# AHupuJR/REFID

Measured on AMD Instinct MI355X. Metric: interpolated frames/sec (train step) GoPro 256x256 11+1, higher is better.
Workload: dtype f32

## Files before the change

### include/refid_hip.h

```cpp
#ifndef REFID_HIP_H
#define REFID_HIP_H

#include <stddef.h>
#include <stdint.h>

#ifdef __cplusplus
extern "C" {
#endif

#define REFID_ABI_VERSION 9

const char* refid_last_error(void);
int refid_abi_version(void);
int refid_experimental_tiles(void);

int refid_device_cu_count(void);

typedef struct refid_pw_extras {
    const float* ln_gamma; const float* ln_beta; float ln_eps; float* ln_out; int ld_ln_out;
    const float* pool; int pool_parts; float inv_hw; int hw; int se_c;
    const float* se_w1; const float* se_b1; const float* se_w2; const float* se_b2;
    float* se_m; float* se_z1; float* se_s;
    float* xs_out; int ld_xs_out;
    const float* res2; int ld_res2;
    float* out2; int ld_out2;
} refid_pw_extras;

typedef struct refid_conv_desc {
    const float* in_a;  const float* in_b;
    int ld_a, ld_b;
    int c_a, c_b;
    const float* w_packed;
    const float* bias;
    float* out;          int ld_out;
    const float* res;    int ld_res;
    const float* mask;   int ld_mask;
    int n, h, w;
    int ho, wo;
    int cout;
    int cout_pad;
    int co_base;
    int kh, kw, stride, pad;
    int mode;
    float slope_pre, slope_post, slope_mask;
    int algo;
    int split_k;
    int wino_tile;
    const refid_pw_extras* pw;
    int mfma_terms;
    float* ws;  size_t ws_bytes;
    const float* add2; int ld_add2;
    float* out2;       int ld_out2;
    int mask_mode;
} refid_conv_desc;

size_t refid_conv_workspace_bytes(const refid_conv_desc* d);
int refid_conv2d(const refid_conv_desc* d, void* stream);

int refid_conv_kc(int kh, int kw, int stride, int mode);
const char* refid_conv_tile_name(int kh, int kw, int stride, int mode, int cout);
int refid_conv_bn(int kh, int kw, int stride, int mode, int cout);

#define REFID_WGRAD_MAX_GROUPS 24
typedef struct refid_wgrad_desc {
    const float* g;      int ld_g;   int c_o;
    const float* in_a;   const float* in_b;
    int ld_a, ld_b;
    int c_a, c_b;
    float* dw;
    float* db;
    float* slabs;
    int n, h, w, ho, wo;
    int kh, kw, stride, pad;
    int i_base, i_total;
    int o_real;
    int algo;
    int phase;
    int groups;
    const float* g_more[REFID_WGRAD_MAX_GROUPS - 1];
    const float* in_a_more[REFID_WGRAD_MAX_GROUPS - 1];
    const float* in_b_more[REFID_WGRAD_MAX_GROUPS - 1];
} refid_wgrad_desc;

size_t refid_wgrad_workspace_bytes(const refid_wgrad_desc* d);
int refid_conv2d_wgrad(const refid_wgrad_desc* d, void* stream);
int refid_wgrad_finish_flush(void* stream);

enum { REFID_ROLE_FWD = 0, REFID_ROLE_DGRAD = 1, REFID_ROLE_CONVT = 2, REFID_ROLE_CONVT_DGRAD = 3,
       REFID_ROLE_DOWN_DGRAD = 4,
       REFID_ROLE_WINO_FWD = 5, REFID_ROLE_WINO_DGRAD = 6,
       REFID_ROLE_CONVT_DGRAD_PW = 7 };
size_t refid_packed_weight_floats(int role, int o, int i, int kh, int kw, int kc, int bn);
int refid_pack_conv_weights(const float* w, float* packed, int role, int o, int i, int kh, int kw,
                            int kc, int bn, void* stream);

int refid_pack_conv_weights_scaled(const float* w, const float* oscale, float* packed, int role, int o,
                                   int i, int kh, int kw, int kc, int bn, void* stream);
int refid_pack_conv_weights_bf16(const float* w, const float* oscale, void* packed_bf16, int role, int o, int i,
                                 int kh, int kw, int kc, int bn, void* stream);
size_t refid_packed_weight_split_bytes(int role, int o, int i, int kh, int kw, int bn, int planes);
size_t refid_packed_weight_split_f16_bytes(int role, int o, int i, int kh, int kw, int bn);
int refid_pack_conv_weights_split_f16(const float* w, const float* oscale, void* packed, int role, int o, int i,
                                      int kh, int kw, int bn, void* stream);
int refid_pack_conv_weights_split(const float* w, const float* oscale, void* packed, int role, int o, int i,
                                  int kh, int kw, int bn, int planes, void* stream);
size_t refid_packed_weight_wino6_bytes(int role, int o, int i, int bn);
int refid_pack_conv_weights_wino6(const float* w, const float* oscale, void* packed, int role, int o, int i, int bn,
                                  void* stream);
size_t refid_packed_weight_wino3h_bytes(int role, int o, int i, int bn);
int refid_pack_conv_weights_wino3h(const float* w, const float* oscale, void* packed, int role, int o, int i, int bn,
                                   void* stream);
size_t refid_packed_weight_wino1h_bytes(int role, int o, int i, int bn);
int refid_pack_conv_weights_wino1h(const float* w, const float* oscale, void* packed, int role, int o, int i, int bn,
                                   void* stream);
size_t refid_pack_entry_bytes(void);
int refid_pack_table_check(const void* table_host, int n);
int refid_pack_entry_fill(void* entry_host, int kind, const float* w, const float* oscale, void* dst, int role, int o, int i,
                          int kh, int kw, int kc, int bn, int planes, int blk0);
int refid_pack_batch_prepass(const void* table_dev, int n, void* stream);
int refid_pack_batch(const void* table_dev, int n, int nblocks, void* stream);
int refid_mul_vec(const float* a, const float* b, float* out, int n, void* stream);
int refid_fold_back(const float* w, const float* b, const float* scale, const float* gw_folded,
                    const float* gb_folded, float* gw, float* gb, float* dscale, int rows, int k, void* stream);

int refid_layernorm2d_fwd(const float* x, int ld_x, const float* w, const float* b, float* out,
                          int ld_out, long long npix, int c, float eps, void* stream);
int refid_layernorm2d_bwd_parts(long long npix, int c);
int refid_layernorm2d_bwd(const float* g, int ld_g, const float* x, int ld_x, const float* w, float* gx,
                          int ld_gx, const float* res, int ld_res, float* dw, float* db, float* parts, long long npix,
                          int c, float eps, void* stream);
int refid_hin_parts(int hw);
int refid_hin_lrelu_fwd(const float* x, int ld_x, const float* gamma, const float* beta, float* out, int ld_out,
                        float* stats, float* parts, int n, int hw, int c, int ch, float eps, float slope,
                        void* stream);
int refid_hin_lrelu_bwd(const float* g, int ld_g, const float* out, int ld_out, const float* x, int ld_x,
                        const float* gamma, const float* stats, float* gx, int ld_gx, float* dgamma,
                        float* dbeta, float* sums, float* parts, int n, int hw, int c, int ch, float slope,
                        void* stream);
int refid_fac_fwd(const float* feat, int ld_feat, const float* filt, int ld_filt, float* out, int ld_out,
                  long long npix, int c, void* stream);
int refid_fac_bwd(const float* g, int ld_g, const float* feat, int ld_feat, const float* filt, int ld_filt,
                  float* gfeat, int ld_gfeat, float* gfilt, int ld_gfilt, long long npix, int c, void* stream);

int refid_dwconv_pool_parts(int h, int wd, int c);
int refid_dwconv3x3_gelu_fwd(const float* in, int ld_in, const float* w, const float* b, float* pre,
                             float* act, float* pool, int n, int h, int wd, int c, void* stream);
int refid_dwconv3x3_bwd_parts(int h, int wd, int c);
int refid_dwconv3x3_bwd(const float* gd, const float* in, int ld_in, const float* w, float* gin,
                        float* dw, float* db, float* parts, int n, int h, int wd, int c, void* stream);
int refid_se_fwd(const float* pool, int n_parts, float inv_hw, const float* w1, const float* b1, const float* w2,
                 const float* b2, float* m, float* z1, float* s, int n, int c, void* stream);
int refid_se_bwd(const float* gs, const float* s, const float* z1, const float* m, const float* w1,
                 const float* w2, float* gm, float* dw1, float* db1, float* dw2, float* db2, float* scratch, int n,
                 int c, void* stream);
int refid_scale_cat(const float* xi, const float* xe, const float* s, float* out, int n, int hw, int c,
                    void* stream);
int refid_egaca_gs_reduce_parts(int hw, int c);
int refid_egaca_gs_reduce(const float* gxs, const float* xi, const float* xe, float* gs, float* parts, int n, int hw,
                          int c, void* stream);
int refid_egaca_bwd_elem(const float* gxs, const float* s, const float* gm, float inv_hw, const float* dwe,
                         float* gdwe, float* gxi, int accumulate_xi, int n, int hw, int c, void* stream);
int refid_gelu_fwd(const float* in, float* out, long long count, void* stream);
int refid_gelu_bwd(const float* g, const float* in, float* out, long long count, void* stream);
int refid_colsum_parts(long long npix, int c);
int refid_colsum(const float* g, int ld_g, float* db, float* parts, long long npix, int c, void* stream);

int refid_charbonnier_parts(long long count);
int refid_charbonnier(const float* pred, const float* gt, float* grad, double* loss_sum, double* parts, long long count,
                      float eps, float grad_scale, void* stream);
int refid_psnr_loss_parts(int n_samples, long long per_sample);
int refid_psnr_loss(const float* pred, const float* gt, float* grad, double* sq, double* loss, double* parts, int n_samples,
                    long long per_sample, float weight, void* stream);
#define REFID_SQNORM_WORDS 2049
int refid_grad_sqnorm(const float* g, double* out, long long count, void* stream);
int refid_clip_adamw(float* p, const float* g, float* m, float* v, const double* sqnorm, float max_norm,
                     float grad_scale, float lr, float beta1, float beta2, float eps, float weight_decay,
                     int step, long long count, void* stream);

int refid_clip_adamw_dev(float* p, const float* g, float* m, float* v, const double* sqnorm, float max_norm,
                         float grad_scale, const float* hyper, float beta1, float beta2, float eps,
                         float weight_decay, long long count, void* stream);

int refid_nchw_to_nhwc(const float* src, long long src_batch_stride, float* dst, int n, int c, int h, int w,
                       int c_pad, void* stream);
int refid_nchw_tsum_to_nhwc(const float* src, long long src_batch_stride, long long t_stride, int t_count, float* dst,
                            int n, int c, int h, int w, int c_pad, void* stream);
int refid_nhwc_to_nchw(const float* src, int ld, float* dst, long long dst_batch_stride,
                       int n, int c, int h, int w, void* stream);
int refid_nchw_to_nhwc_tb(const float* src, long long b_stride, long long t_stride, float* dst, int nb, int nt, int c, int h,
                          int w, int c_pad, void* stream);
int refid_nhwc_to_nchw_tb(const float* src, int ld, float* dst, long long b_stride, long long t_stride, int nb, int nt, int c,
                          int h, int w, void* stream);
int refid_rows_sum_defer(int on);
int refid_rows_sum_flush(void* stream);
int refid_add(const float* a, const float* b, float* out, long long count, void* stream);
#define REFID_SUM_MAX 48
int refid_sum_n(const float* const* in, int n, float* out, long long count, void* stream);
int refid_act_bwd(const float* g, const float* y, float* out, float slope, int accumulate,
                  long long count, void* stream);

int refid_events_to_voxel(const double* ts, const int* xs, const int* ys, const float* ps, long long n_events,
                          int num_bins, int width, int height, double first_stamp, double last_stamp,
                          float* voxel, void* stream);
int refid_sqerr_u8_parts(int n_frames, long long frame_elems);
int refid_sqerr_u8(const float* a, const float* b, int n_frames, long long frame_elems, double* sq, double* parts,
                   void* stream);
int refid_ssim3d_u8_parts(int n_frames, int h, int w);
int refid_ssim3d_u8(const float* a, const float* b, int n_frames, int h, int w, double* sum_out, double* parts,
                    void* stream);
#define REFID_VAL_TAIL_BGR 1
long long refid_val_tail_parts(int n_frames, int h, int w);
int refid_val_tail(const float* pred, const float* gt, int n_frames, int h, int w, int flags, unsigned char* pred_u8,
                   unsigned char* gt_u8, unsigned long long* sq_out, double* ssim_out, void* parts, void* stream);
int refid_tile_add(const float* tile, float* acc, float* cnt, int c, int th, int tw, int h, int w, int i0, int j0,
                   void* stream);
int refid_tile_normalize(float* acc, const float* cnt, int c, int h, int w, void* stream);

typedef struct refid_sample_desc {
    const float* events;
    long long n_events;
    float first_stamp, last_stamp;
    int height, width;
    const unsigned char* frames;
    long long frame_stride;
    int row_pitch;
    int y0, x0;
    int top, left;
    int hflip, vflip, rot90;
} refid_sample_desc;

#define REFID_LAYOUT_BLUR 0
#define REFID_LAYOUT_SHARP 1
#define REFID_ASSEMBLE_ZERO 1
#define REFID_ASSEMBLE_SCATTER 2
#define REFID_ASSEMBLE_FINISH 4
#define REFID_ASSEMBLE_FRAMES 8
#define REFID_ASSEMBLE_ALL 15
typedef struct refid_assemble_desc {
    const refid_sample_desc* samples_host;
    const refid_sample_desc* samples_dev;
    int batch;
    int m, n, layout;
    int crop_h, crop_w;
    long long* scratch;
    float* lq;
    float* voxel;
    float* gt;
} refid_assemble_desc;

int refid_assemble_bins(int m, int n, int layout);
int refid_assemble_batch(const refid_assemble_desc* d, int stages, void* stream);

long long refid_voxel_norm_parts(int batch, long long per_sample);
int refid_voxel_norm(const float* in, float* out, int batch, long long per_sample, void* parts, void* stream);

#define REFID_ASSEMBLE_STATS 16
typedef struct refid_single_desc {
    const refid_sample_desc* samples_host;
    const refid_sample_desc* samples_dev;
    int batch;
    int bins;
    int crop_h, crop_w;
    int norm;
    long long* scratch;
    void* parts;
    float* lq;
    float* voxel;
    float* gt;
} refid_single_desc;
int refid_single_bins(int bins);
int refid_assemble_single(const refid_single_desc* d, int stages, void* stream);

typedef struct refid_seq_pair {
    int left, right;
    long long row0, row1;
    float first_stamp, last_stamp;
} refid_seq_pair;
typedef struct refid_seq_desc {
    const float* events;
    long long n_events;
    const unsigned char* frames;
    int n_frames;
    long long frame_stride;
    int row_pitch;
    int height, width;
    int bgr;
    const refid_seq_pair* pairs_host;
    const refid_seq_pair* pairs_dev;
    int n_pairs;
    int m, n, layout;
    int out_h, out_w;
    long long* scratch;
    float* lq;
    float* voxel;
} refid_seq_desc;
int refid_seq_assemble(const refid_seq_desc* d, int stages, void* stream);

typedef struct refid_seq_single_desc {
    const float* events;
    long long n_events;
    const unsigned char* frames;
    int n_frames;
    long long frame_stride;
    int row_pitch;
    int height, width;
    int bgr;
    const refid_seq_pair* items_host;
    const refid_seq_pair* items_dev;
    int n_items;
    int bins;
    int norm;
    int out_h, out_w;
    long long* scratch;
    void* parts;
// ... 55 lines not shown
```

### refid_amd/_lib.py

```python
import ctypes as C
import os

_HERE = os.path.dirname(os.path.abspath(__file__))
LIB_PATH = os.path.join(_HERE, "librefid_hip.so")


class RefidHipError(RuntimeError):
    pass


class PwExtras(C.Structure):
    _fields_ = [
        ("ln_gamma", C.c_void_p), ("ln_beta", C.c_void_p), ("ln_eps", C.c_float), ("ln_out", C.c_void_p),
        ("ld_ln_out", C.c_int),
        ("pool", C.c_void_p), ("pool_parts", C.c_int), ("inv_hw", C.c_float), ("hw", C.c_int), ("se_c", C.c_int),
        ("se_w1", C.c_void_p), ("se_b1", C.c_void_p), ("se_w2", C.c_void_p), ("se_b2", C.c_void_p),
        ("se_m", C.c_void_p), ("se_z1", C.c_void_p), ("se_s", C.c_void_p),
        ("xs_out", C.c_void_p), ("ld_xs_out", C.c_int),
        ("res2", C.c_void_p), ("ld_res2", C.c_int),
        ("out2", C.c_void_p), ("ld_out2", C.c_int),
    ]


class ConvDesc(C.Structure):
    _fields_ = [
        ("in_a", C.c_void_p), ("in_b", C.c_void_p),
        ("ld_a", C.c_int), ("ld_b", C.c_int),
        ("c_a", C.c_int), ("c_b", C.c_int),
        ("w_packed", C.c_void_p), ("bias", C.c_void_p),
        ("out", C.c_void_p), ("ld_out", C.c_int),
        ("res", C.c_void_p), ("ld_res", C.c_int),
        ("mask", C.c_void_p), ("ld_mask", C.c_int),
        ("n", C.c_int), ("h", C.c_int), ("w", C.c_int),
        ("ho", C.c_int), ("wo", C.c_int),
        ("cout", C.c_int), ("cout_pad", C.c_int), ("co_base", C.c_int),
        ("kh", C.c_int), ("kw", C.c_int), ("stride", C.c_int), ("pad", C.c_int),
        ("mode", C.c_int),
        ("slope_pre", C.c_float), ("slope_post", C.c_float), ("slope_mask", C.c_float),
        ("algo", C.c_int),
        ("split_k", C.c_int), ("wino_tile", C.c_int),
        ("pw", C.POINTER(PwExtras)),
        ("mfma_terms", C.c_int),
        ("ws", C.c_void_p), ("ws_bytes", C.c_size_t),
        ("add2", C.c_void_p), ("ld_add2", C.c_int), ("out2", C.c_void_p), ("ld_out2", C.c_int),
        ("mask_mode", C.c_int),
    ]


WGRAD_MAX_GROUPS = 24


class WgradDesc(C.Structure):
    _fields_ = [
        ("g", C.c_void_p), ("ld_g", C.c_int), ("c_o", C.c_int),
        ("in_a", C.c_void_p), ("in_b", C.c_void_p),
        ("ld_a", C.c_int), ("ld_b", C.c_int),
        ("c_a", C.c_int), ("c_b", C.c_int),
        ("dw", C.c_void_p), ("db", C.c_void_p), ("slabs", C.c_void_p),
        ("n", C.c_int), ("h", C.c_int), ("w", C.c_int), ("ho", C.c_int), ("wo", C.c_int),
        ("kh", C.c_int), ("kw", C.c_int), ("stride", C.c_int), ("pad", C.c_int),
        ("i_base", C.c_int), ("i_total", C.c_int), ("o_real", C.c_int), ("algo", C.c_int),
        ("phase", C.c_int),
        ("groups", C.c_int),
        ("g_more", C.c_void_p * (WGRAD_MAX_GROUPS - 1)), ("in_a_more", C.c_void_p * (WGRAD_MAX_GROUPS - 1)),
        ("in_b_more", C.c_void_p * (WGRAD_MAX_GROUPS - 1)),
    ]


class SampleDesc(C.Structure):
    _fields_ = [
        ("events", C.c_void_p), ("n_events", C.c_longlong),
        ("first_stamp", C.c_float), ("last_stamp", C.c_float),
        ("height", C.c_int), ("width", C.c_int),
        ("frames", C.c_void_p), ("frame_stride", C.c_longlong), ("row_pitch", C.c_int),
        ("y0", C.c_int), ("x0", C.c_int),
        ("top", C.c_int), ("left", C.c_int),
        ("hflip", C.c_int), ("vflip", C.c_int), ("rot90", C.c_int),
    ]


class AssembleDesc(C.Structure):
    _fields_ = [
        ("samples_host", C.c_void_p), ("samples_dev", C.c_void_p),
        ("batch", C.c_int),
        ("m", C.c_int), ("n", C.c_int), ("layout", C.c_int),
        ("crop_h", C.c_int), ("crop_w", C.c_int),
        ("scratch", C.c_void_p),
        ("lq", C.c_void_p), ("voxel", C.c_void_p), ("gt", C.c_void_p),
    ]


class SingleDesc(C.Structure):
    _fields_ = [
        ("samples_host", C.c_void_p), ("samples_dev", C.c_void_p),
        ("batch", C.c_int),
        ("bins", C.c_int),
        ("crop_h", C.c_int), ("crop_w", C.c_int),
        ("norm", C.c_int),
        ("scratch", C.c_void_p),
        ("parts", C.c_void_p),
        ("lq", C.c_void_p), ("voxel", C.c_void_p), ("gt", C.c_void_p),
    ]


class SeqPair(C.Structure):
    _fields_ = [
        ("left", C.c_int), ("right", C.c_int),
        ("row0", C.c_longlong), ("row1", C.c_longlong),
        ("first_stamp", C.c_float), ("last_stamp", C.c_float),
    ]


class SeqDesc(C.Structure):
    _fields_ = [
        ("events", C.c_void_p), ("n_events", C.c_longlong),
        ("frames", C.c_void_p), ("n_frames", C.c_int),
        ("frame_stride", C.c_longlong), ("row_pitch", C.c_int), ("height", C.c_int), ("width", C.c_int), ("bgr", C.c_int),
        ("pairs_host", C.c_void_p), ("pairs_dev", C.c_void_p), ("n_pairs", C.c_int),
        ("m", C.c_int), ("n", C.c_int), ("layout", C.c_int),
        ("out_h", C.c_int), ("out_w", C.c_int),
        ("scratch", C.c_void_p),
        ("lq", C.c_void_p), ("voxel", C.c_void_p),
    ]


class SeqSingleDesc(C.Structure):
    _fields_ = [
        ("events", C.c_void_p), ("n_events", C.c_longlong),
        ("frames", C.c_void_p), ("n_frames", C.c_int),
        ("frame_stride", C.c_longlong), ("row_pitch", C.c_int), ("height", C.c_int), ("width", C.c_int), ("bgr", C.c_int),
        ("items_host", C.c_void_p), ("items_dev", C.c_void_p), ("n_items", C.c_int),
        ("bins", C.c_int), ("norm", C.c_int),
        ("out_h", C.c_int), ("out_w", C.c_int),
        ("scratch", C.c_void_p),
        ("parts", C.c_void_p),
        ("lq", C.c_void_p), ("voxel", C.c_void_p),
    ]


class PngUnfilterDesc(C.Structure):
    _fields_ = [
        ("rows", C.c_void_p), ("frames", C.c_void_p), ("bands", C.c_void_p),
        ("n_bands", C.c_int32), ("n_frames", C.c_int32), ("height", C.c_int32), ("width", C.c_int32), ("channels", C.c_int32),
    ]


class PngFilterDesc(C.Structure):
    _fields_ = [
        ("frames", C.c_void_p), ("rows", C.c_void_p), ("costs", C.c_void_p),
        ("n_frames", C.c_int32), ("height", C.c_int32), ("width", C.c_int32), ("mode", C.c_int32),
    ]


class PngDeflateDesc(C.Structure):
    _fields_ = [
        ("src", C.c_void_p), ("out", C.c_void_p), ("lens", C.c_void_p), ("work", C.c_void_p),
        ("n_streams", C.c_int32), ("stream_bytes", C.c_int32), ("block_bytes", C.c_int32), ("out_pitch", C.c_int32),
    ]


LAYOUT_BLUR, LAYOUT_SHARP = 0, 1
ASSEMBLE_ZERO, ASSEMBLE_SCATTER, ASSEMBLE_FINISH, ASSEMBLE_FRAMES, ASSEMBLE_ALL = 1, 2, 4, 8, 15
ASSEMBLE_STATS = 16

VAL_TAIL_BGR = 1
NIQE_BGR = 1
SCORE_BGR = 1
PNG_MAX_ROW_BYTES = 32760
PNG_FILTER_ADAPTIVE = 5
PNG_FILTER_MAX_WIDTH = 11184810
PNG_DEFLATE_BLOCK = 32768
PNG_DEFLATE_MAX_BLOCK = 65535
PNG_DEFLATE_RECORD = 1088
ABI_VERSION = 9
_lib = None

_PACK_FAMILY = (
    ("refid_packed_weight_floats", ("refid_pack_conv_weights", "refid_pack_conv_weights_scaled", "refid_pack_conv_weights_bf16"),
     "role o i kh kw kc bn"),
    ("refid_packed_weight_split_bytes", ("refid_pack_conv_weights_split",), "role o i kh kw bn planes"),
    ("refid_packed_weight_split_f16_bytes", ("refid_pack_conv_weights_split_f16",), "role o i kh kw bn"),
    ("refid_packed_weight_wino6_bytes", ("refid_pack_conv_weights_wino6",), "role o i bn"),
    ("refid_packed_weight_wino3h_bytes", ("refid_pack_conv_weights_wino3h",), "role o i bn"),
    ("refid_packed_weight_wino1h_bytes", ("refid_pack_conv_weights_wino1h",), "role o i bn"),
)
PACK_GEO = {}


def lib():
    global _lib
    if _lib is not None:
        return _lib
    if not os.path.exists(LIB_PATH):
        raise RefidHipError(
            f"{LIB_PATH} not found: the HIP extension is required (no CPU/eager fallback). "
            "Run `python -m refid_amd.build`.")
    L = C.CDLL(LIB_PATH)
    L.refid_last_error.restype = C.c_char_p
    L.refid_abi_version.restype = C.c_int
    L.refid_device_cu_count.restype = C.c_int
    L.refid_conv2d.argtypes = [C.POINTER(ConvDesc), C.c_void_p]
    L.refid_conv_workspace_bytes.argtypes = [C.POINTER(ConvDesc)]
    L.refid_conv_workspace_bytes.restype = C.c_size_t
    L.refid_conv_kc.argtypes = [C.c_int] * 4
    L.refid_conv_bn.argtypes = [C.c_int] * 5
    L.refid_conv_tile_name.argtypes = [C.c_int] * 5
    L.refid_conv_tile_name.restype = C.c_char_p
    L.refid_wgrad_workspace_bytes.argtypes = [C.POINTER(WgradDesc)]
    L.refid_wgrad_workspace_bytes.restype = C.c_size_t
    L.refid_conv2d_wgrad.argtypes = [C.POINTER(WgradDesc), C.c_void_p]
    L.refid_wgrad_finish_flush.argtypes = [C.c_void_p]
    L.refid_rows_sum_defer.argtypes = [C.c_int]
    L.refid_rows_sum_flush.argtypes = [C.c_void_p]
    L.refid_nchw_to_nhwc.argtypes = [C.c_void_p, C.c_longlong, C.c_void_p] + [C.c_int] * 5 + [C.c_void_p]
    L.refid_nchw_tsum_to_nhwc.argtypes = [C.c_void_p, C.c_longlong, C.c_longlong, C.c_int, C.c_void_p] + [C.c_int] * 5 + \
        [C.c_void_p]
    L.refid_nhwc_to_nchw.argtypes = [C.c_void_p, C.c_int, C.c_void_p, C.c_longlong] + [C.c_int] * 4 + [C.c_void_p]
    L.refid_nchw_to_nhwc_tb.argtypes = [C.c_void_p, C.c_longlong, C.c_longlong, C.c_void_p] + [C.c_int] * 6 + [C.c_void_p]
    L.refid_nhwc_to_nchw_tb.argtypes = [C.c_void_p, C.c_int, C.c_void_p, C.c_longlong, C.c_longlong] + [C.c_int] * 5 + [C.c_void_p]
    L.refid_add.argtypes = [C.c_void_p, C.c_void_p, C.c_void_p, C.c_longlong, C.c_void_p]
    L.refid_sum_n.argtypes = [C.c_void_p, C.c_int, C.c_void_p, C.c_longlong, C.c_void_p]
    L.refid_act_bwd.argtypes = [C.c_void_p, C.c_void_p, C.c_void_p, C.c_float, C.c_int, C.c_longlong, C.c_void_p]
    _bind_extra(L)
    if L.refid_abi_version() != ABI_VERSION:
        raise RefidHipError("librefid_hip.so ABI version mismatch")
    _lib = L
    return L


def _bind_extra(L):
    vp, i, f, ll = C.c_void_p, C.c_int, C.c_float, C.c_longlong
    for size, entries, geo in _PACK_FAMILY:
        PACK_GEO[size] = geo = tuple(geo.split())
        getattr(L, size).argtypes, getattr(L, size).restype = [i] * len(geo), C.c_size_t
        for e in entries:
            PACK_GEO[e] = geo
            getattr(L, e).argtypes = [vp] * (2 if e == "refid_pack_conv_weights" else 3) + [i] * len(geo) + [vp]
    L.refid_pack_batch_prepass.argtypes = [vp, i, vp]
    L.refid_mul_vec.argtypes = [vp, vp, vp, i, vp]
    L.refid_pack_entry_bytes.restype = C.c_size_t
    L.refid_pack_entry_bytes.argtypes = []
    L.refid_pack_entry_fill.argtypes = [vp, i, vp, vp, vp, i, i, i, i, i, i, i, i, i]
    L.refid_pack_batch.argtypes = [vp, i, i, vp]
    L.refid_pack_table_check.argtypes = [vp, i]
    L.refid_fold_back.argtypes = [vp] * 8 + [i, i, vp]
    L.refid_layernorm2d_fwd.argtypes = [vp, i, vp, vp, vp, i, ll, i, f, vp]
    L.refid_layernorm2d_bwd.argtypes = [vp, i, vp, i, vp, vp, i, vp, i, vp, vp, vp, ll, i, f, vp]
    L.refid_layernorm2d_bwd_parts.argtypes = [ll, i]
    L.refid_colsum_parts.argtypes = [ll, i]
    L.refid_egaca_gs_reduce_parts.argtypes = [i, i]
    L.refid_dwconv3x3_gelu_fwd.argtypes = [vp, i, vp, vp, vp, vp, vp, i, i, i, i, vp]
    L.refid_dwconv3x3_bwd.argtypes = [vp, vp, i, vp, vp, vp, vp, vp, i, i, i, i, vp]
    L.refid_dwconv3x3_bwd_parts.argtypes = [i, i, i]
    L.refid_se_fwd.argtypes = [vp, i, f, vp, vp, vp, vp, vp, vp, vp, i, i, vp]
    L.refid_dwconv_pool_parts.argtypes = [i, i, i]
    L.refid_se_bwd.argtypes = [vp] * 12 + [i, i, vp]
    L.refid_scale_cat.argtypes = [vp, vp, vp, vp, i, i, i, vp]
    L.refid_egaca_gs_reduce.argtypes = [vp, vp, vp, vp, vp, i, i, i, vp]
    L.refid_egaca_bwd_elem.argtypes = [vp, vp, vp, f, vp, vp, vp, i, i, i, i, vp]
    L.refid_gelu_fwd.argtypes = [vp, vp, ll, vp]
    L.refid_gelu_bwd.argtypes = [vp, vp, vp, ll, vp]
    L.refid_colsum.argtypes = [vp, i, vp, vp, ll, i, vp]
    L.refid_charbonnier_parts.argtypes = [ll]
    L.refid_charbonnier.argtypes = [vp, vp, vp, vp, vp, ll, f, f, vp]
    L.refid_grad_sqnorm.argtypes = [vp, vp, ll, vp]
    L.refid_psnr_loss_parts.argtypes = [i, ll]
    L.refid_psnr_loss.argtypes = [vp, vp, vp, vp, vp, vp, i, ll, f, vp]
    L.refid_clip_adamw.argtypes = [vp, vp, vp, vp, vp, f, f, f, f, f, f, f, i, ll, vp]
    L.refid_clip_adamw_dev.argtypes = [vp, vp, vp, vp, vp, f, f, vp, f, f, f, f, ll, vp]
    d = C.c_double
    L.refid_events_to_voxel.argtypes = [vp, vp, vp, vp, ll, i, i, i, d, d, vp, vp]
    L.refid_sqerr_u8_parts.argtypes = [i, ll]
    L.refid_sqerr_u8.argtypes = [vp, vp, i, ll, vp, vp, vp]
    L.refid_ssim3d_u8_parts.argtypes = [i, i, i]
    L.refid_ssim3d_u8.argtypes = [vp, vp, i, i, i, vp, vp, vp]
    L.refid_val_tail_parts.argtypes = [i, i, i]
    L.refid_val_tail_parts.restype = ll
    L.refid_val_tail.argtypes = [vp, vp, i, i, i, i, vp, vp, vp, vp, vp, vp]
    L.refid_tile_add.argtypes = [vp, vp, vp, i, i, i, i, i, i, i, vp]
    L.refid_tile_normalize.argtypes = [vp, vp, i, i, i, vp]
    L.refid_hin_parts.argtypes = [i]
    L.refid_hin_lrelu_fwd.argtypes = [vp, i, vp, vp, vp, i, vp, vp, i, i, i, i, f, f, vp]
    L.refid_hin_lrelu_bwd.argtypes = [vp, i, vp, i, vp, i, vp, vp, vp, i, vp, vp, vp, vp, i, i, i, i, f, vp]
    L.refid_fac_fwd.argtypes = [vp, i, vp, i, vp, i, ll, i, vp]
    L.refid_fac_bwd.argtypes = [vp, i, vp, i, vp, i, vp, i, vp, i, ll, i, vp]
    L.refid_assemble_bins.argtypes = [i, i, i]
    L.refid_assemble_batch.argtypes = [C.POINTER(AssembleDesc), i, vp]
    L.refid_seq_assemble.argtypes = [C.POINTER(SeqDesc), i, vp]
    L.refid_voxel_norm_parts.argtypes = [i, ll]
    L.refid_voxel_norm_parts.restype = ll
    L.refid_voxel_norm.argtypes = [vp, vp, i, ll, vp, vp]
    L.refid_single_bins.argtypes = [i]
    L.refid_assemble_single.argtypes = [C.POINTER(SingleDesc), i, vp]
    L.refid_seq_assemble_single.argtypes = [C.POINTER(SeqSingleDesc), i, vp]
    L.refid_niqe_moments_parts.argtypes = [i, i, i]
    L.refid_niqe_moments_parts.restype = ll
    L.refid_niqe_moments.argtypes = [vp, i, i, i, i, i, vp, vp, vp, vp, vp, vp, vp]
    L.refid_png_unfilter.argtypes = [C.POINTER(PngUnfilterDesc), vp]
    L.refid_png_filter.argtypes = [C.POINTER(PngFilterDesc), vp]
    L.refid_png_deflate_bound.argtypes = [C.c_int32, C.c_int32]
    L.refid_png_deflate_bound.restype = C.c_size_t
    L.refid_png_deflate_work_bytes.argtypes = [C.c_int32, C.c_int32, C.c_int32]
    L.refid_png_deflate_work_bytes.restype = C.c_size_t
    L.refid_png_deflate.argtypes = [C.POINTER(PngDeflateDesc), vp]
    L.refid_score_u8_parts.argtypes = [i, i, i, i]
    L.refid_score_u8_parts.restype = ll
    L.refid_score_u8.argtypes = [vp, vp, i, i, i, i, i, vp, vp, vp, vp, vp, vp, vp, vp]


def check(rc, what):
    if rc != 0:
        msg = lib().refid_last_error().decode("utf-8", "replace")
        raise RefidHipError(f"{what} failed (rc={rc}): {msg}")
```

### refid_amd/csrc/conv_args.h

```cpp
#pragma once
#include <functional>

struct ConvKArgs {
    const float* inA; const float* inB;
    int ldA, ldB, Ca, Ctot;
    const float* w; const float* bias;
    float* out; int ldO;
    const float* res; int ldR;
    const float* mask; int ldM;
    int N, H, W, Ho, Wo;
    int Cout, CoutPad, coBase;
    int pad, nchunks, tilesX, tilesY;
    float slopePre, slopePost, slopeMask;
    long long wClsStride;
    int vecOK;
    int ncot;
    int bf16;
    int ksplit = 1;
    long long wsStride = 0;
    const float* add2 = nullptr; float* out2 = nullptr; int ldA2 = 0, ldO2 = 0;
    int maskMode = 0;
    int shuffle = 0;
    int patchW = 0, patchRow = 0;
};


int refid_splitk_count(int nwg, int nchunks, int wgLimit, int minChunks, int div);
size_t refid_splitk_bytes(int ks, long long npix, int cout);
int refid_launch_splitk(const char* tile, const ConvKArgs& a, int ks, long long npix, float* ws, size_t ws_bytes,
                        const std::function<int(const ConvKArgs&)>& partial, hipStream_t st);
size_t refid_wino3x3_workspace_bytes(const ConvKArgs& a, int split_mode);
int refid_launch_wino3x3(const ConvKArgs& a, float* ws, size_t ws_bytes, int split_mode, hipStream_t st);
bool refid_wino6_eligible(const ConvKArgs& a);
size_t refid_wino6_workspace_bytes(const ConvKArgs& a, int split_mode);
int refid_launch_wino6(const ConvKArgs& a, float* ws, size_t ws_bytes, int split_mode, int tile_hint, int terms, hipStream_t st);
bool refid_split3x3_eligible(const ConvKArgs& a);
int refid_launch_split3x3(const ConvKArgs& a, int terms, int mode, int cus, int split_mode, hipStream_t st);
struct PwExtra {
    const float* lnG = nullptr; const float* lnB = nullptr; float lnEps = 0.f; float* lnOut = nullptr; int ldLn = 0;
    const float* pool = nullptr; int poolParts = 0; float invHW = 0.f; int hw = 0; int seC = 0;
    const float* seW1 = nullptr; const float* seB1 = nullptr; const float* seW2 = nullptr; const float* seB2 = nullptr;
    float* seM = nullptr; float* seZ1 = nullptr; float* seS = nullptr;
    float* xsOut = nullptr; int ldXs = 0;
    const float* res2 = nullptr; int ldR2 = 0;
    float* out2 = nullptr; int ldO2 = 0;
};
int refid_launch_pointwise(const ConvKArgs& a, hipStream_t st, const PwExtra* ex = nullptr, int terms = 0);
```

### refid_amd/csrc/conv_igemm.hip

```cpp
#include "common.h"
#include "conv_args.h"
#include "conv_epilogue.h"
#include "conv_planes.h"

namespace {

template <int KH_, int KW_, int S_, int WM_, int WN_, int MT_, int NT_, int NSUB_, int MODE_>
struct Cfg {
    static constexpr int KH = KH_, KW = KW_, S = S_, WM = WM_, WN = WN_, MT = MT_, NT = NT_;
    static constexpr int NSUB = NSUB_, MODE = MODE_;
    static constexpr int TW = 32;
    static constexpr int TH = WM * MT;
    static constexpr int BN = WN * NT * 32;
    static constexpr int NTAPS = (MODE == 2) ? 4 : KH * KW;
    static constexpr int HH = (MODE == 2) ? TH + 2 : (TH - 1) * S + KH;
    static constexpr int HWD = (MODE == 2) ? TW + 2 : (TW - 1) * S + KW;
    static constexpr int HP = HH * HWD;
    static constexpr int NQ = NSUB * 2;
    static constexpr int KC = NSUB * 8;
    static constexpr int A_TOTAL = HP * NQ;
    static constexpr int B_TOTAL = NTAPS * BN * NQ;
    static constexpr int A_ITEMS = (A_TOTAL + 255) / 256;
    static constexpr int B_ITEMS = (B_TOTAL + 255) / 256;
    static constexpr int LDS_BYTES = (A_TOTAL + B_TOTAL) * 16;
// ... 276 lines not shown
    if (kh == 4 && kw == 4 && stride == 2) return F_4x4s2;
    if (kh == 2 && kw == 2 && stride == 2) return F_2x2s2;
    return F_none;
}

}

extern "C" int refid_conv_kc(int kh, int kw, int stride, int mode) {
    switch (family_of(kh, kw, stride, mode)) {
        case F_3x3: case F_5x5: case F_4x4s2: case F_2x2s2: return 8;
        case F_1x1: case F_convT: return 32;
        case F_downDgrad: return 16;
        default: return -1;
    }
}

extern "C" int refid_conv_bn(int kh, int kw, int stride, int mode, int cout) {
    switch (family_of(kh, kw, stride, mode)) {
        case F_3x3: case F_1x1: return cout <= 32 ? 32 : (cout <= 64 ? 64 : 128);
        case F_5x5: return 32;
        case F_4x4s2: return 64;
        case F_2x2s2: case F_downDgrad: case F_convT: return cout <= 64 ? 64 : 128;
        default: return -1;
    }
}

extern "C" const char* refid_conv_tile_name(int kh, int kw, int stride, int mode, int cout) {
    const int bn = refid_conv_bn(kh, kw, stride, mode, cout);
    switch (family_of(kh, kw, stride, mode)) {
        case F_3x3: return bn == 32 ? "Cfg<3, 3, 1, 4, 1, 2, 1, 1, 0>" : bn == 64 ? "Cfg<3, 3, 1, 4, 1, 2, 2, 1, 0>"
                                                                                  : "Cfg<3, 3, 1, 2, 2, 2, 2, 1, 0>";
        case F_5x5: return "Cfg<5, 5, 1, 4, 1, 2, 1, 1, 0>";
        case F_1x1: return bn == 32 ? "Cfg<1, 1, 1, 4, 1, 2, 1, 4, 0>" : bn == 64 ? "Cfg<1, 1, 1, 4, 1, 2, 2, 4, 0>"
                                                                                  : "Cfg<1, 1, 1, 2, 2, 2, 2, 4, 0>";
        case F_4x4s2: return "Cfg<4, 4, 2, 4, 1, 2, 2, 1, 0>";
        case F_2x2s2: return bn == 64 ? "Cfg<2, 2, 2, 4, 1, 2, 2, 1, 0>" : "Cfg<2, 2, 2, 2, 2, 2, 2, 1, 0>";
        case F_convT: return bn == 64 ? "Cfg<1, 1, 1, 4, 1, 2, 2, 4, 1>" : "Cfg<1, 1, 1, 2, 2, 2, 2, 4, 1>";
        case F_downDgrad: return bn == 64 ? "Cfg<3, 3, 1, 4, 1, 2, 2, 2, 2>" : "Cfg<3, 3, 1, 2, 2, 2, 2, 2, 2>";
        default: return "none";
    }
}

extern "C" size_t refid_conv_workspace_bytes(const refid_conv_desc* d) {
    if (!d || d->split_k == 0) return 0;
    ConvKArgs a;
    a.Ca = d->c_a; a.Ctot = d->c_a + d->c_b;
    a.N = d->n; a.H = d->h; a.W = d->w; a.Ho = d->ho; a.Wo = d->wo;
    a.Cout = d->cout; a.CoutPad = d->cout_pad; a.coBase = d->co_base;
    a.vecOK = 1;
    if (d->algo == 1) return refid_wino3x3_workspace_bytes(a, d->split_k);
    if (d->algo == 5) return refid_wino6_workspace_bytes(a, d->split_k);
    if (d->algo != 0 && d->algo != 2) return 0;
    const bool bf = d->algo == 2;
    const int bn = refid_conv_bn(d->kh, d->kw, d->stride, d->mode, d->cout);
    switch (family_of(d->kh, d->kw, d->stride, d->mode)) {
        case F_4x4s2: return igemm_ws_bytes<C4S2_64>(a, 1, d->split_k, bf);
        case F_downDgrad: return bn == 64 ? igemm_ws_bytes<CD_64>(a, 4, d->split_k, bf) : igemm_ws_bytes<CD_128>(a, 4, d->split_k, bf);
        default: return 0;
    }
}

extern "C" int refid_conv2d(const refid_conv_desc* d, void* stream) {
    hipStream_t st = reinterpret_cast<hipStream_t>(stream);
    REFID_CHECK(d != nullptr, "conv2d: null descriptor");
    const Family f = family_of(d->kh, d->kw, d->stride, d->mode);
    REFID_CHECK(f != F_none, "conv2d: unsupported geometry k=%dx%d stride=%d mode=%d", d->kh, d->kw,
                d->stride, d->mode);
    REFID_CHECK(d->in_a && d->w_packed && d->out, "conv2d: null tensor pointer");
    REFID_CHECK(d->c_a > 0 && d->c_a % 4 == 0 && d->c_b % 4 == 0 && d->c_b >= 0,
                "conv2d: channel counts must be multiples of 4 (c_a=%d c_b=%d)", d->c_a, d->c_b);
    REFID_CHECK(d->ld_a % 4 == 0 && (d->c_b == 0 || d->ld_b % 4 == 0),
                "conv2d: pixel pitches must be multiples of 4 floats");
    REFID_CHECK(d->c_b == 0 || d->in_b != nullptr, "conv2d: c_b > 0 but in_b is null");
    REFID_CHECK(d->n > 0 && d->h > 0 && d->w > 0 && d->ho > 0 && d->wo > 0 && d->cout > 0,
                "conv2d: empty problem (n=%d h=%d w=%d ho=%d wo=%d cout=%d)", d->n, d->h, d->w, d->ho,
                d->wo, d->cout);
    REFID_CHECK(d->pw == nullptr || d->algo == 3, "conv2d: pw fusions belong to the pointwise tile (algo 3)");
    REFID_CHECK(d->algo == 0 || d->algo == 2 || ((d->algo == 1 || d->algo == 5) && f == F_3x3) || (d->algo == 3 && (f == F_1x1 || f == F_convT || f == F_2x2s2)) ||
                    (d->algo == 4 && (f == F_3x3 || f == F_4x4s2 || f == F_downDgrad)),
                "conv2d: algo %d does not fit this geometry (1 / 5 = 3x3 stride 1, 3 = 1x1 and ConvTranspose2d(2,2), 4 = 3x3 stride 1 / 4x4 stride 2 and "
                "its input gradient)", d->algo);
    REFID_CHECK(d->algo != 2 || d->c_b == 0 || d->c_a % 8 == 0, "conv2d: bf16 tile needs c_a %% 8 == 0 for two sources");
    const int bn = refid_conv_bn(d->kh, d->kw, d->stride, d->mode, d->cout);
    REFID_CHECK(d->co_base >= 0 && d->co_base + d->cout <= d->cout_pad,
                "conv2d: rows [%d, %d) exceed the packed weight's %d rows", d->co_base, d->co_base + d->cout,
                d->cout_pad);
    if (d->mode == 0) {
        const int eh = (d->h + 2 * d->pad - d->kh) / d->stride + 1;
        const int ew = (d->w + 2 * d->pad - d->kw) / d->stride + 1;
        REFID_CHECK(eh == d->ho && ew == d->wo, "conv2d: output size %dx%d does not match geometry (%dx%d)",
                    d->ho, d->wo, eh, ew);
    } else {
        REFID_CHECK(d->ho == d->h && d->wo == d->w, "conv2d: mode %d needs ho,wo == h,w", d->mode);
        REFID_CHECK(d->mode != 1 || d->cout % 4 == 0, "conv2d: mode 1 needs cout = 4*Co");
    }
    ConvKArgs a;
    a.inA = d->in_a; a.inB = d->in_b; a.ldA = d->ld_a; a.ldB = d->ld_b;
    a.Ca = d->c_a; a.Ctot = d->c_a + d->c_b;
    a.w = d->w_packed; a.bias = d->bias;
    a.out = d->out; a.ldO = d->ld_out;
    a.res = d->res; a.ldR = d->ld_res;
    a.mask = d->mask; a.ldM = d->ld_mask;
    a.add2 = d->add2; a.ldA2 = d->ld_add2; a.out2 = d->out2; a.ldO2 = d->ld_out2;
    a.maskMode = d->mask_mode;
    REFID_CHECK(d->mask_mode == 0 || (d->mask_mode == 1 && d->algo == 3 && d->mask != nullptr),
                "conv2d: mask_mode 1 (GELU derivative) belongs to the pointwise tile (algo 3) and needs a mask tensor");
    REFID_CHECK(d->out2 == nullptr || (d->add2 != nullptr && (d->algo != 3 || d->pw == nullptr)),
                "conv2d: out2 needs add2 (and, on the pointwise tile, no fusions)");
    a.N = d->n; a.H = d->h; a.W = d->w; a.Ho = d->ho; a.Wo = d->wo;
    a.Cout = d->cout; a.CoutPad = d->cout_pad; a.coBase = d->co_base;
    a.pad = d->pad; a.nchunks = 0; a.tilesX = a.tilesY = 0;
    a.slopePre = d->slope_pre; a.slopePost = d->slope_post; a.slopeMask = d->slope_mask;
    auto al16 = [](const void* p) { return (reinterpret_cast<uintptr_t>(p) & 15) == 0; };
    a.vecOK = al16(d->out) && d->ld_out % 4 == 0 && (!d->res || (al16(d->res) && d->ld_res % 4 == 0)) &&
              (!d->mask || (al16(d->mask) && d->ld_mask % 4 == 0)) && (!d->bias || al16(d->bias)) &&
              (!d->out2 || (al16(d->out2) && d->ld_out2 % 4 == 0 && al16(d->add2) && d->ld_add2 % 4 == 0)) &&
              d->co_base % 4 == 0 && (d->mode != 1 || (d->cout / 4) % 4 == 0);
    a.bf16 = (d->algo == 2);
    a.ncot = 0;
    const int kc = refid_conv_kc(d->kh, d->kw, d->stride, d->mode) * (a.bf16 ? 2 : 1);
    a.wClsStride = (long long)cdiv(a.Ctot, kc) * 4 * d->cout_pad * kc;
    if (d->algo == 3) {
        a.shuffle = (d->mode == 1) ? 1 : 0;
        REFID_CHECK(!a.shuffle || (d->pw == nullptr && d->mask == nullptr && d->out2 == nullptr && d->co_base == 0),
                    "conv2d: ConvTranspose2d on the pointwise tile takes no mask / second output / fusions / row range");
        if (f == F_2x2s2) {
            REFID_CHECK(d->c_b == 0 && d->ld_a == d->c_a && d->pad == 0 && d->h == 2 * d->ho && d->w == 2 * d->wo && d->pw == nullptr &&
                            (2 * d->c_a) % 8 == 0,
                        "conv2d: the 2x2 stride-2 patch GEMM (algo 3) needs one source with dense pixels (ld_a == c_a), pad 0, "
                        "even input sizes and c_a %% 4 == 0");
            a.inB = d->in_a + (long long)d->w * d->ld_a;
            a.ldA = a.ldB = 2 * d->ld_a;
            a.Ca = 2 * d->c_a; a.Ctot = 4 * d->c_a;
            a.patchW = d->wo; a.patchRow = 2 * d->w * d->ld_a;
            a.H = d->ho; a.W = d->wo;
            REFID_CHECK((long long)d->n * d->h * d->w * d->ld_a * 4 < 0x7fffffffLL, "conv2d: tensor too large for the pointwise tile's 32-bit offsets");
            return refid_launch_pointwise(a, st, nullptr, 0);
        }
        REFID_CHECK(d->c_b == 0 || d->c_a % 8 == 0, "conv2d: pointwise tile needs c_a %% 8 == 0 for two sources");
        const long long lim = 0x7fffffffLL;
        REFID_CHECK((long long)d->n * d->h * d->w * d->ld_a * 4 < lim &&
                        (d->c_b == 0 || (long long)d->n * d->h * d->w * d->ld_b * 4 < lim),
                    "conv2d: tensor too large for the pointwise tile's 32-bit offsets (use algo 0)");
        if (d->pw != nullptr) {
            const refid_pw_extras* x = d->pw;
            PwExtra e;
            e.lnG = x->ln_gamma; e.lnB = x->ln_beta; e.lnEps = x->ln_eps; e.lnOut = x->ln_out; e.ldLn = x->ld_ln_out;
            e.pool = x->pool; e.poolParts = x->pool_parts; e.invHW = x->inv_hw; e.hw = x->hw; e.seC = x->se_c;
            e.seW1 = x->se_w1; e.seB1 = x->se_b1; e.seW2 = x->se_w2; e.seB2 = x->se_b2;
            e.seM = x->se_m; e.seZ1 = x->se_z1; e.seS = x->se_s;
            e.xsOut = x->xs_out; e.ldXs = x->ld_xs_out;
            e.res2 = x->res2; e.ldR2 = x->ld_res2;
            e.out2 = x->out2; e.ldO2 = x->ld_out2;
            auto al = [](const void* q, int ld) { return (reinterpret_cast<uintptr_t>(q) & 15) == 0 && ld % 4 == 0; };
            REFID_CHECK((!e.lnOut || al(e.lnOut, e.ldLn)) && (!e.xsOut || al(e.xsOut, e.ldXs)) && (!e.res2 || al(e.res2, e.ldR2)) &&
                            (!e.out2 || al(e.out2, e.ldO2)) && (!e.lnG || (al(e.lnG, 4) && al(e.lnB, 4))),
                        "conv2d: pointwise fusion tensors must be 16-byte aligned with pitches that are multiples of 4");
            return refid_launch_pointwise(a, st, &e, d->mfma_terms);
        }
        return refid_launch_pointwise(a, st, nullptr, d->mfma_terms);
    }
    if (d->algo == 4) {
        static int cus = 0;
        if (cus == 0) cus = refid_device_cu_count();
        REFID_CHECK(d->pad == 1, "conv2d: the split tile's geometries all have pad 1");
        return refid_launch_split3x3(a, d->mfma_terms ? d->mfma_terms : 6, f == F_3x3 ? 0 : (f == F_4x4s2 ? 1 : 2),
                                     cus > 0 ? cus : 256, d->split_k, st);
    }
    if (d->algo == 5) return refid_launch_wino6(a, d->ws, d->ws_bytes, d->split_k, d->wino_tile, d->mfma_terms, st);
    if (d->algo == 1) {
        REFID_CHECK(d->c_b == 0 || d->c_a % 8 == 0, "conv2d: Winograd tile needs c_a %% 8 == 0 for two sources");
        const long long lim = 0x7fffffffLL;
        REFID_CHECK((long long)d->n * d->h * d->w * d->ld_a * 4 < lim &&
                        (d->c_b == 0 || (long long)d->n * d->h * d->w * d->ld_b * 4 < lim),
                    "conv2d: tensor too large for the Winograd tile's 32-bit offsets (use algo 0)");
        return refid_launch_wino3x3(a, d->ws, d->ws_bytes, d->split_k, st);
    }
    switch (f) {
        case F_3x3:
            if (bn == 32) return launch<C3_32>(a, 1, st);
            if (bn == 64) return launch<C3_64>(a, 1, st);
            return launch<C3_128>(a, 1, st);
        case F_5x5: return launch<C5_32>(a, 1, st);
        case F_1x1:
            if (bn == 32) return launch<C1_32>(a, 1, st);
            if (bn == 64) return launch<C1_64>(a, 1, st);
            return launch<C1_128>(a, 1, st);
        case F_4x4s2: return launch<C4S2_64>(a, 1, st, SplitArgs{d->ws, d->ws_bytes, d->split_k});
        case F_2x2s2: return bn == 64 ? launch<C2S2_64>(a, 1, st) : launch<C2S2_128>(a, 1, st);
        case F_convT: return bn == 64 ? launch<CT_64>(a, 1, st) : launch<CT_128>(a, 1, st);
        case F_downDgrad: {
            const SplitArgs sp{d->ws, d->ws_bytes, d->split_k};
            return bn == 64 ? launch<CD_64>(a, 4, st, sp) : launch<CD_128>(a, 4, st, sp);
        }
        default: break;
    }
    refid_set_error("conv2d: no tile for this geometry");
    return 1;
}
```

### refid_amd/csrc/conv_pw.hip

```cpp
#include "common.h"
#include "conv_args.h"
#include "conv_epilogue.h"
#include "conv_planes.h"
#include <cstdlib>

namespace {

typedef unsigned int u32x4 __attribute__((ext_vector_type(4)));
constexpr int KC = 8;
__device__ constexpr int PW_TA[6] = {0, 1, 0, 2, 0, 1};
__device__ constexpr int PW_TB[6] = {0, 0, 1, 0, 2, 1};

template <int NT, int XD, bool EX, bool SIX = false>
__global__ __launch_bounds__(256, (SIX || NT > 2) ? 3 : 4) void conv_pw_kernel(const ConvKArgs a, const PwExtra e) {
    const int lane = threadIdx.x & 63, wave = threadIdx.x >> 6;
    const int li = lane & 31, kh = lane >> 5;
    const long long npix = (long long)a.N * a.H * a.W;
    const long long p0 = ((long long)blockIdx.x * 4 + wave) * 32;
    const long long p = p0 + li;
    const int n0 = blockIdx.y * (32 * NT);

    const long long spanA = a.patchW ? (npix / a.patchW) * (long long)a.patchRow : npix * a.ldA;
    const long long spanB = a.patchW ? spanA - a.patchRow / 2 : npix * (a.inB ? a.ldB : a.ldA);
    const __amdgpu_buffer_rsrc_t rsA = __builtin_amdgcn_make_buffer_rsrc(
        const_cast<float*>(a.inA), 0, (int)min(spanA * 4, 0x7fffffffLL), 0x00020000);
    const __amdgpu_buffer_rsrc_t rsB = __builtin_amdgcn_make_buffer_rsrc(
        const_cast<float*>(a.inB ? a.inB : a.inA), 0, (int)min(spanB * 4, 0x7fffffffLL), 0x00020000);
    const __amdgpu_buffer_rsrc_t rsW = __builtin_amdgcn_make_buffer_rsrc(
        const_cast<float*>(a.w), 0, (int)min((long long)a.nchunks * a.CoutPad * KC * (SIX ? 6 : 4), 0x7fffffffLL), 0x00020000);
    const bool pok = p < npix;
    const long long pA = a.patchW ? (p / a.patchW) * a.patchRow + (p % a.patchW) * a.ldA : p * a.ldA;
    const long long pB = a.patchW ? (p / a.patchW) * a.patchRow + (p % a.patchW) * a.ldB : p * a.ldB;
    const int voA = pok ? (int)(pA * 4) + kh * 16 : OOB;
    const int voB = pok ? (int)(pB * 4) + kh * 16 : OOB;
    int voW[NT];
#pragma unroll
    for (int nt = 0; nt < NT; ++nt) {
        const int row = a.coBase + n0 + nt * 32 + li;
        voW[nt] = (row < a.CoutPad) ? (SIX ? row * 32 + kh * 16 : (row * KC + kh * 4) * 4) : OOB;
    }
    const int wChunk = a.CoutPad * KC * 4;
    const int wPlane = a.CoutPad * 32;

    f32x16 acc[NT];
#pragma unroll
    for (int nt = 0; nt < NT; ++nt)
#pragma unroll
        for (int r = 0; r < 16; ++r) acc[nt][r] = 0.f;

    auto load_x = [&](int ch) -> f32x4 {
        const int c0 = ch * KC;
        const bool fromA = c0 < a.Ca;
        const int soff = (fromA ? c0 : c0 - a.Ca) * 4;
        const int vo = (c0 + kh * 4 < a.Ctot) ? (fromA ? voA : voB) : OOB;
        const u32x4 v = fromA ? __builtin_amdgcn_raw_buffer_load_b128(rsA, vo, soff, 0)
                              : __builtin_amdgcn_raw_buffer_load_b128(rsB, vo, soff, 0);
        return __builtin_bit_cast(f32x4, v);
    };
    auto load_w = [&](int ch, f32x4 (&dst)[NT]) {
#pragma unroll
        for (int nt = 0; nt < NT; ++nt)
            dst[nt] = __builtin_bit_cast(f32x4, __builtin_amdgcn_raw_buffer_load_b128(rsW, voW[nt], ch * wChunk, 0));
    };
    auto load_w6 = [&](int c16, f32x4 (&dst)[3][NT]) {
#pragma unroll
        for (int pl = 0; pl < 3; ++pl)
#pragma unroll
            for (int nt = 0; nt < NT; ++nt)
                dst[pl][nt] = __builtin_bit_cast(f32x4, __builtin_amdgcn_raw_buffer_load_b128(rsW, voW[nt], (c16 * 3 + pl) * wPlane, 0));
    };
    auto mfma6 = [&](const f32x4& x0, const f32x4& x1, const f32x4 (&w6)[3][NT]) {
        f32x4 pl[3];
        split8<3>(x0, x1, pl);
#pragma unroll
        for (int t = 0; t < 6; ++t)
#pragma unroll
            for (int nt = 0; nt < NT; ++nt)
                acc[nt] = __builtin_amdgcn_mfma_f32_32x32x16_bf16(__builtin_bit_cast(bf16x8, w6[PW_TA[t]][nt]),
                                                                  __builtin_bit_cast(bf16x8, pl[PW_TB[t]]), acc[nt], 0, 0, 0);
    };

    f32x4 xr[2 * XD];
    f32x4 wr[SIX ? 1 : 2][NT];
    f32x4 w6[SIX ? 2 : 1][3][NT];
    const int nch = a.nchunks;
    __shared__ float sS[EX ? 128 : 1];
    bool ln_done = false;
    if constexpr (EX) {
        if (e.pool != nullptr) {
            __shared__ float sM[128], sZ[64];
            const int C = e.seC, Ch = C / 2, tid = threadIdx.x;
            const int n = (int)(((long long)blockIdx.x * 128) / e.hw);
            for (int c = tid; c < C; c += 256) {
                const float* pp = e.pool + (long long)n * e.poolParts * C + c;
                float s0 = 0.f;
                for (int r = 0; r < e.poolParts; ++r) s0 += pp[(long long)r * C];
                sM[c] = s0 * e.invHW;
            }
            __syncthreads();
            for (int j = tid; j < Ch; j += 256) {
                float z = e.seB1[j];
                for (int c = 0; c < C; ++c) z += e.seW1[j * C + c] * sM[c];
                sZ[j] = z > 0.f ? z : 0.f;
            }
            __syncthreads();
            for (int c = tid; c < C; c += 256) {
                float v = e.seB2[c];
                for (int j = 0; j < Ch; ++j) v += e.seW2[c * Ch + j] * sZ[j];
                sS[c] = 1.f / (1.f + __expf(-v));
            }
            __syncthreads();
            if (e.seS != nullptr && blockIdx.y == 0 && ((long long)blockIdx.x * 128) % e.hw == 0) {
                for (int c = tid; c < C; c += 256) { e.seM[n * C + c] = sM[c]; e.seS[n * C + c] = sS[c]; }
                for (int j = tid; j < Ch; j += 256) e.seZ1[n * Ch + j] = sZ[j];
            }
        }
        if (e.lnG != nullptr) {
#pragma unroll
            for (int j = 0; j < 2 * XD; ++j) xr[j] = (j < nch) ? load_x(j) : f32x4{0.f, 0.f, 0.f, 0.f};
            if constexpr (SIX) load_w6(0, w6[0]);
            else load_w(0, wr[0]);
            float s1 = 0.f;
#pragma unroll
            for (int j = 0; j < 2 * XD; ++j) s1 += (xr[j][0] + xr[j][1]) + (xr[j][2] + xr[j][3]);
            s1 += __shfl_xor(s1, 32, 64);
            const float mu = s1 / (float)a.Ctot;
            float s2 = 0.f;
#pragma unroll
            for (int j = 0; j < 2 * XD; ++j)
                if (j < nch) {
#pragma unroll
                    for (int k = 0; k < 4; ++k) { const float d = xr[j][k] - mu; s2 += d * d; }
                }
            s2 += __shfl_xor(s2, 32, 64);
            const float rstd = 1.f / sqrtf(s2 / (float)a.Ctot + e.lnEps);
#pragma unroll
            for (int j = 0; j < 2 * XD; ++j)
                if (j < nch) {
                    const int c = j * KC + kh * 4;
                    const f32x4 gv = *reinterpret_cast<const f32x4*>(e.lnG + c);
                    const f32x4 bv = *reinterpret_cast<const f32x4*>(e.lnB + c);
#pragma unroll
                    for (int k = 0; k < 4; ++k) xr[j][k] = (xr[j][k] - mu) * rstd * gv[k] + bv[k];
                    if (e.lnOut != nullptr && blockIdx.y == 0 && pok)
                        *reinterpret_cast<f32x4*>(e.lnOut + p * e.ldLn + c) = xr[j];
                }
            if constexpr (SIX) {
#pragma unroll
                for (int j = 0; j < 2 * XD; j += 2)
                    if (j < nch) {
                        if (j + 2 < nch) load_w6(j / 2 + 1, w6[(j / 2 + 1) & 1]);
                        mfma6(xr[j], xr[j + 1], w6[(j / 2) & 1]);
                    }
            } else {
#pragma unroll
                for (int j = 0; j < 2 * XD; ++j)
                    if (j < nch) {
                        if (j + 1 < nch) load_w(j + 1, wr[(j + 1) & 1]);
#pragma unroll
                        for (int kk = 0; kk < 4; ++kk)
#pragma unroll
                            for (int nt = 0; nt < NT; ++nt)
                                acc[nt] = __builtin_amdgcn_mfma_f32_32x32x2f32(wr[j & 1][nt][kk], xr[j][kk], acc[nt], 0, 0, 0);
                    }
            }
            ln_done = true;
        }
    }
    if (!ln_done) {
#pragma unroll
        for (int j = 0; j < XD; ++j)
            if (j < nch) xr[j] = load_x(j);
        if constexpr (SIX) load_w6(0, w6[0]);
        else load_w(0, wr[0]);
        for (int c0 = 0; c0 < nch; c0 += 2 * XD) {
#pragma unroll
            for (int j = 0; j < 2 * XD; ++j) {
                const int c = c0 + j;
                if (c < nch) {
                    if constexpr (SIX) {
                        if ((j & 1) == 0 && c + 2 < nch) load_w6(c / 2 + 1, w6[(j / 2 + 1) & 1]);
                    } else {
                        if (c + 1 < nch) load_w(c + 1, wr[(j + 1) & 1]);
                    }
                    if (c + XD < nch) xr[(j + XD) % (2 * XD)] = load_x(c + XD);
                    if constexpr (EX) {
                        if (e.pool != nullptr) {
                            const int k0 = c * KC + kh * 4;
                            const f32x4 sv = *reinterpret_cast<const f32x4*>(&sS[k0 % e.seC]);
                            xr[j] *= sv;
                            if (e.xsOut != nullptr && blockIdx.y == 0 && pok)
                                *reinterpret_cast<f32x4*>(e.xsOut + p * e.ldXs + k0) = xr[j];
                        }
                    }
                    if constexpr (SIX) {
                        if (j & 1) mfma6(xr[j - 1], xr[j], w6[(j / 2) & 1]);
                    } else {
#pragma unroll
                        for (int kk = 0; kk < 4; ++kk)
#pragma unroll
                            for (int nt = 0; nt < NT; ++nt)
                                acc[nt] = __builtin_amdgcn_mfma_f32_32x32x2f32(wr[j & 1][nt][kk], xr[j][kk], acc[nt], 0, 0, 0);
                    }
                }
            }
        }
    }

    if (a.vecOK) {
        constexpr int HN = (NT > 2) ? 2 : NT;
        constexpr int PITCH = 8 * HN + 1;
        __shared__ f32x4 sT[4][32 * PITCH];
        f32x4* t = sT[wave];
#pragma unroll
        for (int h0 = 0; h0 < NT; h0 += HN) {
            if (h0) __syncthreads();
#pragma unroll
            for (int nt = 0; nt < HN; ++nt)
#pragma unroll
                for (int g = 0; g < 4; ++g) {
                    f32x4 v;
#pragma unroll
                    for (int k = 0; k < 4; ++k) v[k] = acc[h0 + nt][4 * g + k];
                    t[li * PITCH + nt * 8 + 2 * g + kh] = v;
                }
            __syncthreads();
#pragma unroll
            for (int it = 0; it < 4 * HN; ++it) {
                const int f = it * 64 + lane;
                const int px = f / (8 * HN), c4 = f % (8 * HN);
                const long long pp = p0 + px;
                const int j0 = n0 + h0 * 32 + c4 * 4;
                if (pp >= npix || j0 >= a.Cout) continue;
                f32x4 v = t[px * PITCH + c4];
                if (a.shuffle) {
                    const int Co1 = a.Cout >> 2;
                    const unsigned qd = (unsigned)j0 / (unsigned)Co1, ch = (unsigned)j0 - qd * Co1;
                    const unsigned up = (unsigned)pp, row = up / (unsigned)a.W, x = up - row * a.W;
                    const long long op = (long long)(2 * row + (qd >> 1)) * (2 * a.W) + 2 * x + (qd & 1);
                    conv_epilogue(a, v, ch, j0, true, EpiAtOp{op, (int)ch}, false);
                    continue;
                }
                const float* res2 = nullptr;
                if constexpr (EX) {
                    if (e.res2) res2 = e.res2 + pp * e.ldR2 + j0;
                }
                conv_epilogue<true>(a, v, a.coBase + j0, j0, true, EpiAtOp{pp, j0}, false, res2);
                if constexpr (EX) {
                    if (e.out2) {
                        f32x4 gl;
#pragma unroll
                        for (int k = 0; k < 4; ++k) gl[k] = gelu_f(v[k]);
                        *reinterpret_cast<f32x4*>(e.out2 + pp * e.ldO2 + j0) = gl;
                    }
                }
            }
        }
        return;
    }
    if (!pok) return;
#pragma unroll
    for (int nt = 0; nt < NT; ++nt) {
#pragma unroll
        for (int g = 0; g < 4; ++g) {
            const int j0 = n0 + nt * 32 + 8 * g + 4 * kh;
            f32x4 v;
#pragma unroll
            for (int k = 0; k < 4; ++k) v[k] = acc[nt][4 * g + k];
            conv_epilogue<true>(a, v, a.coBase + j0, j0, false, EpiAtOp{p, j0});
        }
    }
}

}

int refid_launch_pointwise(const ConvKArgs& ka, hipStream_t st, const PwExtra* ex, int terms) {
    ConvKArgs a = ka;
    a.nchunks = cdiv(a.Ctot, KC);
    if (a.Cout % 4) a.vecOK = 0;
    const long long npix = (long long)a.N * a.H * a.W;
    const int nb = (int)((npix + 127) / 128);
    const bool six = terms == 6;
    REFID_CHECK(!a.shuffle || (a.vecOK && ex == nullptr && terms == 0 && a.mask == nullptr && a.Cout > 32 && (a.Cout / 4) % 4 == 0 &&
                               npix < 0x7fffffffLL),
                "conv2d: ConvTranspose2d on the pointwise tile needs 16-byte aligned tensors, fp32 products, no mask / fusions and "
                "at least 16 output channels");
    REFID_CHECK(a.out2 == nullptr || (a.vecOK && ex == nullptr), "conv2d: the pointwise tile's second output needs 16-byte aligned tensors and no fusions");
    REFID_CHECK(!a.patchW || (terms == 0 && ex == nullptr && a.inB != nullptr), "conv2d: the patch form of the pointwise tile has fp32 products, no fusions");
    REFID_CHECK(terms == 0 || terms == 6, "conv2d: the pointwise tile has fp32 products (0) or six bf16 products (6), got %d", terms);
    REFID_CHECK(!six || (a.Ctot % 16 == 0 && (a.inB == nullptr || a.Ca % 16 == 0) && a.Cout > 32),
                "conv2d: the six-product pointwise tile needs channel counts that are multiples of 16 and more than 32 outputs");
    if (ex != nullptr) {
        REFID_CHECK(a.vecOK && a.Cout > 32, "conv2d: pointwise fusions need 16-byte aligned tensors and more than 32 outputs");
        REFID_CHECK(!ex->lnG || (a.inB == nullptr && a.Ctot % 8 == 0 && a.Ctot <= 64 && ex->lnB),
                    "conv2d: the LayerNorm prologue needs one source of at most 64 channels (got %d)", a.Ctot);
        REFID_CHECK(!ex->pool || (ex->hw > 0 && ex->hw % 128 == 0 && ex->seC >= 8 && ex->seC <= 128 && ex->seC % 8 == 0 &&
                                  a.Ctot % ex->seC == 0 && ex->poolParts > 0 && ex->seW1 && ex->seB1 && ex->seW2 && ex->seB2 &&
                                  (!ex->seS || (ex->seM && ex->seZ1)) && !ex->lnG),
                    "conv2d: bad squeeze-excite fusion arguments (pixels per sample must be a multiple of 128)");
        if (six) hipLaunchKernelGGL((conv_pw_kernel<2, 4, true, true>), dim3(nb, cdiv(a.Cout, 64)), dim3(256), 0, st, a, *ex);
        else hipLaunchKernelGGL((conv_pw_kernel<2, 4, true>), dim3(nb, cdiv(a.Cout, 64)), dim3(256), 0, st, a, *ex);
        REFID_LAUNCH_CHECK("conv_pw/fused");
        return 0;
    }
    const PwExtra none;
    if (six) hipLaunchKernelGGL((conv_pw_kernel<2, 4, false, true>), dim3(nb, cdiv(a.Cout, 64)), dim3(256), 0, st, a, none);
    else if (a.Cout <= 32) hipLaunchKernelGGL((conv_pw_kernel<1, 8, false>), dim3(nb, 1), dim3(256), 0, st, a, none);
    else {
        static const bool nt4 = []() { const char* e = getenv("REFID_PW_NT4"); return e && e[0] == '1'; }();
        if (nt4 && a.Cout % 128 == 0)
            hipLaunchKernelGGL((conv_pw_kernel<4, 4, false>), dim3(nb, a.Cout / 128), dim3(256), 0, st, a, none);
        else
            hipLaunchKernelGGL((conv_pw_kernel<2, 4, false>), dim3(nb, cdiv(a.Cout, 64)), dim3(256), 0, st, a, none);
    }
    REFID_LAUNCH_CHECK("conv_pw");
    return 0;
}
```

### refid_amd/csrc/egaca.hip

```cpp
#include "common.h"
#include <vector>
#include <cstring>

namespace {

template <int LPP>
__device__ __forceinline__ float group_sum(float v) {
#pragma unroll
    for (int o = LPP / 2; o > 0; o >>= 1) v += __shfl_xor(v, o, 64);
    return v;
}

template <int LPP>
__device__ __forceinline__ float wave_rows_sum(float v) {
#pragma unroll
    for (int o = LPP; o < 64; o <<= 1) v += __shfl_xor(v, o, 64);
    return v;
}

__global__ __launch_bounds__(256) void rows_sum_kernel(const float* __restrict__ parts, int nrows, int ncols,
                                                      float* __restrict__ dst_a, int n_a, float* __restrict__ dst_b,
                                                      int accumulate) {
    const int lane = threadIdx.x & 63;
    const int i = blockIdx.x * 4 + (threadIdx.x >> 6);
    if (i >= ncols) return;
    float a = 0.f;
    for (int b = lane; b < nrows; b += 64) a += parts[(long long)b * ncols + i];
#pragma unroll
    for (int o = 32; o > 0; o >>= 1) a += __shfl_xor(a, o, 64);
    if (lane == 0) {
        float* d = i < n_a ? dst_a + i : dst_b + (i - n_a);
        *d = accumulate ? *d + a : a;
    }
}

constexpr int ROWS_JOBS = 160, ROWS_GROUPS = 24;
struct RowsJob { const float* parts; int nrows; int pad; };
struct RowsGroup { float* dst_a; float* dst_b; int ncols, n_a, first, count, blk0, pad; };
struct RowsBatch { RowsJob job[ROWS_JOBS]; RowsGroup grp[ROWS_GROUPS]; int ngroups; };
static_assert(sizeof(RowsBatch) <= 4096, "kernel-argument block");

__global__ __launch_bounds__(256) void rows_sum_batch_kernel(const RowsBatch b) {
    int gi = 0;
    for (int k = 1; k < b.ngroups; ++k) gi = (int)blockIdx.x >= b.grp[k].blk0 ? k : gi;
    const RowsGroup& g = b.grp[gi];
    const int lane = threadIdx.x & 63;
    const int i = ((int)blockIdx.x - g.blk0) * 4 + (threadIdx.x >> 6);
    if (i >= g.ncols) return;
    float* d = i < g.n_a ? g.dst_a + i : g.dst_b + (i - g.n_a);
    float tot = *d;
    for (int j = g.first; j < g.first + g.count; ++j) {
        const float* parts = b.job[j].parts;
        const int nrows = b.job[j].nrows;
        float a = 0.f;
        for (int r = lane; r < nrows; r += 64) a += parts[(long long)r * g.ncols + i];
#pragma unroll
        for (int o = 32; o > 0; o >>= 1) a += __shfl_xor(a, o, 64);
        tot += a;
    }
    if (lane == 0) *d = tot;
}

struct RowsPending { const float* parts; int nrows, ncols; float* dst_a; int n_a; float* dst_b; };
thread_local std::vector<RowsPending> rows_queue;
thread_local bool rows_defer = false;

int rows_sum_issue(const float* parts, int nrows, int ncols, float* dst_a, int n_a, float* dst_b, hipStream_t st, const char* what) {
    if (rows_defer) {
        rows_queue.push_back({parts, nrows, ncols, dst_a, n_a, dst_b});
        return 0;
    }
    hipLaunchKernelGGL(rows_sum_kernel, dim3(cdiv(ncols, 4)), dim3(256), 0, st, parts, nrows, ncols, dst_a, n_a, dst_b, 1);
    REFID_LAUNCH_CHECK(what);
    return 0;
}

int rows_sum_flush(hipStream_t st) {
    std::vector<char> done(rows_queue.size(), 0);
    size_t left = rows_queue.size();
    while (left) {
        RowsBatch b;
        memset(&b, 0, sizeof(b));
        int nj = 0, ng = 0, blk = 0;
        for (size_t k = 0; k < rows_queue.size() && ng < ROWS_GROUPS && nj < ROWS_JOBS; ++k) {
            if (done[k]) continue;
            const RowsPending& q = rows_queue[k];
            bool open = false;
            for (int g = 0; g < ng; ++g) open = open || (b.grp[g].dst_a == q.dst_a && b.grp[g].dst_b == q.dst_b);
            if (open) continue;
            RowsGroup& g = b.grp[ng];
            g.dst_a = q.dst_a; g.dst_b = q.dst_b; g.ncols = q.ncols; g.n_a = q.n_a; g.first = nj; g.count = 0; g.blk0 = blk;
            for (size_t m = k; m < rows_queue.size() && nj < ROWS_JOBS; ++m) {
                const RowsPending& r = rows_queue[m];
                if (done[m] || r.dst_a != q.dst_a || r.dst_b != q.dst_b) continue;
                if (r.ncols != q.ncols || r.n_a != q.n_a) break;
                b.job[nj].parts = r.parts; b.job[nj].nrows = r.nrows;
                ++nj; ++g.count; done[m] = 1; --left;
            }
            blk += cdiv(g.ncols, 4);
            ++ng;
        }
        b.ngroups = ng;
        hipLaunchKernelGGL(rows_sum_batch_kernel, dim3(blk), dim3(256), 0, st, b);
        if (hipGetLastError() != hipSuccess) { rows_queue.clear(); refid_set_error("rows_sum_batch: launch failed"); return 1; }
    }
    rows_queue.clear();
    return 0;
}

template <int LPP>
__global__ __launch_bounds__(256) void ln_fwd_kernel(const float* __restrict__ x, int ldx,
                                                    const float* __restrict__ w, const float* __restrict__ b,
                                                    float* __restrict__ out, int ldo, long long npix, float eps) {
    constexpr int C = LPP * 4, PPB = 256 / LPP;
    const int q = threadIdx.x % LPP;
    const f32x4 wv = *reinterpret_cast<const f32x4*>(w + q * 4);
    const f32x4 bv = *reinterpret_cast<const f32x4*>(b + q * 4);
    for (long long p = blockIdx.x * (long long)PPB + threadIdx.x / LPP; p < npix; p += (long long)gridDim.x * PPB) {
        const f32x4 v = *reinterpret_cast<const f32x4*>(x + p * ldx + q * 4);
        const float mu = group_sum<LPP>(v[0] + v[1] + v[2] + v[3]) * (1.f / C);
        const f32x4 d = v - mu;
        const float var = group_sum<LPP>(d[0] * d[0] + d[1] * d[1] + d[2] * d[2] + d[3] * d[3]) * (1.f / C);
        const float rstd = 1.f / sqrtf(var + eps);
        *reinterpret_cast<f32x4*>(out + p * ldo + q * 4) = wv * (d * rstd) + bv;
    }
}

template <int LPP>
__global__ __launch_bounds__(256) void ln_bwd_kernel(const float* __restrict__ g, int ldg,
                                                    const float* __restrict__ x, int ldx,
                                                    const float* __restrict__ w, float* gx, int ldgx,
                                                    const float* res, int ldr, float* __restrict__ parts,
                                                    long long npix, float eps) {
    constexpr int C = LPP * 4, PPB = 256 / LPP;
    __shared__ float sred[4][2 * C];
    const int q = threadIdx.x % LPP;
    const f32x4 wv = *reinterpret_cast<const f32x4*>(w + q * 4);
    f32x4 pdw = {0.f, 0.f, 0.f, 0.f}, pdb = {0.f, 0.f, 0.f, 0.f};
    constexpr int U = 4;
    const long long stride = (long long)gridDim.x * PPB;
    for (long long p0 = blockIdx.x * (long long)PPB + threadIdx.x / LPP; p0 < npix; p0 += stride * U) {
        f32x4 v[U], gv[U], rv[U];
        bool ok[U];
#pragma unroll
        for (int u = 0; u < U; ++u) {
            const long long p = p0 + u * stride;
            ok[u] = p < npix;
            const long long pc = ok[u] ? p : p0;
            v[u] = *reinterpret_cast<const f32x4*>(x + pc * ldx + q * 4);
            gv[u] = *reinterpret_cast<const f32x4*>(g + pc * ldg + q * 4);
            rv[u] = res ? *reinterpret_cast<const f32x4*>(res + pc * ldr + q * 4) : f32x4{0.f, 0.f, 0.f, 0.f};
        }
#pragma unroll
// ... 172 lines not shown
    const int lane = threadIdx.x & 63, wave = threadIdx.x >> 6;
    for (int j = wave; j < Ch; j += 4) {
        float a = 0.f;
        for (int c = lane; c < C; c += 64) a += W1[j * C + c] * sm[c];
#pragma unroll
        for (int o = 32; o > 0; o >>= 1) a += __shfl_xor(a, o, 64);
        if (lane == 0) {
            a += b1[j];
            a = a > 0.f ? a : 0.f;
            sz[j] = a; z1[n * Ch + j] = a;
        }
    }
    __syncthreads();
    for (int c = wave; c < C; c += 4) {
        float a = 0.f;
        for (int j = lane; j < Ch; j += 64) a += W2[c * Ch + j] * sz[j];
#pragma unroll
        for (int o = 32; o > 0; o >>= 1) a += __shfl_xor(a, o, 64);
        if (lane == 0) s[n * C + c] = 1.f / (1.f + __expf(-(a + b2[c])));
    }
}

__global__ __launch_bounds__(256) void se_bwd_kernel(const float* __restrict__ gs, const float* __restrict__ s,
                                                    const float* __restrict__ z1, const float* __restrict__ m,
                                                    const float* __restrict__ W1, const float* __restrict__ W2,
                                                    float* __restrict__ gm, float* __restrict__ scratch, int N, int C) {
    __shared__ float d2[256], d1[128], sz[128], sm[256];
    const int Ch = C / 2;
    const int n = blockIdx.x;
    for (int c = threadIdx.x; c < C; c += 256) {
        const float sv = s[n * C + c];
        d2[c] = gs[n * C + c] * sv * (1.f - sv);
        sm[c] = m[n * C + c];
    }
    for (int j = threadIdx.x; j < Ch; j += 256) sz[j] = z1[n * Ch + j];
    __syncthreads();
    for (int j = threadIdx.x; j < Ch; j += 256) {
        float a = 0.f;
        for (int c = 0; c < C; ++c) a += W2[c * Ch + j] * d2[c];
        d1[j] = sz[j] > 0.f ? a : 0.f;
    }
    __syncthreads();
    for (int c = threadIdx.x; c < C; c += 256) {
        float a = 0.f;
        for (int j = 0; j < Ch; ++j) a += W1[j * C + c] * d1[j];
        gm[n * C + c] = a;
        scratch[n * (C + Ch) + c] = d2[c];
    }
    for (int j = threadIdx.x; j < Ch; j += 256) scratch[n * (C + Ch) + C + j] = d1[j];
}

__global__ __launch_bounds__(256) void se_bwd_params_kernel(const float* __restrict__ scratch, const float* __restrict__ z1,
                                                           const float* __restrict__ m, float* __restrict__ dW1,
                                                           float* __restrict__ db1, float* __restrict__ dW2,
                                                           float* __restrict__ db2, int N, int C) {
    const int Ch = C / 2, S = C + Ch;
    const int e = blockIdx.x * 256 + threadIdx.x;
    if (e < C * Ch) {
        float a2 = 0.f, a1 = 0.f;
        for (int n = 0; n < N; ++n) {
            a2 += scratch[n * S + e / Ch] * z1[n * Ch + e % Ch];
            a1 += scratch[n * S + C + e / C] * m[n * C + e % C];
        }
        dW2[e] += a2;
        dW1[e] += a1;
    }
    if (e < C) { float a = 0.f; for (int n = 0; n < N; ++n) a += scratch[n * S + e]; db2[e] += a; }
    if (e < Ch) { float a = 0.f; for (int n = 0; n < N; ++n) a += scratch[n * S + C + e]; db1[e] += a; }
}

template <int LPP>
__global__ __launch_bounds__(256) void scale_cat_kernel(const float* __restrict__ xi, const float* __restrict__ xe,
                                                       const float* __restrict__ s, float* __restrict__ out,
                                                       int HW, long long npix) {
    constexpr int C = LPP * 4, L2 = LPP * 2, PPB = 256 / L2;
    const int q = threadIdx.x % L2;
    for (long long p = blockIdx.x * (long long)PPB + threadIdx.x / L2; p < npix; p += (long long)gridDim.x * PPB) {
        const int n = (int)(p / HW);
        const int c = (q % LPP) * 4;
        const float* src = (q < LPP ? xi : xe) + p * C + c;
        const f32x4 v = *reinterpret_cast<const f32x4*>(src);
        const f32x4 sv = *reinterpret_cast<const f32x4*>(s + n * C + c);
        *reinterpret_cast<f32x4*>(out + p * 2 * C + q * 4) = v * sv;
    }
}

template <int LPP>
__global__ __launch_bounds__(256) void gs_reduce_kernel(const float* __restrict__ gxs, const float* __restrict__ xi,
                                                       const float* __restrict__ xe, float* __restrict__ parts, int HW) {
    constexpr int C = LPP * 4, PPB = 256 / LPP;
    __shared__ float sred[4][C];
    const int q = threadIdx.x % LPP, n = blockIdx.y;
    f32x4 ps = {0.f, 0.f, 0.f, 0.f};
    for (int p = blockIdx.x * PPB + threadIdx.x / LPP; p < HW; p += gridDim.x * PPB) {
        const long long pix = (long long)n * HW + p;
        const f32x4 gi = *reinterpret_cast<const f32x4*>(gxs + pix * 2 * C + q * 4);
        const f32x4 ge = *reinterpret_cast<const f32x4*>(gxs + pix * 2 * C + C + q * 4);
        const f32x4 a = *reinterpret_cast<const f32x4*>(xi + pix * C + q * 4);
        const f32x4 b = *reinterpret_cast<const f32x4*>(xe + pix * C + q * 4);
        ps += gi * a + ge * b;
    }
    const int wave = threadIdx.x >> 6, lane = threadIdx.x & 63;
#pragma unroll
    for (int k = 0; k < 4; ++k) {
        const float a = wave_rows_sum<LPP>(ps[k]);
        if (lane < LPP) sred[wave][q * 4 + k] = a;
    }
    __syncthreads();
    if (threadIdx.x < C)
        parts[((long long)n * gridDim.x + blockIdx.x) * C + threadIdx.x] =
            ((sred[0][threadIdx.x] + sred[1][threadIdx.x]) + sred[2][threadIdx.x]) + sred[3][threadIdx.x];
}

__global__ __launch_bounds__(256) void gs_sum_kernel(const float* __restrict__ parts, int nblk, int C, int total,
                                                    float* __restrict__ gs) {
    const int n = blockIdx.x, c = threadIdx.x % C, r = threadIdx.x / C, R = 256 / C;
    __shared__ float sh[256];
    float a = 0.f;
    for (int b = r; b < nblk; b += R) a += parts[((long long)n * nblk + b) * C + c];
    sh[threadIdx.x] = a;
    __syncthreads();
    if (threadIdx.x < C) {
        float t = sh[threadIdx.x];
        for (int k = 1; k < R; ++k) t += sh[k * C + threadIdx.x];
        gs[n * C + threadIdx.x] = t;
    }
}

template <int LPP>
__global__ __launch_bounds__(256) void egaca_bwd_elem_kernel(const float* __restrict__ gxs, const float* __restrict__ s,
                                                            const float* __restrict__ gm, float invHW,
                                                            const float* __restrict__ dwe, float* __restrict__ gdwe,
                                                            float* __restrict__ gxi, int accXi, int HW, long long npix) {
    constexpr int C = LPP * 4, PPB = 256 / LPP;
    const int q = threadIdx.x % LPP;
    for (long long p = blockIdx.x * (long long)PPB + threadIdx.x / LPP; p < npix; p += (long long)gridDim.x * PPB) {
        const int n = (int)(p / HW);
        const f32x4 sv = *reinterpret_cast<const f32x4*>(s + n * C + q * 4);
        const f32x4 gmv = *reinterpret_cast<const f32x4*>(gm + n * C + q * 4);
        const f32x4 gi = *reinterpret_cast<const f32x4*>(gxs + p * 2 * C + q * 4);
        const f32x4 ge = *reinterpret_cast<const f32x4*>(gxs + p * 2 * C + C + q * 4);
        const f32x4 dv = *reinterpret_cast<const f32x4*>(dwe + p * C + q * 4);
        f32x4 o;
#pragma unroll
        for (int k = 0; k < 4; ++k) o[k] = (ge[k] * sv[k] + gmv[k] * invHW) * gelu_d(dv[k]);
        *reinterpret_cast<f32x4*>(gdwe + p * C + q * 4) = o;
        f32x4 xi = gi * sv;
        float* xo = gxi + p * C + q * 4;
        if (accXi) xi += *reinterpret_cast<const f32x4*>(xo);
        *reinterpret_cast<f32x4*>(xo) = xi;
    }
}

__global__ __launch_bounds__(256) void gelu_fwd_kernel(const f32x4* __restrict__ in, f32x4* __restrict__ out, long long n4) {
    for (long long i = blockIdx.x * 256ll + threadIdx.x; i < n4; i += (long long)gridDim.x * 256) {
        const f32x4 v = in[i];
        f32x4 o;
#pragma unroll
        for (int k = 0; k < 4; ++k) o[k] = gelu_f(v[k]);
        out[i] = o;
    }
}

__global__ __launch_bounds__(256) void gelu_bwd_kernel(const f32x4* __restrict__ g, const f32x4* __restrict__ in,
                                                      f32x4* __restrict__ out, long long n4) {
    for (long long i = blockIdx.x * 256ll + threadIdx.x; i < n4; i += (long long)gridDim.x * 256) {
        const f32x4 v = in[i], gv = g[i];
        f32x4 o;
#pragma unroll
        for (int k = 0; k < 4; ++k) o[k] = gv[k] * gelu_d(v[k]);
        out[i] = o;
    }
}

__global__ __launch_bounds__(256) void colsum_kernel(const float* __restrict__ g, int ldg, float* __restrict__ parts,
                                                    int C, long long npix) {
    __shared__ f32x4 sb[256];
    const int Q = C / 4, PPB = 256 / Q;
    const int q = threadIdx.x % Q;
    f32x4 acc = {0.f, 0.f, 0.f, 0.f};
    for (long long p = blockIdx.x * (long long)PPB + threadIdx.x / Q; p < npix; p += (long long)gridDim.x * PPB)
        acc += *reinterpret_cast<const f32x4*>(g + p * ldg + q * 4);
    sb[threadIdx.x] = acc;
    __syncthreads();
    if (threadIdx.x < Q) {
        f32x4 a = sb[threadIdx.x];
        for (int r = 1; r < PPB; ++r) a += sb[r * Q + threadIdx.x];
        *reinterpret_cast<f32x4*>(parts + (long long)blockIdx.x * C + threadIdx.x * 4) = a;
    }
}

__global__ __launch_bounds__(64) void fold_back_kernel(const float* __restrict__ W, const float* __restrict__ b,
                                                      const float* __restrict__ scale, const float* __restrict__ Gf,
                                                      const float* __restrict__ gbf, float* __restrict__ G,
                                                      float* __restrict__ gb, float* __restrict__ dscale, int K) {
    const int r = blockIdx.x;
    const float sc = scale[r];
    float a = 0.f;
    for (int k = threadIdx.x; k < K; k += 64) {
        const float gf = Gf[(long long)r * K + k];
        a += W[(long long)r * K + k] * gf;
        G[(long long)r * K + k] += sc * gf;
    }
#pragma unroll
    for (int o = 32; o > 0; o >>= 1) a += __shfl_xor(a, o, 64);
    if (threadIdx.x == 0) {
        dscale[r] += a + b[r] * gbf[r];
        gb[r] += sc * gbf[r];
    }
}

__global__ __launch_bounds__(256) void mul_vec_kernel(const float* a, const float* b, float* out, int n) {
    const int i = blockIdx.x * 256 + threadIdx.x;
    if (i < n) out[i] = a[i] * b[i];
}

int blocks_for(long long items, int per_block, int cap = 2048) {
    long long b = (items + per_block - 1) / per_block;
    return (int)(b < 1 ? 1 : (b > cap ? cap : b));
}

}

#define LPP_DISPATCH(C, CALL)                                                     \
    switch (C) {                                                                  \
        case 16: { constexpr int LPP = 4; CALL; break; }                          \
        case 32: { constexpr int LPP = 8; CALL; break; }                          \
        case 64: { constexpr int LPP = 16; CALL; break; }                         \
        case 128: { constexpr int LPP = 32; CALL; break; }                        \
        default: refid_set_error("egaca: unsupported channel count %d (16/32/64/128)", C); return 1; \
    }

extern "C" int refid_layernorm2d_fwd(const float* x, int ld_x, const float* w, const float* b, float* out,
                                     int ld_out, long long npix, int c, float eps, void* stream) {
    REFID_CHECK(x && w && b && out && npix > 0, "layernorm2d_fwd: bad arguments");
    hipStream_t st = (hipStream_t)stream;
    LPP_DISPATCH(c, hipLaunchKernelGGL(ln_fwd_kernel<LPP>, dim3(blocks_for(npix, 256 / LPP)), dim3(256), 0, st, x,
                                       ld_x, w, b, out, ld_out, npix, eps));
    REFID_LAUNCH_CHECK("layernorm2d_fwd");
    return 0;
}

extern "C" int refid_layernorm2d_bwd_parts(long long npix, int c) {
    if (c != 16 && c != 32 && c != 64 && c != 128) return -1;
    return blocks_for(npix, 256 / (c / 4), 512);
}

extern "C" int refid_layernorm2d_bwd(const float* g, int ld_g, const float* x, int ld_x, const float* w, float* gx,
                                     int ld_gx, const float* res, int ld_res, float* dw, float* db, float* parts,
                                     long long npix, int c, float eps, void* stream) {
    REFID_CHECK(g && x && w && gx && dw && db && parts && npix > 0, "layernorm2d_bwd: bad arguments");
    hipStream_t st = (hipStream_t)stream;
    const int nb = refid_layernorm2d_bwd_parts(npix, c);
    LPP_DISPATCH(c, hipLaunchKernelGGL(ln_bwd_kernel<LPP>, dim3(nb), dim3(256), 0, st,
                                       g, ld_g, x, ld_x, w, gx, ld_gx, res, ld_res, parts, npix, eps));
    REFID_LAUNCH_CHECK("layernorm2d_bwd");
    return rows_sum_issue(parts, nb, 2 * c, dw, c, db, st, "layernorm2d_bwd/sum");
}

extern "C" int refid_dwconv_pool_parts(int h, int wd, int c) {
    if (c != 16 && c != 32 && c != 64 && c != 128) return -1;
    return blocks_for((long long)h * wd, 256 / (c / 4), 64);
}

extern "C" int refid_dwconv3x3_gelu_fwd(const float* in, int ld_in, const float* w, const float* b, float* pre,
                                        float* act, float* pool, int n, int h, int wd, int c, void* stream) {
    REFID_CHECK(in && w && b && pre && act && n > 0 && h > 0 && wd > 0, "dwconv3x3_gelu_fwd: bad arguments");
    hipStream_t st = (hipStream_t)stream;
    LPP_DISPATCH(c, hipLaunchKernelGGL(dw_fwd_kernel<LPP>, dim3(refid_dwconv_pool_parts(h, wd, c), n),
                                       dim3(256), 0, st, in, ld_in, w, b, pre, act, pool, h, wd));
    REFID_LAUNCH_CHECK("dwconv3x3_gelu_fwd");
    return 0;
}

extern "C" int refid_dwconv3x3_bwd_parts(int h, int wd, int c) {
    if (c != 16 && c != 32 && c != 64 && c != 128) return -1;
    return blocks_for((long long)h * wd, 256 / (c / 4), 64);
}

extern "C" int refid_dwconv3x3_bwd(const float* gd, const float* in, int ld_in, const float* w, float* gin,
                                   float* dw, float* db, float* parts, int n, int h, int wd, int c, void* stream) {
    REFID_CHECK(gd && in && w && gin && dw && db && parts && n > 0, "dwconv3x3_bwd: bad arguments (parts is required)");
    hipStream_t st = (hipStream_t)stream;
    const int nb = refid_dwconv3x3_bwd_parts(h, wd, c);
    LPP_DISPATCH(c, hipLaunchKernelGGL(dw_bwd_kernel<LPP>, dim3(nb, n), dim3(256), 0, st, gd, in, ld_in, w, gin, parts, h, wd));
    REFID_LAUNCH_CHECK("dwconv3x3_bwd");
    return rows_sum_issue(parts, nb * n, c * 10, dw, c * 9, db, st, "dwconv3x3_bwd/sum");
}

extern "C" int refid_se_fwd(const float* pool, int n_parts, float inv_hw, const float* w1, const float* b1,
                            const float* w2, const float* b2, float* m, float* z1, float* s, int n, int c,
                            void* stream) {
    REFID_CHECK(pool && w1 && b1 && w2 && b2 && m && z1 && s && n > 0 && n_parts > 0 && c > 0 && c <= 256 && c % 2 == 0 && 256 % c == 0,
                "se_fwd: bad arguments (c=%d; must divide 256)", c);
    hipLaunchKernelGGL(se_fwd_kernel, dim3(n), dim3(256), 0, (hipStream_t)stream, pool, n_parts, inv_hw, w1, b1, w2,
                       b2, m, z1, s, c);
    REFID_LAUNCH_CHECK("se_fwd");
    return 0;
}

extern "C" int refid_se_bwd(const float* gs, const float* s, const float* z1, const float* m, const float* w1,
                            const float* w2, float* gm, float* dw1, float* db1, float* dw2, float* db2, float* scratch,
                            int n, int c, void* stream) {
    REFID_CHECK(gs && s && z1 && m && w1 && w2 && gm && dw1 && db1 && dw2 && db2 && scratch && n > 0 && c <= 256,
                "se_bwd: bad arguments");
    hipLaunchKernelGGL(se_bwd_kernel, dim3(n), dim3(256), 0, (hipStream_t)stream, gs, s, z1, m, w1, w2, gm, scratch, n, c);
    REFID_LAUNCH_CHECK("se_bwd");
    hipLaunchKernelGGL(se_bwd_params_kernel, dim3(cdiv(c * (c / 2), 256)), dim3(256), 0, (hipStream_t)stream, scratch, z1, m,
                       dw1, db1, dw2, db2, n, c);
    REFID_LAUNCH_CHECK("se_bwd/params");
    return 0;
}

extern "C" int refid_scale_cat(const float* xi, const float* xe, const float* s, float* out, int n, int hw, int c,
                               void* stream) {
    REFID_CHECK(xi && xe && s && out && n > 0 && hw > 0, "scale_cat: bad arguments");
    const long long npix = (long long)n * hw;
    hipStream_t st = (hipStream_t)stream;
    LPP_DISPATCH(c, hipLaunchKernelGGL(scale_cat_kernel<LPP>, dim3(blocks_for(npix, 256 / (2 * LPP))), dim3(256), 0,
                                       st, xi, xe, s, out, hw, npix));
    REFID_LAUNCH_CHECK("scale_cat");
    return 0;
}

extern "C" int refid_egaca_gs_reduce_parts(int hw, int c) {
    if (c != 16 && c != 32 && c != 64 && c != 128) return -1;
    return blocks_for(hw, 256 / (c / 4), 128);
}

extern "C" int refid_egaca_gs_reduce(const float* gxs, const float* xi, const float* xe, float* gs, float* parts, int n,
                                     int hw, int c, void* stream) {
    REFID_CHECK(gxs && xi && xe && gs && parts && n > 0 && hw > 0, "egaca_gs_reduce: bad arguments");
    hipStream_t st = (hipStream_t)stream;
    const int nb = refid_egaca_gs_reduce_parts(hw, c);
    LPP_DISPATCH(c, hipLaunchKernelGGL(gs_reduce_kernel<LPP>, dim3(nb, n), dim3(256), 0, st, gxs, xi, xe, parts, hw));
    REFID_LAUNCH_CHECK("egaca_gs_reduce");
    hipLaunchKernelGGL(gs_sum_kernel, dim3(n), dim3(256), 0, st, parts, nb, c, n * c, gs);
    REFID_LAUNCH_CHECK("egaca_gs_reduce/sum");
    return 0;
}

extern "C" int refid_egaca_bwd_elem(const float* gxs, const float* s, const float* gm, float inv_hw, const float* dwe,
                                    float* gdwe, float* gxi, int accumulate_xi, int n, int hw, int c, void* stream) {
    REFID_CHECK(gxs && s && gm && dwe && gdwe && gxi && n > 0 && hw > 0, "egaca_bwd_elem: bad arguments");
    const long long npix = (long long)n * hw;
    hipStream_t st = (hipStream_t)stream;
    LPP_DISPATCH(c, hipLaunchKernelGGL(egaca_bwd_elem_kernel<LPP>, dim3(blocks_for(npix, 256 / LPP)), dim3(256), 0, st,
                                       gxs, s, gm, inv_hw, dwe, gdwe, gxi, accumulate_xi, hw, npix));
    REFID_LAUNCH_CHECK("egaca_bwd_elem");
    return 0;
}

extern "C" int refid_gelu_fwd(const float* in, float* out, long long count, void* stream) {
    REFID_CHECK(in && out && count > 0 && count % 4 == 0, "gelu_fwd: bad arguments");
    hipLaunchKernelGGL(gelu_fwd_kernel, dim3(blocks_for(count / 4, 256)), dim3(256), 0, (hipStream_t)stream,
                       (const f32x4*)in, (f32x4*)out, count / 4);
    REFID_LAUNCH_CHECK("gelu_fwd");
    return 0;
}

extern "C" int refid_gelu_bwd(const float* g, const float* in, float* out, long long count, void* stream) {
    REFID_CHECK(g && in && out && count > 0 && count % 4 == 0, "gelu_bwd: bad arguments");
    hipLaunchKernelGGL(gelu_bwd_kernel, dim3(blocks_for(count / 4, 256)), dim3(256), 0, (hipStream_t)stream,
                       (const f32x4*)g, (const f32x4*)in, (f32x4*)out, count / 4);
    REFID_LAUNCH_CHECK("gelu_bwd");
    return 0;
}

extern "C" int refid_colsum_parts(long long npix, int c) {
    if (c < 4 || c > 1024 || c % 4 != 0 || 256 % (c / 4) != 0) return -1;
    return blocks_for(npix, 256 / (c / 4), 256);
}

extern "C" int refid_colsum(const float* g, int ld_g, float* db, float* parts, long long npix, int c, void* stream) {
    REFID_CHECK(g && db && parts && npix > 0 && c >= 4 && c <= 1024 && c % 4 == 0 && 256 % (c / 4) == 0,
                "colsum: bad arguments (c=%d; c/4 must divide 256)", c);
    const int nb = refid_colsum_parts(npix, c);
    hipLaunchKernelGGL(colsum_kernel, dim3(nb), dim3(256), 0, (hipStream_t)stream, g, ld_g, parts, c, npix);
    REFID_LAUNCH_CHECK("colsum");
    return rows_sum_issue(parts, nb, c, db, c, nullptr, (hipStream_t)stream, "colsum/sum");
}

extern "C" int refid_rows_sum_defer(int on) {
    rows_queue.clear();
    rows_defer = on != 0;
    return 0;
}

extern "C" int refid_rows_sum_flush(void* stream) {
    rows_defer = false;
    return rows_sum_flush((hipStream_t)stream);
}

extern "C" int refid_fold_back(const float* w, const float* b, const float* scale, const float* gw_folded,
                               const float* gb_folded, float* gw, float* gb, float* dscale, int rows, int k,
                               void* stream) {
    REFID_CHECK(w && b && scale && gw_folded && gb_folded && gw && gb && dscale && rows > 0 && k > 0,
                "fold_back: bad arguments");
    REFID_CHECK(gw_folded != gw && gb_folded != gb, "fold_back: the folded gradient must not alias the accumulated one");
    hipLaunchKernelGGL(fold_back_kernel, dim3(rows), dim3(64), 0, (hipStream_t)stream, w, b, scale, gw_folded, gb_folded,
                       gw, gb, dscale, k);
    REFID_LAUNCH_CHECK("fold_back");
    return 0;
}

extern "C" int refid_mul_vec(const float* a, const float* b, float* out, int n, void* stream) {
    REFID_CHECK(a && b && out && n > 0, "mul_vec: bad arguments");
    hipLaunchKernelGGL(mul_vec_kernel, dim3(cdiv(n, 256)), dim3(256), 0, (hipStream_t)stream, a, b, out, n);
    REFID_LAUNCH_CHECK("mul_vec");
    return 0;
}
```

### refid_amd/engine.py

```python
import os
from collections import OrderedDict

import torch

from . import ops
from ._lib import RefidHipError


def param_shapes(img_chn, ev_chn=2, out_chn=3, base=32, num_residual_blocks=2, num_block=1, num_encoders=3):
    b = base
    sh = OrderedDict()

    def conv(name, co, ci, k, bias=True):
        sh[name + ".weight"] = (co, ci, k, k)
        if bias:
            sh[name + ".bias"] = (co,)

    conv("head.conv2d", b, ev_chn, 5)
    enc_in = [b * 2 ** i for i in range(num_encoders)]
    enc_out = [b * 2 ** (i + 1) for i in range(num_encoders)]

    def evr(prefix, ci, co, fuse, atten):
        conv(prefix + ".conv.conv2d", co, ci, 3)
        if atten:
# ... 292 lines not shown
            sf_bn = ops.conv_bn(3, 3, 1, 0, co)
            sf_pad = -(-co // sf_bn) * sf_bn
            if not (fp16 and wp6 is not None):
                wps = _Packing("wps", "split", ops.pack_geo(ops.ROLE_FWD, co, ci, 3, 3, 8, sf_bn, planes))
            if need_dgrad and co % 8 == 0 and (not (fp16 and wd6 is not None) or (ci == 2 * co and co < WINO6_MIN_CO)):
                sd_bn = self.d_bn if self.d_algo != 1 else ops.conv_bn(3, 3, 1, 0, min(ci, 128))
                if ci == 2 * co:
                    sd_bn = ops.conv_bn(3, 3, 1, 0, co)
                sd_pad = -(-ci // sd_bn) * sd_bn
                wds = _Packing("wds", "split", ops.pack_geo(ops.ROLE_DGRAD, co, ci, 3, 3, 8, sd_bn, planes))
        if kind == "down" and ci % 8 == 0 and co % 8 == 0 and (terms or DOWN_SPLIT):
            self.split = terms = terms or DOWN_SPLIT
            planes = {1: 1, 3: 2, 6: 3, ops.TERMS_F16X3: 2}[terms]
            f16 = terms == ops.TERMS_F16X3
            if not bf16:
                sf_bn = ops.conv_bn(4, 4, 2, 0, co)
                sf_pad = -(-co // sf_bn) * sf_bn
                wps = _Packing("wps", ops.split_form(4, 4, f16), ops.pack_geo(ops.ROLE_FWD, co, ci, 4, 4, 8, sf_bn, planes))
            if need_dgrad:
                sd_bn = ops.conv_bn(4, 4, 2, 2, ci)
                sd_pad = -(-ci // sd_bn) * sd_bn
                wds = _Packing("wds", ops.split_form(4, 4, f16), ops.pack_geo(ops.ROLE_DOWN_DGRAD, co, ci, 4, 4, 8, sd_bn, planes))
        self.wp_lazy = wp.lazy = LAZY_FALLBACK_PACKS and wp6 is not None and (self.f_algo == 1 or fp16)
        self.wd_lazy = LAZY_FALLBACK_PACKS and wd6 is not None and (self.d_algo == 1 or fp16)
        if wd is not None:
            wd.lazy = self.wd_lazy
        self.packings = [p for p in (wp, wd, wp6, wd6, wps, wds) if p is not None]
        self._lazy = {p.attr: p for p in self.packings if p.lazy}
        self.wd = self.wp6 = self.wd6 = self.wps = self.wds = None
        for p in self.packings:
            setattr(self, p.attr, p.alloc(self.w.device))
        self.b_eff = self.b
        if self.scale is not None and self.has_bias:
            self.b_eff = torch.empty_like(self.b)
        kh, kw, st, md = f_geo
        self._f_split = self._f_wino6 = self._d_split = self._d_wino6 = self._d_plain = None
        if wps is not None:
            self._f_split = ("wps", dict(kh=kh, kw=kw, stride=st, pad=1, mode=0, cout_pad=sf_pad, algo=4, terms=self.split), True, False)
        if wp6 is not None and (self.split == 0 or fp16):
            self._f_wino6 = ("wp6", dict(kh=3, kw=3, stride=1, pad=1, mode=0, cout_pad=-(-self.f_rows // 64) * 64, algo=5,
                                     terms=f_terms), True, False)
        self._f_plain = ("wp", dict(kh=kh, kw=kw, stride=st, pad=self.pad, mode=md, cout_pad=self.f_pad, algo=self.f_algo),
                         self.f_algo != 3, True)
        if need_dgrad:
            kh, kw, st, md = d_geo
            if wds is not None:
                self._d_split = ("wds", dict(kh=kh, kw=kw, stride=st, pad=1, mode=md, cout_pad=sd_pad, algo=4, terms=self.split), True, False)
            if wd6 is not None and (self.split == 0 or fp16):
                self._d_wino6 = ("wd6", dict(kh=3, kw=3, stride=1, pad=1, mode=0, cout_pad=-(-self.d_rows // 64) * 64, algo=5,
                                         terms=d_terms), True, False)
            self._d_plain = ("wd", dict(kh=kh, kw=kw, stride=st, pad=d_padding, mode=md, cout_pad=self.d_pad, algo=self.d_algo),
                             self.d_algo != 3 or kind == "convT", self.d_algo == 3 and kind == "conv")
        self.wslab = None
        self.w_calls = 0
        self.w_last = None
        self.w_pend = []
        self.w_algo, self.w_bias = 0, True
        self.w_group = 1

    def plan_repack(self, plan):
        for p in self.packings:
            if not p.lazy:
                p.plan(self, plan)
        if self.scale is not None and self.has_bias:
            plan.add_mul_vec(self.b, self.scale, self.b_eff)

    def _packed(self, attr):
        p = self._lazy.get(attr)
        if p is not None and p.epoch != self.arena.pack_epoch:
            p.pack(self)
        return getattr(self, attr)

    def pack_fallbacks(self):
        for attr in self._lazy:
            self._packed(attr)

    def repack(self):
        for p in self.packings:
            p.pack(self)
        if self.scale is not None and self.has_bias:
            ops.mul_vec(self.b, self.scale, out=self.b_eff)

    def _fwd_route(self, n, ho, wo, a, b, pw):
        r = self._f_split
        if r is not None and (self.split > 1 or b is None) and a.shape[3] % 8 == 0 and pw is None and \
                (self.kind == "conv" or (b is None and _fills_gpu(n, ho, wo, self.co, 1))):
            return r
        r = self._f_wino6
        if r is not None and (b is None or a.shape[3] % 16 == 0):
            return r
        return self._f_plain

    def fwd(self, a, b=None, res=None, slope_pre=1.0, slope_post=1.0, out=None, pw=None, bias=True, plus=None):
        n, h, w, _ = a.shape
        bv = self.b_eff if bias else None
        if self.kind == "conv":
            ho, wo, oc = h, w, self.co
        elif self.kind == "down":
            ho, wo, oc = h // 2, w // 2, self.co
        else:
            ho, wo, oc = 2 * h, 2 * w, self.co
        if out is None:
            out = torch.empty((n, ho, wo, _pad4(oc)), dtype=torch.float32, device=a.device)
            if _pad4(oc) != oc:
                out.zero_()
                out = out[..., :oc]
        o2 = torch.empty_like(out) if plus is not None else None
        parts = ((a, b, res, out),)
        if n * a.stride(0) >= _LIM4 or n * out.stride(0) >= _LIM4 or (b is not None and n * b.stride(0) >= _LIM4):
            if pw is not None:
                raise RefidHipError(f"{self.name}: fused pointwise extras cannot be issued in sub-batches (tensor >= 2 GiB)")
            parts = _sub_batches(n, a, b, res, out)
        for a_i, b_i, res_i, out_i in parts:
            attr, geo, fused, takes_pw = self._fwd_route(a_i.shape[0], ho, wo, a_i, b_i, pw)
            fused = fused and plus is not None and len(parts) == 1
            extra = dict(add2=plus, out2=o2) if fused else {}
            if takes_pw:
                extra["pw"] = pw
            ops.conv2d(a_i, self._packed(attr), out_i, cout=self.f_rows, in_b=b_i, bias=bv, res=res_i, slope_pre=slope_pre,
                       slope_post=slope_post, **geo, **extra)
        if plus is None:
            return out
        if not fused:
            ops.add(out, plus, out=o2)
        return out, o2

    def can_fwd_from(self):
        return self.kind == "conv" and self.k == 1 and self.f_algo == 3 and not self.bf16

    def fwd_from(self, a, k_base):
        if not self.can_fwd_from() or k_base % self.f_kc or a.shape[3] % self.f_kc:
            raise RefidHipError(f"{self.name}: fwd_from needs the fp32 pointwise tile and chunk-aligned channel blocks")
        n, h, w, _ = a.shape
        out = torch.empty((n, h, w, self.co), dtype=torch.float32, device=a.device)
        ops.conv2d(a, self.wp[(k_base // self.f_kc) * self.f_pad * self.f_kc:], out, kh=1, kw=1, stride=1, pad=0, mode=0,
                   cout=self.f_rows, cout_pad=self.f_pad, bias=self.b_eff, algo=3)
        return out

    def _dgrad_route(self, g, cnt):
        r = self._d_wino6
        if self.fp16 and r is not None and cnt >= WINO6_MIN_CO:
            return r
        r = self._d_split
        if r is not None and (self.kind == "conv" or _fills_gpu(g.shape[0], g.shape[1], g.shape[2], cnt, 4)):
            return r
        r = self._d_wino6
        if r is not None and cnt >= WINO6_MIN_CO:
            return r
        return self._d_plain

    def gelu_mask_ok(self, g, rows=None):
        return self.wd is not None and self._dgrad_route(g, rows[1] if rows is not None else self.d_rows)[3]

    def dgrad(self, g, rows=None, res=None, mask=None, slope_mask=1.0, out=None, plus=None, gelu_mask=False):
        if self.wd is None:
            raise RefidHipError(f"{self.name}: dgrad weights were not requested")
        base, cnt = rows if rows is not None else (0, self.d_rows)
        n, h, w, _ = g.shape
        if self.kind == "conv":
            ho, wo = h, w
        elif self.kind == "down":
            ho, wo = 2 * h, 2 * w
        else:
            ho, wo = h // 2, w // 2
        if out is None:
            out = torch.empty((n, ho, wo, cnt), dtype=torch.float32, device=g.device)
        o2 = torch.empty_like(out) if plus is not None else None
        parts = ((g, res, mask, out),)
        if n * g.stride(0) >= _LIM4 or n * out.stride(0) >= _LIM4:
            parts = _sub_batches(n, g, res, mask, out)
        for g_i, res_i, mask_i, out_i in parts:
            attr, geo, fused, gelu_ok = self._dgrad_route(g_i, cnt)
            if gelu_mask and not gelu_ok:
                raise RefidHipError(f"{self.name}: gelu_mask needs the fp32 pointwise input-gradient tile (d_algo {self.d_algo}); "
                                    f"apply ops.gelu_bwd separately")
            fused = fused and plus is not None and len(parts) == 1
            extra = dict(add2=plus, out2=o2) if fused else (dict(mask_mode=1) if gelu_mask else {})
            if self.d_role == ops.ROLE_CONVT_DGRAD_PW and g_i.stride(2) != g_i.shape[3]:
                g_i = g_i.contiguous()
            ops.conv2d(g_i, self._packed(attr), out_i, cout=cnt, co_base=base, res=res_i, mask=mask_i, slope_mask=slope_mask,
                       **geo, **extra)
        if plus is None:
            return out
        if not fused:
            ops.add(out, plus, out=o2)
        return out, o2

    def wgrad(self, g, a, b=None, bias=True, i_base=0):
        if i_base:
            if self.kind != "conv" or b is not None or bias:
                raise RefidHipError(f"{self.name}: a column-block weight gradient is one source, no bias, stride-1 conv")
            ops.conv2d_wgrad(g, a, self.gw, kh=self.k, kw=self.k, stride=1, pad=self.pad, i_base=i_base, i_total=self.ci,
                             algo=0, phase=0)
            return
        if self.kind == "convT":
            if self.has_bias and bias:
                ops.colsum(g, self.gb)
            g, a, b, bias = a, g, None, False
            if CONVT_PWS and PWS_WGRAD and not self.bf16 and a.stride(2) == a.shape[3] and g.shape[2] % 32 == 0 and \
                    self._pws_plan_ok(self.ci, 2 * self.co, 2 * self.co, 4 * self.co):
                return self._wgrad_issue(g, a, None, False, 8)
            return self._wgrad_issue(g, a, None, False, 0)
        algo = 1 if (USE_WINOGRAD and self.kind == "conv" and self.k == 3 and self.co >= WGRAD_WINO_MIN_CO and self.ci >= 32) else 0
        if algo == 1 and b is not None and a.shape[3] % 32 != 0:
            algo = 0
        if algo == 1 and WGRAD_F4 and min(g.shape[1], g.shape[2]) >= WGRAD_F4_MIN_HW and g.shape[3] % 4 == 0 and \
                a.shape[3] % 4 == 0 and (b is None or b.shape[3] % 4 == 0):
            algo = 5
        if self.kind == "down" and WGRAD_DOWN_F4 and USE_WINOGRAD and self.co >= 32 and self.ci >= 32 and a.shape[3] % 32 == 0 and \
                (b is None or b.shape[3] % 32 == 0) and a.shape[1] % 2 == 0 and a.shape[2] % 2 == 0 and \
                min(g.shape[1], g.shape[2]) >= WGRAD_F4_MIN_HW and g.shape[3] % 4 == 0:
            algo = 7
        if self.bf16 and self.kind == "conv" and self.k == 3 and self.co > 32 and self.ci > 32:
            algo = 2
        return self._wgrad_issue(g, a, b, bias, algo)

    def _wgrad_issue(self, g, a, b, bias, algo):
        gb = self.gb if bias else None
        pws = PWS_WGRAD and self.kind == "conv" and self.k == 1 and algo == 0 and self._pws_ok(a, b)
        if self.w_group > 1 and ((self.kind == "conv" and self.k == 3 and self.ci > 4) or self.kind in ("down", "convT") or pws):
            if self.w_pend and ((self.w_pend[0][2] is None) != (b is None) or self.w_algo != algo or self.w_bias != bias):
                self._launch_group()
            self.w_pend.append((g, a, b))
            self.w_algo, self.w_bias = algo, bias
            if len(self.w_pend) >= self.w_group:
                self._launch_group()
            return
        self._slab_layout(algo)
        self.wslab = ops.conv2d_wgrad(g, a, self.gw, in_b=b, db=gb, algo=algo, phase=1 if self.w_calls == 0 else 2,
                                      slabs=self.wslab, **self._wg_geo())
        self.w_calls += 1
        self.w_last = (g, a, b, algo)

    def _wg_geo(self):
        if self.kind == "convT":
            return dict(kh=2, kw=2, stride=2, pad=0, i_total=self.co)
        return dict(kh=self.k, kw=self.k, stride=self.stride, pad=self.pad, i_total=self.ci)

    def _pws_ok(self, a, b):
        return self._pws_plan_ok(self.co, a.shape[3], b.shape[3] if b is not None else 0, self.ci)

    @staticmethod
    def _pws_plan_ok(co, ca, cb, ci):
        if co < 64 or co % 32 or ca % 32 or cb % 32 or ci % 32:
            return False
        two = cb or ci > ca
        wi = 4 if ci >= 128 else (2 if ci >= 64 else 1)
        while two and wi > 1 and ca % (32 * wi):
            wi //= 2
        return not (co >= 128 and wi == 1 and two and ca % 64)

    def _slab_layout(self, algo):
        if self.w_calls and self.w_last is not None and self.w_last[3] != algo:
            g, a, b, old = self.w_last
            ops.conv2d_wgrad(g, a, self.gw, in_b=b, db=self.gb if self.kind != "convT" else None, algo=old, phase=3,
                             slabs=self.wslab, **self._wg_geo())
            self.w_calls = 0

    def _launch_group(self):
        (g, a, b), more = self.w_pend[0], self.w_pend[1:]
        self._slab_layout(self.w_algo)
        self.wslab = ops.conv2d_wgrad(g, a, self.gw, in_b=b, db=self.gb if self.w_bias else None, algo=self.w_algo,
                                      phase=1 if self.w_calls == 0 else 2, slabs=self.wslab, more=more, **self._wg_geo())
        self.w_calls += 1
        self.w_last = (g, a, b, self.w_algo)
        self.w_pend = []

    def finish_wgrad(self, batched=False):
        if self.w_calls == 0 and not self.w_pend:
            return
        if self.w_pend:
            self._launch_group()
        g, a, b, algo = self.w_last
        ops.conv2d_wgrad(g, a, self.gw, in_b=b, db=self.gb if self.kind != "convT" else None, algo=algo,
                         phase=4 if batched else 3, slabs=self.wslab, **self._wg_geo())
        self.w_calls = 0
        self.w_last = None


def finish_wgrads(op_list):
    batched = FINISH_BATCH
    try:
        for o in op_list:
            o.finish_wgrad(batched)
    finally:
        try:
            if batched:
                ops.wgrad_finish_flush()
        finally:
            ops.rows_sum_flush()


class _Trunk:

    def __init__(self, arena, prefix, compute_dtype="fp32"):
        self.c0 = ConvOp(arena, prefix + ".0", compute_dtype=compute_dtype)
        self.blocks = []
        k = 0
        while f"{prefix}.2.{k}.conv1.weight" in arena.shapes:
            self.blocks.append((ConvOp(arena, f"{prefix}.2.{k}.conv1", compute_dtype=compute_dtype), ConvOp(arena, f"{prefix}.2.{k}.conv2", compute_dtype=compute_dtype)))
            k += 1
        self.c1, self.c2 = self.blocks[0]
        self.C = self.c0.co

    def ops(self):
        return [self.c0] + [c for blk in self.blocks for c in blk]


class _Egaca:
    def __init__(self, arena, a, compute_dtype="fp32"):
        self.a = a
        P, G = arena.p, arena.g
        self.conv1 = ConvOp(arena, a + ".conv1", compute_dtype=compute_dtype)
        self.conv1_e = ConvOp(arena, a + ".conv1_e", compute_dtype=compute_dtype)
        self.conv3 = ConvOp(arena, a + ".conv3", scale_name=a + ".beta", compute_dtype=compute_dtype)
        self.conv4 = ConvOp(arena, a + ".conv4", compute_dtype=compute_dtype)
        self.conv5 = ConvOp(arena, a + ".conv5", scale_name=a + ".gamma", compute_dtype=compute_dtype)
        self.side = ConvOp(arena, a + ".conv_y_side", compute_dtype=compute_dtype)
        self.c = self.conv1.ci
        self.wp_cat = self.b_cat = None
        c5, sd = self.conv5, self.side
        if LINEAR_SPLIT and c5.f_algo == 3 and sd.f_algo == 3 and not c5.bf16 and (c5.f_pad, c5.f_kc, c5.f_bn) == (sd.f_pad, sd.f_kc, sd.f_bn) \
                and c5.ci % 8 == 0 and c5.has_bias and sd.has_bias:
            n5 = c5.wp.numel()
            self.wp_cat = torch.empty(n5 + sd.wp.numel(), dtype=torch.float32, device=c5.wp.device)
            c5.wp, sd.wp = self.wp_cat[:n5], self.wp_cat[n5:]
            self.b_cat = torch.empty_like(sd.b)
        self.names = {n: (P(f"{a}.{n}"), G(f"{a}.{n}")) for n in (
            "norm1.weight", "norm1.bias", "norm1_e.weight", "norm1_e.bias", "norm2.weight", "norm2.bias",
            "conv2.weight", "conv2.bias", "conv2_e.weight", "conv2_e.bias",
# ... 43 lines not shown
            raise ValueError(f"compute_dtype must be 'fp32', 'bf16x3', 'bf16' or 'fp16', got {compute_dtype!r}")
        self.compute_dtype = cd = compute_dtype
        self.img_chn, self.ev_chn, self.out_chn, self.base = img_chn, ev_chn, out_chn, base
        self.nres = num_residual_blocks
        self.device = torch.device(device)
        self.shapes = param_shapes(img_chn, ev_chn, out_chn, base, num_residual_blocks, num_block, NL)
        self.arena = A = ParamArena(self.shapes, self.device)
        self.head_ev = ConvOp(A, "head.conv2d", need_dgrad=False, compute_dtype=cd)
        self.head_img = ConvOp(A, "head_img.conv2d", need_dgrad=False, compute_dtype=cd)
        self.enc_b = [_EvrLevel(A, f"encoders_backward.{i}", i, False, dead_down=(i == NL - 1), compute_dtype=cd) for i in range(NL)]
        self.enc_f = [_EvrLevel(A, f"encoders_forward.{i}", i, True, compute_dtype=cd) for i in range(NL)]
        self.img = []
        for i in range(NL):
            p = f"img_encoders.{i}"
            self.img.append(dict(identity=ConvOp(A, p + ".identity", compute_dtype=cd), conv_1=ConvOp(A, p + ".conv_1", compute_dtype=cd),
                                 conv_2=ConvOp(A, p + ".conv_2", compute_dtype=cd),
                                 down=ConvOp(A, p + ".down", kind="down", compute_dtype=cd)))
        self.res = [(ConvOp(A, f"resblocks.{i}.conv1", compute_dtype=cd), ConvOp(A, f"resblocks.{i}.conv2", compute_dtype=cd))
                    for i in range(self.nres)]
        self.dec = []
        for j in range(NL):
            p = f"decoders.{j}"
            self.dec.append(dict(t2=ConvOp(A, p + ".transposed_conv2d", kind="convT", compute_dtype=cd),
                                 trunk=_Trunk(A, p + ".forward_trunk.main", compute_dtype=cd)))
        self.pred = ConvOp(A, "pred.conv2d", compute_dtype=cd)
        self.all_ops = [self.head_ev, self.head_img, self.pred]
        for lv in self.enc_b + self.enc_f:
            self.all_ops += lv.ops()
        for e in self.img:
            self.all_ops += list(e.values())
        for c1, c2 in self.res:
            self.all_ops += [c1, c2]
        for d in self.dec:
            self.all_ops += [d["t2"]] + d["trunk"].ops()
        self.early_ops = [self.pred]
        for lv in self.enc_f:
            self.early_ops += lv.ops()
        for c1, c2 in self.res:
            self.early_ops += [c1, c2]
        for d in self.dec:
            self.early_ops += [d["t2"]] + d["trunk"].ops()
        self.packed_version = -1
        self.param_version = 0
        self._pack_plan = None
        self.ctx = None
        self._bind_fold_scratch()
        img_ops = {id(o) for e in self.img for o in e.values()} | {id(self.head_img), id(self.head_ev)}
        self.recurrent_ops = [o for o in self.all_ops if id(o) not in img_ops]

    def _set_wgrad_groups(self, T, pixels=0):
        n = max(1, min(WGRAD_GROUP, T))
        n = wgrad_group_cap(n, pixels, self.device)
        for o in self.recurrent_ops:
            o.w_group = n

    def _bind_fold_scratch(self):
        self.folded_ops = [o for o in self.all_ops if o.scale is not None]
        n = sum((o.gw_arena.numel() + 3) // 4 * 4 + (o.gb_arena.numel() + 3) // 4 * 4 for o in self.folded_ops)
        self.fold_scratch = torch.zeros(max(n, 4), dtype=torch.float32, device=self.device)
        off = 0
        for o in self.folded_ops:
            for attr, ref in (("gw", o.gw_arena), ("gb", o.gb_arena)):
                k = ref.numel()
                setattr(o, attr, self.fold_scratch[off:off + k].view(ref.shape))
                off += (k + 3) // 4 * 4

    def mark_params_changed(self):
        self.param_version += 1

    def repack(self):
        if self.packed_version == self.param_version:
            return
        if PACK_BATCH:
            if self._pack_plan is None:
                plan = ops.PackPlan(self.all_ops[0].w.device)
                for o in self.all_ops:
                    o.plan_repack(plan)
                self._pack_plan = plan.build()
            self._pack_plan.run()
            self.arena.pack_epoch += 1
        else:
            for o in self.all_ops:
                o.repack()
        for lv in self.enc_b + self.enc_f:
            if lv.att is not None and lv.att.wp_cat is not None:
                ops.add(lv.att.conv5.b_eff, lv.att.side.b, out=lv.att.b_cat)
        self.packed_version = self.param_version

    def _egaca_img_path(self, A, img):
        n, h, w, c = img.shape
        if EGACA_FUSED and 32 < c <= 64 and c % 8 == 0 and A.conv1.f_algo == 3:
            ln_i = torch.empty_like(img)
            c1i = A.conv1.fwd(img, pw=dict(ln_gamma=A.p("norm1.weight"), ln_beta=A.p("norm1.bias"), ln_out=ln_i))
        else:
            ln_i = ops.layernorm2d_fwd(img, A.p("norm1.weight"), A.p("norm1.bias"))
            c1i = A.conv1.fwd(ln_i)
        dwi, xi = ops.dwconv3x3_gelu_fwd(c1i, A.p("conv2.weight"), A.p("conv2.bias"))
        return dict(ln_i=ln_i, c1i=c1i, dwi=dwi, xi=xi, gxi=None)

    def _egaca_fwd(self, A, ev, img, ip, st):
        n, h, w, c = ev.shape
        if EGACA_FUSED and (h * w) % 128 == 0 and 32 < c <= 64 and c % 8 == 0 and A.conv1_e.f_algo == 3 and \
                ops.dwconv_pool_parts(h, w, c) <= 256:
            return self._egaca_fwd_fused(A, ev, img, ip, st)
        ln_e = ops.layernorm2d_fwd(ev, A.p("norm1_e.weight"), A.p("norm1_e.bias"))
        c1e = A.conv1_e.fwd(ln_e)
        dwe, xe, pool = ops.dwconv3x3_gelu_fwd(c1e, A.p("conv2_e.weight"), A.p("conv2_e.bias"), want_pool=True)
        m, z1, s = ops.se_fwd(pool, 1.0 / (h * w), A.p("se_1.1.weight"), A.p("se_1.1.bias"),
                              A.p("se_1.3.weight"), A.p("se_1.3.bias"))
        xs = ops.scale_cat(ip["xi"], xe, s)
        evimg = ops.add(ev, img)
        y = A.conv3.fwd(xs, res=evimg)
        ln2 = ops.layernorm2d_fwd(y, A.p("norm2.weight"), A.p("norm2.bias"))
        c4 = A.conv4.fwd(ln2)
        f4 = ops.gelu_fwd(c4)
        side = A.side.fwd(y)
        out = A.conv5.fwd(f4, res=side)
        if st is not None:
            st["eg"] = dict(ev=ev, ln_e=ln_e, c1e=c1e, dwe=dwe, xe=xe, m=m, z1=z1, s=s, xs=xs, y=y, ln2=ln2,
                            c4=c4, f4=f4)
        return out

    def _egaca_fwd_fused(self, A, ev, img, ip, st):
        n, h, w, c = ev.shape
        save = st is not None
        dev = ev.device
        new = lambda *shape: torch.empty(shape, dtype=torch.float32, device=dev)
        ln_e = new(n, h, w, c) if save else None
        c1e = A.conv1_e.fwd(ev, pw=dict(ln_gamma=A.p("norm1_e.weight"), ln_beta=A.p("norm1_e.bias"), ln_out=ln_e))
        dwe, xe, pool = ops.dwconv3x3_gelu_fwd(c1e, A.p("conv2_e.weight"), A.p("conv2_e.bias"), want_pool=True)
        m = z1 = s = xs = None
        if save:
            m, z1, s, xs = new(n, c), new(n, c // 2), new(n, c), new(n, h, w, 2 * c)
        y = A.conv3.fwd(ip["xi"], xe, res=ev,
                        pw=dict(pool=pool, hw=h * w, se_w1=A.p("se_1.1.weight"), se_b1=A.p("se_1.1.bias"),
                                se_w2=A.p("se_1.3.weight"), se_b2=A.p("se_1.3.bias"), se_m=m, se_z1=z1, se_s=s,
                                xs_out=xs, res2=img))
        ln2 = new(n, h, w, c) if save else None
        f4 = new(n, h, w, A.conv4.co)
        c4 = A.conv4.fwd(y, pw=dict(ln_gamma=A.p("norm2.weight"), ln_beta=A.p("norm2.bias"), ln_out=ln2, out2=f4))
        if A.wp_cat is not None:
            out = new(n, h, w, A.conv5.co)
            ops.conv2d(f4, A.wp_cat, out, kh=1, kw=1, stride=1, pad=0, mode=0, cout=A.conv5.co, cout_pad=A.conv5.f_pad, in_b=y,
                       bias=A.b_cat, algo=3)
        else:
            side = A.side.fwd(y)
            out = A.conv5.fwd(f4, res=side)
        if save:
            st["eg"] = dict(ev=ev, ln_e=ln_e, c1e=c1e, dwe=dwe, xe=xe, m=m, z1=z1, s=s, xs=xs, y=y, ln2=ln2, c4=c4, f4=f4)
        return out

    def _egaca_bwd(self, A, g_u, img_grad, ip, st, gy_keep=None):
        e = st["eg"]
        A.conv5.wgrad(g_u, e["f4"])
        if LINEAR_SPLIT and A.conv5.gelu_mask_ok(g_u):
            g_c4 = A.conv5.dgrad(g_u, mask=e["c4"], gelu_mask=True)
        else:
            g_f4 = A.conv5.dgrad(g_u)
            g_c4 = ops.gelu_bwd(g_f4, e["c4"], out=g_f4)
        A.conv4.wgrad(g_c4, e["ln2"])
        g_ln2 = A.conv4.dgrad(g_c4)
        A.side.wgrad(g_u, e["y"])
        g_y = A.side.dgrad(g_u)
        ops.layernorm2d_bwd(g_ln2, e["y"], A.p("norm2.weight"), g_y, A.g("norm2.weight"), A.g("norm2.bias"),
                            accumulate=True)
        A.conv3.wgrad(g_y, e["xs"])
        g_xs = A.conv3.dgrad(g_y)
        gs = ops.egaca_gs_reduce(g_xs, ip["xi"], e["xe"])
        gm = ops.se_bwd(gs, e["s"], e["z1"], e["m"], A.p("se_1.1.weight"), A.p("se_1.3.weight"),
                        A.g("se_1.1.weight"), A.g("se_1.1.bias"), A.g("se_1.3.weight"), A.g("se_1.3.bias"))
        first = ip["gxi"] is None
        if first:
            ip["gxi"] = torch.empty_like(ip["xi"])
        g_dwe = ops.egaca_bwd_elem(g_xs, e["s"], gm, e["dwe"], ip["gxi"], accumulate_xi=not first)
        g_c1e = ops.dwconv3x3_bwd(g_dwe, e["c1e"], A.p("conv2_e.weight"), A.g("conv2_e.weight"), A.g("conv2_e.bias"))
        A.conv1_e.wgrad(g_c1e, e["ln_e"])
        g_lne = A.conv1_e.dgrad(g_c1e)
        if gy_keep is not None:
            gy_keep.append(g_y)
        else:
            ops.add(img_grad, g_y, out=img_grad)
        g_ev = ops.layernorm2d_bwd(g_lne, e["ev"], A.p("norm1_e.weight"), torch.empty_like(g_y),
                                   A.g("norm1_e.weight"), A.g("norm1_e.bias"), res=g_y)
        return g_ev

    def _egaca_img_bwd(self, A, img, img_grad, ip):
        if ip["gxi"] is None:
            return
        g_dwi = ops.gelu_bwd(ip["gxi"], ip["dwi"])
        g_c1i = ops.dwconv3x3_bwd(g_dwi, ip["c1i"], A.p("conv2.weight"), A.g("conv2.weight"), A.g("conv2.bias"))
        A.conv1.wgrad(g_c1i, ip["ln_i"])
        g_lni = A.conv1.dgrad(g_c1i)
        ops.layernorm2d_bwd(g_lni, img, A.p("norm1.weight"), img_grad, A.g("norm1.weight"), A.g("norm1.bias"),
                            accumulate=True)

    def _egaca_fold_back(self, A):
        for conv, nm in ((A.conv3, "beta"), (A.conv5, "gamma")):
            ops.fold_back(conv.w, conv.b, conv.scale, conv.gw, conv.gb, conv.gw_arena, conv.gb_arena,
                          A.g(nm).view(-1))

    @staticmethod
    def _trunk_fwd(T, u, h, st, plus=None):
        v = T.c0.fwd(u, h, slope_pre=0.1)
        xs, rs, x = [], [], v
        for k, (c1, c2) in enumerate(T.blocks):
            r = c1.fwd(x, slope_pre=0.0)
            xs.append(x); rs.append(r)
            x = c2.fwd(r, res=x, plus=plus if k == len(T.blocks) - 1 else None)
        s, sp = x if plus is not None else (x, None)
        if st is not None:
            st.update(u=u, h=h, v=v, r=rs[0], xs=xs, rs=rs, s=s)
        return s if plus is None else (s, sp)

    @staticmethod
    def _trunk_bwd(T, g_s, st, mask_u=None, slope_u=1.0):
        u, h, v = st["u"], st["h"], st["v"]
        C = T.C
        g = g_s
        for k in range(len(T.blocks) - 1, -1, -1):
            c1, c2 = T.blocks[k]
            x, r = st["xs"][k], st["rs"][k]
            c2.wgrad(g, r)
            g_r = c2.dgrad(g, mask=r, slope_mask=0.0)
            c1.wgrad(g_r, x)
            g = c1.dgrad(g_r, res=g, mask=v, slope_mask=0.1) if k == 0 else c1.dgrad(g_r, res=g)
        g_v = g
        T.c0.wgrad(g_v, u, h)
        g_u = T.c0.dgrad(g_v, rows=(0, C), mask=mask_u, slope_mask=slope_u)
        g_h = T.c0.dgrad(g_v, rows=(C, C)) if h is not None else None
        return g_u, g_h

    def _evr_fwd(self, L, a, xb, h_prev, Sb, ip, st, plus=None):
        i = L.level
        if i == 0:
            src = a
            u = L.conv.fwd(a, slope_pre=0.04)
        elif i >= 2:
            if L.q_const is not None:
                src = a
                u = L.conv.fwd(a, res=L.q_const, slope_post=0.04, bias=False)
            else:
                src = ops.add(a, xb[i - 1])
                u = L.conv.fwd(src, slope_pre=0.04)
        else:
            src = a
            u = self._egaca_fwd(L.att, a, xb[0], ip, st)
        s = self._trunk_fwd(L.trunk, u, h_prev, st)
        f = s
        if L.fuse is not None:
            if L.p_fuse is not None:
                f = L.fuse.fwd(s, res=L.p_fuse, slope_post=0.2, bias=False)
            else:
                f = L.fuse.fwd(s, Sb, slope_pre=0.2)
        o = op = None
        if L.down is not None:
            o = L.down.fwd(f, plus=plus)
            if plus is not None:
                o, op = o
        if st is not None:
            st.update(src=src, f=f, Sb=Sb)
        return (o, s) if plus is None else (o, s, op)

    def forward(self, x, event, save=True):
        if x.dim() == 5:
            x = x.reshape(x.shape[0], x.shape[1] * x.shape[2], x.shape[3], x.shape[4])
        if x.dtype != torch.float32 or event.dtype != torch.float32 or not x.is_cuda or not event.is_cuda:
            raise RefidHipError("forward: float32 CUDA tensors required")
        B, T, nb, H, W = event.shape
        NL = self.NL
        if H % (1 << NL) or W % (1 << NL):
            raise RuntimeError(f"H and W must be multiples of {1 << NL}, got {H}x{W}")
        if x.shape != (B, self.img_chn, H, W) or nb != self.ev_chn:
            raise RuntimeError(f"unexpected input shapes x={tuple(x.shape)} event={tuple(event.shape)}")
        self.repack()
        dev = x.device
        x = x.contiguous()
        event = event.contiguous()
        x_in = ops.nchw_to_nhwc(x, _pad4(self.img_chn))
        ev_in = ops.nchw_to_nhwc_tb(event, _pad4(self.ev_chn))
        head = self.head_img.fwd(x_in, slope_pre=0.2)
        e_all = self.head_ev.fwd(ev_in, slope_pre=0.2)
        xb, img_saved = [], []
        g = head
        for i in range(NL):
            E = self.img[i]
            c1 = E["conv_1"].fwd(g, slope_pre=0.2)
            c2 = E["conv_2"].fwd(c1, slope_pre=0.2)
            sm = E["identity"].fwd(g, res=c2)
            o = E["down"].fwd(sm)
            img_saved.append((g, c1, c2, sm))
            xb.append(o)
            g = o
        ip_b = self._egaca_img_path(self.enc_b[1].att, xb[0])
        ip_f = self._egaca_img_path(self.enc_f[1].att, xb[0])

        lin = LINEAR_SPLIT
        for L in self.enc_b[2:] + self.enc_f[2:]:
            L.q_const = L.conv.fwd(xb[L.level - 1]) if lin else None
        for L in self.enc_f:
            L.p_fuse = None
        q_pred = None
        if lin:
            q_pred = torch.zeros((B, H, W, _pad4(self.out_chn)), dtype=torch.float32, device=dev)
            self.pred.fwd(head, out=q_pred[..., :self.out_chn])

        main = torch.cuda.current_stream()
        pipe = use_pipeline(B, H, W)
        lvs = [main] + ([LV_STREAMS[k].get(dev) for k in range(NL - 1)] if pipe else [main] * (NL - 1))
        for s_ in lvs[1:]:
            if s_ is not main:
                s_.wait_stream(main)

        def level(L, i, cur, h_prev, Sb_i, ip, st, plus=None):
            if lvs[i] is main and i == 0:
                return self._evr_fwd(L, cur, xb, h_prev, Sb_i, ip, st, plus)
            if lvs[i] is not lvs[i - 1]:
                lvs[i].wait_stream(lvs[i - 1])
                cur.record_stream(lvs[i])
            with torch.cuda.stream(lvs[i]):
                return self._evr_fwd(L, cur, xb, h_prev, Sb_i, ip, st, plus)

        hb = [None] * NL
        steps_b = []
        for t in range(T - 1, -1, -1):
            cur = e_all[t * B:(t + 1) * B]
            sts = []
            for i in range(NL):
                st = {} if save else None
                cur, hb[i] = level(self.enc_b[i], i, cur, hb[i], None, ip_b, st)
                sts.append(st)
            steps_b.append((t, sts))
        Sb = hb
        if lin:
            for i, L in enumerate(self.enc_f):
                with torch.cuda.stream(lvs[i]):
                    if L.fuse.can_fwd_from() and L.C % L.fuse.f_kc == 0 and _pad4(L.fuse.co) == L.fuse.co:
# ... 283 lines not shown
```

### refid_amd/ops.py

```python
import collections
import ctypes as C
import os

import torch

from . import _lib
from ._lib import ConvDesc, WgradDesc, check, lib

ROLE_FWD, ROLE_DGRAD, ROLE_CONVT, ROLE_CONVT_DGRAD, ROLE_DOWN_DGRAD, ROLE_WINO_FWD, ROLE_WINO_DGRAD, ROLE_CONVT_DGRAD_PW = range(8)


WINO_SPLIT = {"0": 0, "s": 1}.get(os.environ.get("REFID_SPLITK", os.environ.get("REFID_WINO_SPLITK", "auto"))[:1], 2)

WINO_TILE = int(os.environ.get("REFID_WINO_TILE", "0"))

PROFILE = None


def _stream():
    return C.c_void_p(torch.cuda.current_stream().cuda_stream)


_REQUIRE_CUDA = True


def _nhwc(t, name):
    if t is None:
        return None, 0
    if t.dtype != torch.float32 or (_REQUIRE_CUDA and not t.is_cuda):
        raise _lib.RefidHipError(f"{name}: expected a CUDA float32 tensor, got {t.dtype} on {t.device}")
    if t.dim() != 4:
        raise _lib.RefidHipError(f"{name}: expected NHWC 4-D tensor, got shape {tuple(t.shape)}")
    n, h, w, c = t.shape
    ld = t.stride(2)
    ok = t.stride(3) == 1 and ld % 4 == 0 and ld >= c
    ok = ok and (h == 1 or t.stride(1) == w * ld) and (n == 1 or t.stride(0) == h * w * ld)
    if not ok or t.data_ptr() % 16 != 0:
        raise _lib.RefidHipError(f"{name}: not a dense-pixel NHWC view (shape {tuple(t.shape)}, "
                                 f"strides {t.stride()}, ptr%16={t.data_ptr() % 16})")
    return t.data_ptr(), ld


def conv_kc(kh, kw, stride, mode=0):
    return lib().refid_conv_kc(kh, kw, stride, mode)


def conv_bn(kh, kw, stride, mode, cout):
    return lib().refid_conv_bn(kh, kw, stride, mode, cout)


_Form = collections.namedtuple("_Form", "kind planes dtype size entry")
_FORMS = {
    "f32": _Form(0, 0, torch.float32, "refid_packed_weight_floats", "refid_pack_conv_weights"),
    "bf16": _Form(0, 1, torch.bfloat16, "refid_packed_weight_floats", "refid_pack_conv_weights_bf16"),
    "split": _Form(1, None, torch.bfloat16, "refid_packed_weight_split_bytes", "refid_pack_conv_weights_split"),
    "split1x1": _Form(2, None, torch.bfloat16, "refid_packed_weight_split_bytes", "refid_pack_conv_weights_split"),
    "split_f16": _Form(6, 2, torch.bfloat16, "refid_packed_weight_split_f16_bytes", "refid_pack_conv_weights_split_f16"),
    "wino6": _Form(3, 3, torch.bfloat16, "refid_packed_weight_wino6_bytes", "refid_pack_conv_weights_wino6"),
    "wino3h": _Form(5, 2, torch.bfloat16, "refid_packed_weight_wino3h_bytes", "refid_pack_conv_weights_wino3h"),
    "wino1h": _Form(5, 1, torch.float16, "refid_packed_weight_wino1h_bytes", "refid_pack_conv_weights_wino1h"),
}


def pack_geo(role, o, i, kh=3, kw=3, kc=16, bn=64, planes=0):
    return dict(role=role, o=o, i=i, kh=kh, kw=kw, kc=kc, bn=bn, planes=planes)


def split_form(kh, kw, f16=False):
    return "split_f16" if f16 else ("split1x1" if kh == 1 and kw == 1 else "split")


def wino6_form(f16=False, terms=None):
    if terms is None:
        terms = 3 if f16 else 0
    if terms not in (0, 6, 3, 1):
        raise _lib.RefidHipError(f"Winograd packing: terms must be 0 / 6 (three bf16 planes), 3 (two fp16 planes) or 1 (one fp16 "
                                 f"plane), got {terms}")
    return {0: "wino6", 6: "wino6", 3: "wino3h", 1: "wino1h"}[terms]


def pack_elems(form, geo):
    f = _FORMS[form]
    n = getattr(lib(), f.size)(*(geo[k] for k in _lib.PACK_GEO[f.size]))
    return n if f.size.endswith("floats") else n // 2


def pack_bytes(form, geo):
    return pack_elems(form, geo) * _FORMS[form].dtype.itemsize


def pack_alloc(form, geo, device):
    return torch.empty(pack_elems(form, geo), dtype=_FORMS[form].dtype, device=device)


def pack_form(form, w, geo, out=None, oscale=None, what="pack_form"):
    f = _FORMS[form]
    n = pack_elems(form, geo)
    if n == 0:
        raise _lib.RefidHipError(f"{what}: bad geometry")
    if not w.is_contiguous():
        raise _lib.RefidHipError(f"{what}: weight must be contiguous")
    if out is None:
        out = torch.empty(n, dtype=f.dtype, device=w.device)
    elif out.numel() * out.element_size() != n * f.dtype.itemsize:
        raise _lib.RefidHipError(f"{what}: out has the wrong size")
    elif not out.is_contiguous():
        raise _lib.RefidHipError(f"{what}: out must be contiguous")
    name, ptrs = f.entry, [w.data_ptr(), None if oscale is None else oscale.data_ptr(), out.data_ptr()]
    if form == "f32":
        name, ptrs = (name, ptrs[::2]) if oscale is None else (name + "_scaled", ptrs)
    check(getattr(lib(), name)(*ptrs, *(geo[k] for k in _lib.PACK_GEO[name]), _stream()), name)
    return out


def packed_weight_floats(role, bn, kc, kh, kw, o, i):
    return pack_elems("f32", pack_geo(role, o, i, kh, kw, kc, bn))


def pack_conv_weights(w, role, bn, kc, kh, kw, o, i, out=None, oscale=None):
    return pack_form("f32", w, pack_geo(role, o, i, kh, kw, kc, bn), out, oscale, "pack_conv_weights")


def pack_conv_weights_bf16(w, role, bn, kc, kh, kw, o, i, out=None, oscale=None):
    return pack_form("bf16", w, pack_geo(role, o, i, kh, kw, kc, bn), out, oscale, "pack_conv_weights_bf16")


TERMS_F16X3 = 19


def packed_weight_split_bytes(role, bn, kh, kw, o, i, planes, f16=False):
    return pack_bytes(split_form(kh, kw, f16), pack_geo(role, o, i, kh, kw, 8, bn, planes))


def pack_conv_weights_split(w, role, bn, kh, kw, o, i, planes=3, out=None, oscale=None, f16=False):
    return pack_form(split_form(kh, kw, f16), w, pack_geo(role, o, i, kh, kw, 8, bn, planes), out, oscale, "pack_conv_weights_split")


def packed_weight_wino6_bytes(role, o, i, f16=False, terms=None):
    return pack_bytes(wino6_form(f16, terms), pack_geo(role, o, i))


def pack_conv_weights_wino6(w, role, o, i, out=None, oscale=None, f16=False, terms=None):
    return pack_form(wino6_form(f16, terms), w, pack_geo(role, o, i), out, oscale, "pack_conv_weights_wino6")


def _pw_extras(pw, out):
    x = _lib.PwExtras()
    if pw.get("ln_gamma") is not None:
        x.ln_gamma, x.ln_beta, x.ln_eps = _c(pw["ln_gamma"], "ln_gamma"), _c(pw["ln_beta"], "ln_beta"), pw.get("ln_eps", 1e-6)
        if pw.get("ln_out") is not None:
            x.ln_out, x.ld_ln_out = _nhwc(pw["ln_out"], "ln_out")
    if pw.get("pool") is not None:
        pool = pw["pool"]
        x.pool, x.pool_parts, x.se_c = _c(pool, "pool"), pool.shape[1], pool.shape[2]
        x.hw = pw["hw"]
        x.inv_hw = 1.0 / pw["hw"]
        x.se_w1, x.se_b1, x.se_w2, x.se_b2 = (_c(pw[k], k) for k in ("se_w1", "se_b1", "se_w2", "se_b2"))
        if pw.get("se_s") is not None:
            x.se_m, x.se_z1, x.se_s = _c(pw["se_m"], "se_m"), _c(pw["se_z1"], "se_z1"), _c(pw["se_s"], "se_s")
        if pw.get("xs_out") is not None:
            x.xs_out, x.ld_xs_out = _nhwc(pw["xs_out"], "xs_out")
    if pw.get("res2") is not None:
        if pw["res2"].shape != out.shape:
            raise _lib.RefidHipError("conv2d: res2 shape differs from the output's")
        x.res2, x.ld_res2 = _nhwc(pw["res2"], "res2")
    if pw.get("out2") is not None:
        if pw["out2"].shape != out.shape:
            raise _lib.RefidHipError("conv2d: out2 shape differs from the output's")
        x.out2, x.ld_out2 = _nhwc(pw["out2"], "out2")
    return x


def conv2d(in_a, w_packed, out, *, kh, kw, stride=1, pad=0, mode=0, cout, cout_pad, co_base=0,
           in_b=None, bias=None, res=None, mask=None, slope_pre=1.0, slope_post=1.0, slope_mask=1.0, algo=0, pw=None,
           terms=0, add2=None, out2=None, mask_mode=0):
    if DESC_CACHE and pw is None and PROFILE is None:
        return _conv2d_cached(in_a, w_packed, out, kh, kw, stride, pad, mode, cout, cout_pad, co_base, in_b, bias, res, mask,
                              slope_pre, slope_post, slope_mask, algo, terms, add2, out2, mask_mode)
    d = ConvDesc()
    d.mfma_terms = terms
    if pw is not None:
        if algo != 3:
            raise _lib.RefidHipError("conv2d: pw fusions need the pointwise tile (algo 3)")
        pwx = _pw_extras(pw, out)
        d.pw = C.pointer(pwx)
    d.in_a, d.ld_a = _nhwc(in_a, "in_a")
    d.c_a = in_a.shape[3]
    if in_b is not None:
        d.in_b, d.ld_b = _nhwc(in_b, "in_b")
        d.c_b = in_b.shape[3]
        if in_b.shape[:3] != in_a.shape[:3]:
            raise _lib.RefidHipError("conv2d: in_a / in_b pixel grids differ")
    if algo == 5 and terms == 1:
        chunk = 16 * cout_pad * 16 * 2
        have = w_packed.numel() * w_packed.element_size()
        if w_packed.dtype != torch.float16 or have < 64 + -(-(d.c_a + d.c_b) // 16) * chunk or (have - 64) % chunk:
            raise _lib.RefidHipError(f"conv2d: algo 5 with terms=1 reads the one-plane fp16 packing (a float16 tensor from "
                                     f"pack_conv_weights_wino6 with terms=1: 64 + chunks x {chunk} bytes), got {have} bytes of "
                                     f"{w_packed.dtype}")
    d.w_packed = w_packed.data_ptr()
    d.bias = bias.data_ptr() if bias is not None else None
    d.out, d.ld_out = _nhwc(out, "out")
    d.res, d.ld_res = _nhwc(res, "res")
    d.mask, d.ld_mask = _nhwc(mask, "mask")
    if out2 is not None:
        if add2 is None or add2.shape != out.shape or out2.shape != out.shape:
            raise _lib.RefidHipError("conv2d: out2 needs add2, both of the output's shape")
        d.add2, d.ld_add2 = _nhwc(add2, "add2")
        d.out2, d.ld_out2 = _nhwc(out2, "out2")
    d.n, d.h, d.w = in_a.shape[0], in_a.shape[1], in_a.shape[2]
    if mode == 0:
        d.ho, d.wo = out.shape[1], out.shape[2]
        chan_ok = out.shape[3] == cout
    else:
        d.ho, d.wo = d.h, d.w
        if out.shape[1] != 2 * d.h or out.shape[2] != 2 * d.w:
            raise _lib.RefidHipError("conv2d: mode 1/2 output must be (2h, 2w)")
        chan_ok = out.shape[3] == (cout // 4 if mode == 1 else cout)
    if not chan_ok or out.shape[0] != d.n:
        raise _lib.RefidHipError(f"conv2d: output shape {tuple(out.shape)} inconsistent with cout={cout} mode={mode}")
    for t, nm in ((res, "res"), (mask, "mask")):
        if t is not None and t.shape != out.shape:
            raise _lib.RefidHipError(f"conv2d: {nm} shape {tuple(t.shape)} != out shape {tuple(out.shape)}")
    d.cout, d.cout_pad, d.co_base = cout, cout_pad, co_base
    d.kh, d.kw, d.stride, d.pad, d.mode = kh, kw, stride, pad, mode
    d.slope_pre, d.slope_post, d.slope_mask = slope_pre, slope_post, slope_mask
    d.mask_mode = mask_mode
    d.algo = algo
    d.wino_tile = WINO_TILE
    if WINO_SPLIT and algo in (0, 1, 2, 4, 5):
        d.split_k = WINO_SPLIT
        need = lib().refid_conv_workspace_bytes(C.byref(d))
        if need:
            ws = _workspace(need, in_a.device, "conv")
            d.ws, d.ws_bytes = ws.data_ptr(), ws.numel() * 4
    if PROFILE is None:
        check(lib().refid_conv2d(C.byref(d), _stream()), "refid_conv2d")
        return out
    e0, e1 = torch.cuda.Event(enable_timing=True), torch.cuda.Event(enable_timing=True)
    e0.record()
    check(lib().refid_conv2d(C.byref(d), _stream()), "refid_conv2d")
    e1.record()
    taps = {0: kh * kw, 1: 1, 2: 16}[mode]
    flops = 2.0 * d.n * d.ho * d.wo * cout * (d.c_a + d.c_b) * taps
    name = "conv_igemm_kernel<" + lib().refid_conv_tile_name(kh, kw, stride, mode, cout).decode() + \
        (", true> [bf16 operands]" if algo == 2 else ">")
    if algo == 1:
        name = "conv_wino_kernel<1, 2>" if cout <= 32 else "conv_wino_kernel<2, 1>"
    if algo == 5:
        name = "conv_wino6_kernel<2>" if cout > 32 else "conv_wino6_kernel<1>"
        if terms == 3:
            name = name[:-1] + ", true>"
        if terms == 1:
            name = name[:-1] + ", true, fp16x1>"
    if algo == 4:
        name = "conv_split_kernel<%s>" % ("3, fp16" if terms == TERMS_F16X3 else (terms or 6))
    if algo == 3:
        name = "conv_pw_kernel<1, 8>" if cout <= 32 else ("conv_pw_kernel<2, 4, six>" if terms == 6 else "conv_pw_kernel<2, 4>")
    opix = d.n * out.shape[1] * out.shape[2]
    nbytes = 4.0 * (d.n * d.h * d.w * (d.c_a + d.c_b) + opix * out.shape[3] * (1 + (res is not None) + (mask is not None))
                    + cout * (d.c_a + d.c_b) * taps)
    if out2 is not None:
        nbytes += 8.0 * opix * out.shape[3]
    if pw is not None:
        for k in ("ln_out", "xs_out", "out2", "res2"):
            if pw.get(k) is not None:
                nbytes += 4.0 * pw[k].numel()
    PROFILE.append((name, flops, e0, e1,
                    (d.n, d.h, d.w, d.c_a, d.c_b, cout, int(res is not None), int(mask is not None), int(bias is not None)),
                    nbytes))
    return out


DESC_CACHE = os.environ.get("REFID_DESC_CACHE", "0") == "1"
_DESC_CACHE = {}
_DESC_PTRS = ("in_a", "in_b", "w_packed", "bias", "out", "res", "mask", "add2", "out2")


def _sig(t):
    return None if t is None else (t.shape, t.stride())


def _conv2d_cached(in_a, w_packed, out, kh, kw, stride, pad, mode, cout, cout_pad, co_base, in_b, bias, res, mask,
                   slope_pre, slope_post, slope_mask, algo, terms, add2, out2, mask_mode):
    global lib, DESC_CACHE
    key = (kh, kw, stride, pad, mode, cout, cout_pad, co_base, slope_pre, slope_post, slope_mask, algo, terms, mask_mode,
           WINO_TILE, WINO_SPLIT, _sig(in_a), _sig(in_b), _sig(out), _sig(res), _sig(mask), _sig(add2), _sig(out2),
           bias is not None, in_a.dtype, out.dtype, in_a.device)
    ent = _DESC_CACHE.get(key)
    if ent is None:
        real, seen = lib(), []

        class _Recorder:
            def __getattr__(self, name):
                if name == "refid_conv2d":
                    def launch(dref, st):
                        seen.append(ConvDesc.from_buffer_copy(C.string_at(C.addressof(dref._obj), C.sizeof(ConvDesc))))
                        return real.refid_conv2d(dref, st)
                    return launch
                return getattr(real, name)

        keep_lib, keep_flag = lib, DESC_CACHE
        rec = _Recorder()
        lib, DESC_CACHE = (lambda: rec), False
        try:
            conv2d(in_a, w_packed, out, kh=kh, kw=kw, stride=stride, pad=pad, mode=mode, cout=cout, cout_pad=cout_pad,
                   co_base=co_base, in_b=in_b, bias=bias, res=res, mask=mask, slope_pre=slope_pre, slope_post=slope_post,
                   slope_mask=slope_mask, algo=algo, terms=terms, add2=add2, out2=out2, mask_mode=mask_mode)
        finally:
            lib, DESC_CACHE = keep_lib, keep_flag
        _DESC_CACHE[key] = (seen[0], int(seen[0].ws_bytes))
        return out
    d, ws_bytes = ConvDesc.from_buffer_copy(ent[0]), ent[1]
    if _REQUIRE_CUDA and not (in_a.is_cuda and out.is_cuda):
        raise _lib.RefidHipError("conv2d: expected CUDA tensors")
    ptrs = (in_a.data_ptr(), None if in_b is None else in_b.data_ptr(), w_packed.data_ptr(),
            None if bias is None else bias.data_ptr(), out.data_ptr(), None if res is None else res.data_ptr(),
            None if mask is None else mask.data_ptr(),
            None if (add2 is None or out2 is None) else add2.data_ptr(),
            None if out2 is None else out2.data_ptr())
    for nm, p in zip(_DESC_PTRS, ptrs):
        if p is not None and p % 16 != 0 and nm not in ("w_packed", "bias"):
# ... 184 lines not shown


def sum_n(tensors, out=None):
    ts = list(tensors)
    if not ts:
        raise _lib.RefidHipError("sum_n: no inputs")
    if out is None:
        out = torch.empty_like(ts[0])
    for t in ts + [out]:
        if not t.is_contiguous() or t.shape != ts[0].shape or t.dtype != torch.float32:
            raise _lib.RefidHipError("sum_n: contiguous same-shape float32 tensors required")
    while True:
        part, ts = ts[:SUM_MAX], ts[SUM_MAX:]
        ptrs = (C.c_void_p * len(part))(*[t.data_ptr() for t in part])
        check(lib().refid_sum_n(ptrs, len(part), out.data_ptr(), out.numel(), _stream()), "refid_sum_n")
        if not ts:
            return out
        ts = [out] + ts


def act_bwd(g, y, slope, out=None, accumulate=False):
    if out is None:
        out = torch.empty_like(g)
        accumulate = False
    if not (g.is_contiguous() and y.is_contiguous() and out.is_contiguous()) or g.shape != y.shape:
        raise _lib.RefidHipError("act_bwd: contiguous same-shape tensors required")
    check(lib().refid_act_bwd(g.data_ptr(), y.data_ptr(), out.data_ptr(), slope, int(accumulate), g.numel(), _stream()),
          "refid_act_bwd")
    return out


def _c(t, name):
    if t.dtype != torch.float32 or not t.is_cuda or not t.is_contiguous():
        raise _lib.RefidHipError(f"{name}: contiguous CUDA float32 tensor required")
    return t.data_ptr()


def layernorm2d_fwd(x, w, b, out=None, eps=1e-6):
    px, ld = _nhwc(x, "x")
    if out is None:
        out = torch.empty(x.shape, dtype=torch.float32, device=x.device)
    po, ldo = _nhwc(out, "out")
    npix = x.shape[0] * x.shape[1] * x.shape[2]
    check(lib().refid_layernorm2d_fwd(px, ld, _c(w, "w"), _c(b, "b"), po, ldo, npix, x.shape[3], eps, _stream()),
          "refid_layernorm2d_fwd")
    return out


def layernorm2d_bwd(g, x, w, gx, dw, db, accumulate=False, res=None, eps=1e-6):
    pg, ldg = _nhwc(g, "g")
    px, ldx = _nhwc(x, "x")
    pgx, ldgx = _nhwc(gx, "gx")
    if accumulate and res is None:
        res = gx
    pr, ldr = _nhwc(res, "res") if res is not None else (None, 0)
    npix = x.shape[0] * x.shape[1] * x.shape[2]
    c = x.shape[3]
    nb = lib().refid_layernorm2d_bwd_parts(npix, c)
    if nb <= 0:
        raise _lib.RefidHipError(f"layernorm2d_bwd: unsupported channel count {c}")
    parts = torch.empty((nb, 2 * c), dtype=torch.float32, device=x.device)
    check(lib().refid_layernorm2d_bwd(pg, ldg, px, ldx, _c(w, "w"), pgx, ldgx, pr, ldr, _c(dw, "dw"),
                                      _c(db, "db"), parts.data_ptr(), npix, c, eps, _stream()), "refid_layernorm2d_bwd")
    _keep_rows(parts)
    return gx


def dwconv_pool_parts(h, w, c):
    return lib().refid_dwconv_pool_parts(h, w, c)


def dwconv3x3_gelu_fwd(x, w, b, want_pool=False):
    px, ld = _nhwc(x, "x")
    n, h, wd, c = x.shape
    pre = torch.empty((n, h, wd, c), dtype=torch.float32, device=x.device)
    act = torch.empty_like(pre)
    pool = None
    if want_pool:
        parts = lib().refid_dwconv_pool_parts(h, wd, c)
        if parts <= 0:
            raise _lib.RefidHipError(f"dwconv3x3: unsupported channel count {c}")
        pool = torch.empty((n, parts, c), dtype=torch.float32, device=x.device)
    check(lib().refid_dwconv3x3_gelu_fwd(px, ld, _c(w, "w"), _c(b, "b"), pre.data_ptr(), act.data_ptr(),
                                         pool.data_ptr() if pool is not None else None, n, h, wd, c, _stream()),
          "refid_dwconv3x3_gelu_fwd")
    return (pre, act, pool) if want_pool else (pre, act)


def dwconv3x3_bwd(gd, x, w, dw, db):
    px, ld = _nhwc(x, "x")
    n, h, wd, c = x.shape
    gin = torch.empty((n, h, wd, c), dtype=torch.float32, device=x.device)
    nparts = lib().refid_dwconv3x3_bwd_parts(h, wd, c)
    if nparts <= 0:
        raise _lib.RefidHipError(f"dwconv3x3_bwd: unsupported channel count {c}")
    parts = torch.empty((n * nparts, 10 * c), dtype=torch.float32, device=x.device)
    check(lib().refid_dwconv3x3_bwd(_c(gd, "gd"), px, ld, _c(w, "w"), gin.data_ptr(), _c(dw, "dw"), _c(db, "db"),
                                    parts.data_ptr(), n, h, wd, c, _stream()), "refid_dwconv3x3_bwd")
    _keep_rows(parts)
    return gin


def se_fwd(pool, inv_hw, w1, b1, w2, b2):
    if pool.dim() == 2:
        pool = pool.unsqueeze(1)
    n, parts, c = pool.shape
    m = torch.empty((n, c), dtype=torch.float32, device=pool.device)
    z1 = torch.empty((n, c // 2), dtype=torch.float32, device=pool.device)
    s = torch.empty_like(m)
    check(lib().refid_se_fwd(_c(pool, "pool"), parts, inv_hw, _c(w1, "w1"), _c(b1, "b1"), _c(w2, "w2"), _c(b2, "b2"),
                             m.data_ptr(), z1.data_ptr(), s.data_ptr(), n, c, _stream()), "refid_se_fwd")
    return m, z1, s


def se_bwd(gs, s, z1, m, w1, w2, dw1, db1, dw2, db2):
    n, c = gs.shape
    gm = torch.empty_like(gs)
    scratch = torch.empty((n, c + c // 2), dtype=torch.float32, device=gs.device)
    check(lib().refid_se_bwd(_c(gs, "gs"), _c(s, "s"), _c(z1, "z1"), _c(m, "m"), _c(w1, "w1"), _c(w2, "w2"),
                             gm.data_ptr(), _c(dw1, "dw1"), _c(db1, "db1"), _c(dw2, "dw2"), _c(db2, "db2"),
                             scratch.data_ptr(), n, c, _stream()), "refid_se_bwd")
    return gm


def scale_cat(xi, xe, s):
    n, h, w, c = xi.shape
    out = torch.empty((n, h, w, 2 * c), dtype=torch.float32, device=xi.device)
    check(lib().refid_scale_cat(_c(xi, "xi"), _c(xe, "xe"), _c(s, "s"), out.data_ptr(), n, h * w, c, _stream()),
          "refid_scale_cat")
    return out


def egaca_gs_reduce(gxs, xi, xe):
    n, h, w, c = xi.shape
    gs = torch.empty((n, c), dtype=torch.float32, device=xi.device)
    nb = lib().refid_egaca_gs_reduce_parts(h * w, c)
    if nb <= 0:
        raise _lib.RefidHipError(f"egaca_gs_reduce: unsupported channel count {c}")
    parts = torch.empty((n, nb, c), dtype=torch.float32, device=xi.device)
    check(lib().refid_egaca_gs_reduce(_c(gxs, "gxs"), _c(xi, "xi"), _c(xe, "xe"), gs.data_ptr(), parts.data_ptr(), n,
                                      h * w, c, _stream()), "refid_egaca_gs_reduce")
    return gs


def egaca_bwd_elem(gxs, s, gm, dwe, gxi, accumulate_xi):
    n, h, w, c = dwe.shape
    gdwe = torch.empty_like(dwe)
    check(lib().refid_egaca_bwd_elem(_c(gxs, "gxs"), _c(s, "s"), _c(gm, "gm"), 1.0 / (h * w), _c(dwe, "dwe"),
                                     gdwe.data_ptr(), _c(gxi, "gxi"), int(accumulate_xi), n, h * w, c, _stream()),
          "refid_egaca_bwd_elem")
    return gdwe


def gelu_fwd(x):
    out = torch.empty_like(x)
    check(lib().refid_gelu_fwd(_c(x, "x"), out.data_ptr(), x.numel(), _stream()), "refid_gelu_fwd")
    return out


def gelu_bwd(g, x, out=None):
    if out is None:
        out = torch.empty_like(x)
    check(lib().refid_gelu_bwd(_c(g, "g"), _c(x, "x"), out.data_ptr(), x.numel(), _stream()), "refid_gelu_bwd")
    return out


def colsum(g, db):
    pg, ld = _nhwc(g, "g")
    npix = g.shape[0] * g.shape[1] * g.shape[2]
    nb = lib().refid_colsum_parts(npix, g.shape[3])
    if nb <= 0:
        raise _lib.RefidHipError(f"colsum: unsupported channel count {g.shape[3]}")
    parts = torch.empty((nb, g.shape[3]), dtype=torch.float32, device=g.device)
    check(lib().refid_colsum(pg, ld, _c(db, "db"), parts.data_ptr(), npix, g.shape[3], _stream()), "refid_colsum")
    _keep_rows(parts)


class PackPlan:

    def __init__(self, device):
        self.device = device
        self.esz = lib().refid_pack_entry_bytes()
        self.items = []
        self.keep = []
        self.table = None
        self.nblocks = 0

    def _add(self, kind, w, oscale, dst, role=0, o=0, i=0, kh=1, kw=1, kc=8, bn=32, planes=0):
        if self.table is not None:
            raise _lib.RefidHipError("PackPlan: already built")
        for t in (w, oscale, dst):
            if t is not None and not t.is_contiguous():
                raise _lib.RefidHipError("PackPlan: tensors must be contiguous")
        self.items.append((kind, w, oscale, dst, role, o, i, kh, kw, kc, bn, planes))
        self.keep += [w, oscale, dst]

    def add_form(self, form, w, geo, out, oscale=None):
        f = _FORMS[form]
        self._add(f.kind, w, oscale, out, **dict(geo, planes=geo["planes"] if f.planes is None else f.planes))

    def add_pack(self, w, role, bn, kc, kh, kw, o, i, out, oscale=None, bf16=False):
        self.add_form("bf16" if bf16 else "f32", w, pack_geo(role, o, i, kh, kw, kc, bn), out, oscale)

    def add_split(self, w, role, bn, kh, kw, o, i, planes, out, oscale=None, f16=False):
        self.add_form(split_form(kh, kw, f16), w, pack_geo(role, o, i, kh, kw, 8, bn, planes), out, oscale)

    def add_wino6(self, w, role, o, i, out, oscale=None, f16=False, terms=None):
        self.add_form(wino6_form(f16, terms), w, pack_geo(role, o, i), out, oscale)

    def add_mul_vec(self, a, b, out):
        self._add(4, a, b, out, o=a.numel())

    def build(self):
        L = lib()
        buf = (C.c_char * (self.esz * len(self.items)))()
        blk = 0
        for n, (kind, w, oscale, dst, role, o, i, kh, kw, kc, bn, planes) in enumerate(self.items):
            nb = L.refid_pack_entry_fill(C.addressof(buf) + n * self.esz, kind, w.data_ptr(),
                                         oscale.data_ptr() if oscale is not None else None, dst.data_ptr(), role, o, i, kh, kw,
                                         kc, bn, planes, blk)
            if nb <= 0:
                raise _lib.RefidHipError(f"refid_pack_entry_fill (record {n}, kind {kind}): " + L.refid_last_error().decode())
            blk += nb
        if L.refid_pack_table_check(C.addressof(buf), len(self.items)) != blk:
            raise _lib.RefidHipError("refid_pack_table_check: " + L.refid_last_error().decode())
        self.nblocks = blk
        self.table = torch.frombuffer(bytearray(bytes(buf)), dtype=torch.uint8).to(self.device)
        return self

    def run(self):
        if any(it[0] in (5, 6) for it in self.items):
            check(lib().refid_pack_batch_prepass(self.table.data_ptr(), len(self.items), _stream()), "refid_pack_batch_prepass")
        check(lib().refid_pack_batch(self.table.data_ptr(), len(self.items), self.nblocks, _stream()), "refid_pack_batch")


def mul_vec(a, b, out=None):
    if out is None:
        out = torch.empty_like(a)
    check(lib().refid_mul_vec(_c(a, "a"), _c(b, "b"), out.data_ptr(), a.numel(), _stream()), "refid_mul_vec")
    return out


def fold_back(w, b, scale, gw_folded, gb_folded, gw, gb, dscale):
    rows = scale.numel()
    k = w.numel() // rows
    check(lib().refid_fold_back(_c(w, "w"), _c(b, "b"), _c(scale, "scale"), _c(gw_folded, "gw_folded"),
                                _c(gb_folded, "gb_folded"), _c(gw, "gw"), _c(gb, "gb"), _c(dscale, "dscale"), rows, k,
                                _stream()), "refid_fold_back")


def charbonnier(pred, gt, grad=None, eps=1e-12, grad_scale=None):
    n = pred.numel()
    buf = torch.empty(1 + lib().refid_charbonnier_parts(n), dtype=torch.float64, device=pred.device)
    if grad_scale is None:
        grad_scale = 1.0 / n
    check(lib().refid_charbonnier(_c(pred, "pred"), _c(gt, "gt"), grad.data_ptr() if grad is not None else None,
                                  buf.data_ptr(), buf[1:].data_ptr(), n, eps, grad_scale, _stream()), "refid_charbonnier")
    return buf[:1]


def psnr_loss(pred, gt, grad=None, weight=1.0, want_sq=False):
    nb = pred.shape[0]
    per = pred.numel() // nb
    buf = torch.empty(nb + 1 + lib().refid_psnr_loss_parts(nb, per), dtype=torch.float64, device=pred.device)
    check(lib().refid_psnr_loss(_c(pred, "pred"), _c(gt, "gt"), grad.data_ptr() if grad is not None else None,
                                buf.data_ptr(), buf[nb:].data_ptr(), buf[nb + 1:].data_ptr(), nb, per, weight, _stream()),
          "refid_psnr_loss")
    return (buf[nb:nb + 1], buf[:nb]) if want_sq else buf[nb:nb + 1]


SQNORM_WORDS = 2049


def grad_sqnorm(flat_g, out=None):
    if out is None:
        out = torch.empty(SQNORM_WORDS, dtype=torch.float64, device=flat_g.device)
    elif out.numel() < SQNORM_WORDS:
        raise _lib.RefidHipError("grad_sqnorm: out needs SQNORM_WORDS doubles")
    check(lib().refid_grad_sqnorm(_c(flat_g, "g"), out.data_ptr(), flat_g.numel(), _stream()), "refid_grad_sqnorm")
    return out


def clip_adamw(p, g, m, v, sqnorm, *, max_norm, lr, betas, eps, weight_decay, step, grad_scale=1.0):
    check(lib().refid_clip_adamw(_c(p, "p"), _c(g, "g"), _c(m, "m"), _c(v, "v"),
                                 sqnorm.data_ptr() if sqnorm is not None else None, max_norm, grad_scale, lr,
                                 betas[0], betas[1], eps, weight_decay, step, p.numel(), _stream()),
          "refid_clip_adamw")


def clip_adamw_dev(p, g, m, v, sqnorm, hyper, *, max_norm, betas, eps, weight_decay, grad_scale=1.0):
    check(lib().refid_clip_adamw_dev(_c(p, "p"), _c(g, "g"), _c(m, "m"), _c(v, "v"),
                                     sqnorm.data_ptr() if sqnorm is not None else None, max_norm, grad_scale,
                                     _c(hyper, "hyper"), betas[0], betas[1], eps, weight_decay, p.numel(), _stream()),
          "refid_clip_adamw_dev")


def hin_lrelu_fwd(x, gamma, beta, slope=0.2, eps=1e-5, out=None):
    px, ld = _nhwc(x, "x")
    n, h, w, c = x.shape
    ch = 0 if gamma is None else gamma.numel()
    if out is None:
        out = torch.empty((n, h, w, c), dtype=torch.float32, device=x.device)
    po, ldo = _nhwc(out, "out")
    stats = parts = None
    if ch:
        stats = torch.empty((n, 2, ch), dtype=torch.float32, device=x.device)
# ... 245 lines not shown
```

Baseline: 517.7.

## Fuse EGACA backward: LayerNorm bwd into pointwise dgrad, gate+dwconv bwd, gs+SE bwd

Adds a LayerNorm-backward epilogue to the 64-channel pointwise dgrad tile, so the conv input gradient is turned straight into the LN input gradient plus per-block dw/db partials. It also adds a fused gate-elementwise plus depthwise-3x3 backward kernel and a kernel that does the gs reduction and the SE backward together. The goal is to cut intermediate tensor round-trips and kernel launches in the EGACA backward. In exchange there are extra shuffle reductions in the epilogue, more register and shared-memory pressure, and unfused fallbacks that stay in place for unsupported shapes.

```diff
diff --git a/include/refid_hip.h b/include/refid_hip.h
--- a/include/refid_hip.h
+++ b/include/refid_hip.h
@@ -24,6 +24,8 @@
     float* xs_out; int ld_xs_out;
     const float* res2; int ld_res2;
     float* out2; int ld_out2;
+    const float* ln_bwd_x; int ld_ln_bwd_x; const float* ln_bwd_gamma; const float* ln_bwd_res; int ld_ln_bwd_res;
+    float* ln_bwd_parts; float* ln_bwd_dw; float* ln_bwd_db;
 } refid_pw_extras;
 
 typedef struct refid_conv_desc {
@@ -160,6 +162,13 @@
                           int c, void* stream);
 int refid_egaca_bwd_elem(const float* gxs, const float* s, const float* gm, float inv_hw, const float* dwe,
                          float* gdwe, float* gxi, int accumulate_xi, int n, int hw, int c, void* stream);
+int refid_egaca_gs_se_bwd(const float* gxs, const float* xi, const float* xe, float* gs, float* parts, const float* s,
+                          const float* z1, const float* m, const float* w1, const float* w2, float* gm, float* dw1,
+                          float* db1, float* dw2, float* db2, float* scratch, int n, int hw, int c, void* stream);
+int refid_egaca_gate_dw_bwd_parts(int h, int wd, int c);
+int refid_egaca_gate_dw_bwd(const float* gxs, const float* s, const float* gm, float inv_hw, const float* dwe,
+                            const float* in, int ld_in, const float* w, float* gin, float* gxi, int accumulate_xi,
+                            float* dw, float* db, float* parts, int n, int h, int wd, int c, void* stream);
 int refid_gelu_fwd(const float* in, float* out, long long count, void* stream);
 int refid_gelu_bwd(const float* g, const float* in, float* out, long long count, void* stream);
 int refid_colsum_parts(long long npix, int c);
diff --git a/refid_amd/_lib.py b/refid_amd/_lib.py
--- a/refid_amd/_lib.py
+++ b/refid_amd/_lib.py
@@ -19,6 +19,9 @@
         ("xs_out", C.c_void_p), ("ld_xs_out", C.c_int),
         ("res2", C.c_void_p), ("ld_res2", C.c_int),
         ("out2", C.c_void_p), ("ld_out2", C.c_int),
+        ("ln_bwd_x", C.c_void_p), ("ld_ln_bwd_x", C.c_int), ("ln_bwd_gamma", C.c_void_p), ("ln_bwd_res", C.c_void_p),
+        ("ld_ln_bwd_res", C.c_int),
+        ("ln_bwd_parts", C.c_void_p), ("ln_bwd_dw", C.c_void_p), ("ln_bwd_db", C.c_void_p),
     ]
 
 
@@ -258,6 +261,9 @@
     L.refid_scale_cat.argtypes = [vp, vp, vp, vp, i, i, i, vp]
     L.refid_egaca_gs_reduce.argtypes = [vp, vp, vp, vp, vp, i, i, i, vp]
     L.refid_egaca_bwd_elem.argtypes = [vp, vp, vp, f, vp, vp, vp, i, i, i, i, vp]
+    L.refid_egaca_gs_se_bwd.argtypes = [vp] * 16 + [i, i, i, vp]
+    L.refid_egaca_gate_dw_bwd_parts.argtypes = [i, i, i]
+    L.refid_egaca_gate_dw_bwd.argtypes = [vp, vp, vp, f, vp, vp, i, vp, vp, vp, i, vp, vp, vp, i, i, i, i, vp]
     L.refid_gelu_fwd.argtypes = [vp, vp, ll, vp]
     L.refid_gelu_bwd.argtypes = [vp, vp, vp, ll, vp]
     L.refid_colsum.argtypes = [vp, i, vp, vp, ll, i, vp]
diff --git a/refid_amd/csrc/conv_args.h b/refid_amd/csrc/conv_args.h
--- a/refid_amd/csrc/conv_args.h
+++ b/refid_amd/csrc/conv_args.h
@@ -44,5 +44,9 @@
     float* xsOut = nullptr; int ldXs = 0;
     const float* res2 = nullptr; int ldR2 = 0;
     float* out2 = nullptr; int ldO2 = 0;
+    const float* lnbX = nullptr; int ldLnbX = 0; const float* lnbG = nullptr; const float* lnbRes = nullptr; int ldLnbRes = 0;
+    float* lnbParts = nullptr; float* lnbDw = nullptr; float* lnbDb = nullptr;
 };
+int refid_rows_sum_issue(const float* parts, int nrows, int ncols, float* dst_a, int n_a, float* dst_b, hipStream_t st,
+                         const char* what);
 int refid_launch_pointwise(const ConvKArgs& a, hipStream_t st, const PwExtra* ex = nullptr, int terms = 0);
diff --git a/refid_amd/csrc/conv_igemm.hip b/refid_amd/csrc/conv_igemm.hip
--- a/refid_amd/csrc/conv_igemm.hip
+++ b/refid_amd/csrc/conv_igemm.hip
@@ -452,9 +452,12 @@
             e.xsOut = x->xs_out; e.ldXs = x->ld_xs_out;
             e.res2 = x->res2; e.ldR2 = x->ld_res2;
             e.out2 = x->out2; e.ldO2 = x->ld_out2;
+            e.lnbX = x->ln_bwd_x; e.ldLnbX = x->ld_ln_bwd_x; e.lnbG = x->ln_bwd_gamma; e.lnbRes = x->ln_bwd_res; e.ldLnbRes = x->ld_ln_bwd_res;
+            e.lnbParts = x->ln_bwd_parts; e.lnbDw = x->ln_bwd_dw; e.lnbDb = x->ln_bwd_db;
             auto al = [](const void* q, int ld) { return (reinterpret_cast<uintptr_t>(q) & 15) == 0 && ld % 4 == 0; };
             REFID_CHECK((!e.lnOut || al(e.lnOut, e.ldLn)) && (!e.xsOut || al(e.xsOut, e.ldXs)) && (!e.res2 || al(e.res2, e.ldR2)) &&
-                            (!e.out2 || al(e.out2, e.ldO2)) && (!e.lnG || (al(e.lnG, 4) && al(e.lnB, 4))),
+                            (!e.out2 || al(e.out2, e.ldO2)) && (!e.lnG || (al(e.lnG, 4) && al(e.lnB, 4))) &&
+                            (!e.lnbX || (al(e.lnbX, e.ldLnbX) && al(e.lnbG, 4) && (!e.lnbRes || al(e.lnbRes, e.ldLnbRes)))),
                         "conv2d: pointwise fusion tensors must be 16-byte aligned with pitches that are multiples of 4");
             return refid_launch_pointwise(a, st, &e, d->mfma_terms);
         }
diff --git a/refid_amd/csrc/conv_pw.hip b/refid_amd/csrc/conv_pw.hip
--- a/refid_amd/csrc/conv_pw.hip
+++ b/refid_amd/csrc/conv_pw.hip
@@ -6,12 +6,18 @@
 
 namespace {
 
+__device__ __forceinline__ float pw_group_sum16(float v) {
+#pragma unroll
+    for (int o = 8; o > 0; o >>= 1) v += __shfl_xor(v, o, 64);
+    return v;
+}
+
 typedef unsigned int u32x4 __attribute__((ext_vector_type(4)));
 constexpr int KC = 8;
 __device__ constexpr int PW_TA[6] = {0, 1, 0, 2, 0, 1};
 __device__ constexpr int PW_TB[6] = {0, 0, 1, 0, 2, 1};
 
-template <int NT, int XD, bool EX, bool SIX = false>
+template <int NT, int XD, bool EX, bool SIX = false, bool LNB = false>
 __global__ __launch_bounds__(256, (SIX || NT > 2) ? 3 : 4) void conv_pw_kernel(const ConvKArgs a, const PwExtra e) {
     const int lane = threadIdx.x & 63, wave = threadIdx.x >> 6;
     const int li = lane & 31, kh = lane >> 5;
@@ -212,6 +218,8 @@
         constexpr int PITCH = 8 * HN + 1;
         __shared__ f32x4 sT[4][32 * PITCH];
         f32x4* t = sT[wave];
+        f32x4 lnx[LNB ? 4 : 1], lnr[LNB ? 4 : 1], lnw, pdw = {0.f, 0.f, 0.f, 0.f}, pdb = {0.f, 0.f, 0.f, 0.f};
+        if constexpr (LNB) lnw = *reinterpret_cast<const f32x4*>(e.lnbG + (lane & 15) * 4);
 #pragma unroll
         for (int h0 = 0; h0 < NT; h0 += HN) {
             if (h0) __syncthreads();
@@ -227,12 +235,39 @@
             __syncthreads();
 #pragma unroll
             for (int it = 0; it < 4 * HN; ++it) {
+                if constexpr (LNB) {
+                    if ((it & 3) == 0) {
+#pragma unroll
+                        for (int u = 0; u < 4; ++u) {
+                            const long long pq = p0 + (it + u) * 4 + (lane >> 4);
+                            const long long pc = pq < npix ? pq : 0;
+                            lnx[u] = *reinterpret_cast<const f32x4*>(e.lnbX + pc * e.ldLnbX + (lane & 15) * 4);
+                            lnr[u] = e.lnbRes ? *reinterpret_cast<const f32x4*>(e.lnbRes + pc * e.ldLnbRes + (lane & 15) * 4)
+                                              : f32x4{0.f, 0.f, 0.f, 0.f};
+                        }
+                    }
+                }
                 const int f = it * 64 + lane;
                 const int px = f / (8 * HN), c4 = f % (8 * HN);
                 const long long pp = p0 + px;
                 const int j0 = n0 + h0 * 32 + c4 * 4;
                 if (pp >= npix || j0 >= a.Cout) continue;
                 f32x4 v = t[px * PITCH + c4];
+                if constexpr (LNB) {
+                    const f32x4 x = lnx[it & 3];
+                    const float mu = pw_group_sum16(x[0] + x[1] + x[2] + x[3]) * (1.f / 64);
+                    const f32x4 d = x - mu;
+                    const float var = pw_group_sum16(d[0] * d[0] + d[1] * d[1] + d[2] * d[2] + d[3] * d[3]) * (1.f / 64);
+                    const float rstd = 1.f / sqrtf(var + e.lnEps);
+                    const f32x4 y = d * rstd;
+                    const f32x4 gh = v * lnw;
+                    const float m1 = pw_group_sum16(gh[0] + gh[1] + gh[2] + gh[3]) * (1.f / 64);
+                    const float m2 = pw_group_sum16(gh[0] * y[0] + gh[1] * y[1] + gh[2] * y[2] + gh[3] * y[3]) * (1.f / 64);
+                    *reinterpret_cast<f32x4*>(a.out + pp * a.ldO + j0) = (gh - y * m2 - m1) * rstd + lnr[it & 3];
+                    pdw += v * y;
+                    pdb += v;
+                    continue;
+                }
                 if (a.shuffle) {
                     const int Co1 = a.Cout >> 2;
                     const unsigned qd = (unsigned)j0 / (unsigned)Co1, ch = (unsigned)j0 - qd * Co1;
@@ -255,6 +290,19 @@
                     }
                 }
             }
+        }
+        if constexpr (LNB) {
+            __shared__ float sred[4][128];
+            __syncthreads();
+#pragma unroll
+            for (int k = 0; k < 4; ++k) {
+                const float sw = refid_wave_rows_sum<16>(pdw[k]), sb = refid_wave_rows_sum<16>(pdb[k]);
+                if (lane < 16) { sred[wave][lane * 4 + k] = sw; sred[wave][64 + lane * 4 + k] = sb; }
+            }
+            __syncthreads();
+            if (threadIdx.x < 128)
+                e.lnbParts[(long long)blockIdx.x * 128 + threadIdx.x] =
+                    ((sred[0][threadIdx.x] + sred[1][threadIdx.x]) + sred[2][threadIdx.x]) + sred[3][threadIdx.x];
         }
         return;
     }
@@ -290,6 +338,16 @@
     REFID_CHECK(terms == 0 || terms == 6, "conv2d: the pointwise tile has fp32 products (0) or six bf16 products (6), got %d", terms);
     REFID_CHECK(!six || (a.Ctot % 16 == 0 && (a.inB == nullptr || a.Ca % 16 == 0) && a.Cout > 32),
                 "conv2d: the six-product pointwise tile needs channel counts that are multiples of 16 and more than 32 outputs");
+    if (ex != nullptr && ex->lnbX != nullptr) {
+        REFID_CHECK(a.vecOK && !six && a.Cout == 64 && !a.shuffle && !a.patchW && !a.bias && !a.res && !a.mask && !a.out2 &&
+                        a.slopePre == 1.f && a.slopePost == 1.f && !ex->lnG && !ex->pool && !ex->res2 && !ex->out2,
+                    "conv2d: the LayerNorm backward epilogue needs 64 outputs in one column tile, 16-byte aligned tensors and no "
+                    "bias / residual / mask / activation / other fusion (got %d outputs)", a.Cout);
+        REFID_CHECK(ex->lnbG && ex->lnbParts && ex->lnbDw && ex->lnbDb, "conv2d: the LayerNorm backward epilogue needs gamma, parts, dw and db");
+        hipLaunchKernelGGL((conv_pw_kernel<2, 4, false, false, true>), dim3(nb, 1), dim3(256), 0, st, a, *ex);
+        REFID_LAUNCH_CHECK("conv_pw/ln_bwd");
+        return refid_rows_sum_issue(ex->lnbParts, nb, 128, ex->lnbDw, 64, ex->lnbDb, st, "conv_pw/ln_bwd sum");
+    }
     if (ex != nullptr) {
         REFID_CHECK(a.vecOK && a.Cout > 32, "conv2d: pointwise fusions need 16-byte aligned tensors and more than 32 outputs");
         REFID_CHECK(!ex->lnG || (a.inB == nullptr && a.Ctot % 8 == 0 && a.Ctot <= 64 && ex->lnB),
diff --git a/refid_amd/csrc/egaca.hip b/refid_amd/csrc/egaca.hip
--- a/refid_amd/csrc/egaca.hip
+++ b/refid_amd/csrc/egaca.hip
@@ -1,4 +1,5 @@
 #include "common.h"
+#include "conv_args.h"
 #include <vector>
 #include <cstring>
 
@@ -477,6 +478,184 @@
     }
 }
 
+__global__ __launch_bounds__(256) void gs_se_bwd_kernel(const float* __restrict__ parts, int nblk, const float* __restrict__ s,
+                                                       const float* __restrict__ z1, const float* __restrict__ m,
+                                                       const float* __restrict__ W1, const float* __restrict__ W2,
+                                                       float* __restrict__ gs, float* __restrict__ gm,
+                                                       float* __restrict__ dW1, float* __restrict__ db1,
+                                                       float* __restrict__ dW2, float* __restrict__ db2, int N, int C) {
+    extern __shared__ float sh[];
+    float* dd = sh + 1024;
+    const int Ch = C / 2, S = C + Ch;
+    {
+        const int c = threadIdx.x % C, r = threadIdx.x / C, R = 256 / C;
+        for (int n0 = 0; n0 < N; n0 += 4) {
+            float a[4] = {0.f, 0.f, 0.f, 0.f};
+            const float* pp[4];
+#pragma unroll
+            for (int u = 0; u < 4; ++u) pp[u] = parts + (long long)min(n0 + u, N - 1) * nblk * C + c;
+            for (int b = r; b < nblk; b += R) {
+#pragma unroll
+                for (int u = 0; u < 4; ++u) a[u] += pp[u][(long long)b * C];
+            }
+#pragma unroll
+            for (int u = 0; u < 4; ++u) sh[u * 256 + threadIdx.x] = a[u];
+            __syncthreads();
+            for (int i = threadIdx.x; i < 4 * C; i += 256) {
+                const int u = i / C, cc = i % C, n = n0 + u;
+                if (n < N) {
+                    float t = sh[u * 256 + cc];
+                    for (int k = 1; k < R; ++k) t += sh[u * 256 + k * C + cc];
+                    if (blockIdx.x == 0) gs[n * C + cc] = t;
+                    const float sv = s[n * C + cc];
+                    dd[n * S + cc] = t * sv * (1.f - sv);
+                }
+            }
+            __syncthreads();
+        }
+    }
+    for (int i = threadIdx.x; i < N * Ch; i += 256) {
+        const int n = i / Ch, j = i % Ch;
+        float a = 0.f;
+        for (int c = 0; c < C; ++c) a += W2[c * Ch + j] * dd[n * S + c];
+        dd[n * S + C + j] = z1[n * Ch + j] > 0.f ? a : 0.f;
+    }
+    __syncthreads();
+    if (blockIdx.x == 0)
+        for (int i = threadIdx.x; i < N * C; i += 256) {
+            const int n = i / C, c = i % C;
+            float a = 0.f;
+            for (int j = 0; j < Ch; ++j) a += W1[j * C + c] * dd[n * S + C + j];
+            gm[n * C + c] = a;
+        }
+    const int e = blockIdx.x * 256 + threadIdx.x;
+    if (e < C * Ch) {
+        float a2 = 0.f, a1 = 0.f;
+        for (int n = 0; n < N; ++n) {
+            a2 += dd[n * S + e / Ch] * z1[n * Ch + e % Ch];
+            a1 += dd[n * S + C + e / C] * m[n * C + e % C];
+        }
+        dW2[e] += a2;
+        dW1[e] += a1;
+    }
+    if (e < C) { float a = 0.f; for (int n = 0; n < N; ++n) a += dd[n * S + e]; db2[e] += a; }
+    if (e < Ch) { float a = 0.f; for (int n = 0; n < N; ++n) a += dd[n * S + C + e]; db1[e] += a; }
+}
+constexpr int GS_SE_MAX_FLOATS = 6144;
+
+constexpr int GD_TH = 8, GD_TW = 16, GD_HW = GD_TW + 2, GD_HALO = (GD_TH + 2) * GD_HW;
+__global__ __launch_bounds__(256, 3) void egaca_gate_dw_bwd_kernel(const float* __restrict__ gxs, const float* __restrict__ s,
+                                                               const float* __restrict__ gm, float invHW,
+                                                               const float* __restrict__ dwe, const float* __restrict__ in,
+                                                               int ldi, const float* __restrict__ w, float* __restrict__ gin,
+                                                               float* gxi, int accXi, float* __restrict__ parts, int H, int W,
+                                                               int tilesX) {
+    constexpr int C = 64, LPP = 16;
+    __shared__ f32x4 tile[GD_HALO * LPP];
+    const int q = threadIdx.x % LPP, r = threadIdx.x / LPP, n = blockIdx.y;
+    const int ty0 = ((int)blockIdx.x / tilesX) * GD_TH, tx0 = ((int)blockIdx.x % tilesX) * GD_TW;
+    const long long org = ((long long)n * H + ty0) * W + tx0;
+    const f32x4 sv = *reinterpret_cast<const f32x4*>(s + n * C + q * 4);
+    const f32x4 gmv = *reinterpret_cast<const f32x4*>(gm + n * C + q * 4);
+    const int x = tx0 + r;
+#pragma unroll 1
+    for (int i0 = 0; i0 < GD_TH; i0 += 4) {
+        f32x4 gi[4], old[4];
+        bool ok[4];
+#pragma unroll
+        for (int u = 0; u < 4; ++u) {
+            ok[u] = ty0 + i0 + u < H && x < W;
+            const long long pix = ok[u] ? org + (long long)(i0 + u) * W + r : org;
+            gi[u] = *reinterpret_cast<const f32x4*>(gxs + pix * 2 * C + q * 4);
+            old[u] = accXi ? *reinterpret_cast<const f32x4*>(gxi + pix * C + q * 4) : f32x4{0.f, 0.f, 0.f, 0.f};
+        }
+#pragma unroll
+        for (int u = 0; u < 4; ++u) {
+            f32x4 xi = gi[u] * sv;
+            if (accXi) xi += old[u];
+            if (ok[u]) *reinterpret_cast<f32x4*>(gxi + (org + (long long)(i0 + u) * W + r) * C + q * 4) = xi;
+        }
+    }
+#pragma unroll 1
+    for (int h0 = r; h0 < GD_HALO; h0 += 64) {
+        f32x4 ge[4], dv[4];
+        bool ok[4];
+#pragma unroll
+        for (int u = 0; u < 4; ++u) {
+            const int hp = h0 + 16 * u;
+            const int hy = ty0 - 1 + hp / GD_HW, hx = tx0 - 1 + hp % GD_HW;
+            ok[u] = hp < GD_HALO && hy >= 0 && hy < H && hx >= 0 && hx < W;
+            const long long pix = ok[u] ? ((long long)n * H + hy) * W + hx : org;
+            ge[u] = *reinterpret_cast<const f32x4*>(gxs + pix * 2 * C + C + q * 4);
+            dv[u] = *reinterpret_cast<const f32x4*>(dwe + pix * C + q * 4);
+        }
+#pragma unroll
+        for (int u = 0; u < 4; ++u) {
+            const int hp = h0 + 16 * u;
+            f32x4 o;
+#pragma unroll
+            for (int k = 0; k < 4; ++k) o[k] = ok[u] ? (ge[u][k] * sv[k] + gmv[k] * invHW) * gelu_d(dv[u][k]) : 0.f;
+            if (hp < GD_HALO) tile[hp * LPP + q] = o;
+        }
+    }
+    float wr[4][9], pw[4][9];
+#pragma unroll
+    for (int k = 0; k < 4; ++k)
+#pragma unroll
+        for (int t = 0; t < 9; ++t) { wr[k][t] = w[(q * 4 + k) * 9 + t]; pw[k][t] = 0.f; }
+    f32x4 pb = {0.f, 0.f, 0.f, 0.f};
+    __syncthreads();
+#pragma unroll 1
+    for (int i0 = 0; i0 < GD_TH; i0 += 2) {
+        f32x4 cv[2];
+        bool ok[2];
+#pragma unroll
+        for (int u = 0; u < 2; ++u) {
+            ok[u] = ty0 + i0 + u < H && x < W;
+            const long long pix = ok[u] ? org + (long long)(i0 + u) * W + r : org;
+            cv[u] = *reinterpret_cast<const f32x4*>(in + pix * ldi + q * 4);
+            if (!ok[u]) cv[u] = f32x4{0.f, 0.f, 0.f, 0.f};
+        }
+#pragma unroll
+        for (int u = 0; u < 2; ++u) {
+            const int i = i0 + u;
+            f32x4 a = {0.f, 0.f, 0.f, 0.f};
+#pragma unroll
+            for (int dy = 0; dy < 3; ++dy)
+#pragma unroll
+                for (int dx = 0; dx < 3; ++dx) {
+                    const int t = dy * 3 + dx;
+                    const f32x4 gn = tile[((i + 2 - dy) * GD_HW + (r + 2 - dx)) * LPP + q];
+#pragma unroll
+                    for (int k = 0; k < 4; ++k) {
+                        a[k] += gn[k] * wr[k][t];
+                        pw[k][t] += cv[u][k] * gn[k];
+                    }
+                    if (t == 4) pb += gn;
+                }
+            if (ok[u]) *reinterpret_cast<f32x4*>(gin + (org + (long long)i * W + r) * C + q * 4) = a;
+        }
+    }
+    __syncthreads();
+    float* sred = reinterpret_cast<float*>(tile);
+    const int wave = threadIdx.x >> 6, lane = threadIdx.x & 63;
+#pragma unroll
+    for (int k = 0; k < 4; ++k) {
+#pragma unroll
+        for (int t = 0; t < 9; ++t) {
+            const float a = wave_rows_sum<LPP>(pw[k][t]);
+            if (lane < LPP) sred[wave * (C * 10) + (q * 4 + k) * 9 + t] = a;
+        }
+        const float b = wave_rows_sum<LPP>(pb[k]);
+        if (lane < LPP) sred[wave * (C * 10) + C * 9 + q * 4 + k] = b;
+    }
+    __syncthreads();
+    float* dst = parts + ((long long)blockIdx.y * gridDim.x + blockIdx.x) * (C * 10);
+    for (int i = threadIdx.x; i < C * 10; i += 256)
+        dst[i] = ((sred[i] + sred[C * 10 + i]) + sred[2 * C * 10 + i]) + sred[3 * C * 10 + i];
+}
+static_assert(GD_HALO * 16 * 16 >= 4 * 64 * 10 * 4, "the tile's LDS also holds the four waves' partial sums");
+
 __global__ __launch_bounds__(256) void gelu_fwd_kernel(const f32x4* __restrict__ in, f32x4* __restrict__ out, long long n4) {
     for (long long i = blockIdx.x * 256ll + threadIdx.x; i < n4; i += (long long)gridDim.x * 256) {
         const f32x4 v = in[i];
@@ -547,6 +726,11 @@
 
 }
 
+int refid_rows_sum_issue(const float* parts, int nrows, int ncols, float* dst_a, int n_a, float* dst_b, hipStream_t st,
+                         const char* what) {
+    return rows_sum_issue(parts, nrows, ncols, dst_a, n_a, dst_b, st, what);
+}
+
 #define LPP_DISPATCH(C, CALL)                                                     \
     switch (C) {                                                                  \
         case 16: { constexpr int LPP = 4; CALL; break; }                          \
@@ -676,6 +860,48 @@
     return 0;
 }
 
+extern "C" int refid_egaca_gs_se_bwd(const float* gxs, const float* xi, const float* xe, float* gs, float* parts,
+                                     const float* s, const float* z1, const float* m, const float* w1, const float* w2,
+                                     float* gm, float* dw1, float* db1, float* dw2, float* db2, float* scratch, int n, int hw,
+                                     int c, void* stream) {
+    REFID_CHECK(gxs && xi && xe && gs && parts && s && z1 && m && w1 && w2 && gm && dw1 && db1 && dw2 && db2 && n > 0 && hw > 0,
+                "egaca_gs_se_bwd: bad arguments");
+    const bool one = c >= 4 && c <= 256 && 256 % c == 0 && (long long)n * (c + c / 2) <= GS_SE_MAX_FLOATS;
+    if (!one) {
+        REFID_CHECK(scratch, "egaca_gs_se_bwd: n = %d, c = %d takes the three-launch form, which needs `scratch`", n, c);
+        if (int rc = refid_egaca_gs_reduce(gxs, xi, xe, gs, parts, n, hw, c, stream)) return rc;
+        return refid_se_bwd(gs, s, z1, m, w1, w2, gm, dw1, db1, dw2, db2, scratch, n, c, stream);
+    }
+    hipStream_t st = (hipStream_t)stream;
+    const int nb = refid_egaca_gs_reduce_parts(hw, c);
+    LPP_DISPATCH(c, hipLaunchKernelGGL(gs_reduce_kernel<LPP>, dim3(nb, n), dim3(256), 0, st, gxs, xi, xe, parts, hw));
+    REFID_LAUNCH_CHECK("egaca_gs_se_bwd/reduce");
+    hipLaunchKernelGGL(gs_se_bwd_kernel, dim3(cdiv(c * (c / 2), 256)), dim3(256), (1024 + n * (c + c / 2)) * sizeof(float), st,
+                       parts, nb, s, z1, m, w1, w2, gs, gm, dw1, db1, dw2, db2, n, c);
+    REFID_LAUNCH_CHECK("egaca_gs_se_bwd");
+    return 0;
+}
+
+extern "C" int refid_egaca_gate_dw_bwd_parts(int h, int wd, int c) {
+    if (c != 64 || h <= 0 || wd <= 0) return -1;
+    return cdiv(h, GD_TH) * cdiv(wd, GD_TW);
+}
+
+extern "C" int refid_egaca_gate_dw_bwd(const float* gxs, const float* s, const float* gm, float inv_hw, const float* dwe,
+                                       const float* in, int ld_in, const float* w, float* gin, float* gxi, int accumulate_xi,
+                                       float* dw, float* db, float* parts, int n, int h, int wd, int c, void* stream) {
+    REFID_CHECK(gxs && s && gm && dwe && in && w && gin && gxi && dw && db && parts && n > 0 && n <= 65535 && h > 0 && wd > 0 &&
+                ld_in >= c && ld_in % 4 == 0, "egaca_gate_dw_bwd: bad arguments");
+    REFID_CHECK(c == 64, "egaca_gate_dw_bwd: c = %d (the tiled form is for 64 channels: refid_egaca_bwd_elem + "
+                "refid_dwconv3x3_bwd take the other widths)", c);
+    hipStream_t st = (hipStream_t)stream;
+    const int nb = refid_egaca_gate_dw_bwd_parts(h, wd, c);
+    hipLaunchKernelGGL(egaca_gate_dw_bwd_kernel, dim3(nb, n), dim3(256), 0, st, gxs, s, gm, inv_hw, dwe, in, ld_in, w, gin, gxi,
+                       accumulate_xi, parts, h, wd, cdiv(wd, GD_TW));
+    REFID_LAUNCH_CHECK("egaca_gate_dw_bwd");
+    return rows_sum_issue(parts, nb * n, c * 10, dw, c * 9, db, st, "egaca_gate_dw_bwd/sum");
+}
+
 extern "C" int refid_gelu_fwd(const float* in, float* out, long long count, void* stream) {
     REFID_CHECK(in && out && count > 0 && count % 4 == 0, "gelu_fwd: bad arguments");
     hipLaunchKernelGGL(gelu_fwd_kernel, dim3(blocks_for(count / 4, 256)), dim3(256), 0, (hipStream_t)stream,
diff --git a/refid_amd/engine.py b/refid_amd/engine.py
--- a/refid_amd/engine.py
+++ b/refid_amd/engine.py
@@ -468,7 +468,11 @@
     def gelu_mask_ok(self, g, rows=None):
         return self.wd is not None and self._dgrad_route(g, rows[1] if rows is not None else self.d_rows)[3]
 
-    def dgrad(self, g, rows=None, res=None, mask=None, slope_mask=1.0, out=None, plus=None, gelu_mask=False):
+    def ln_bwd_ok(self, g):
+        return self.wd is not None and self.kind == "conv" and self.k == 1 and self.d_rows == 64 and \
+            g.shape[0] * g.stride(0) < _LIM4 and self._dgrad_route(g, self.d_rows)[3]
+
+    def dgrad(self, g, rows=None, res=None, mask=None, slope_mask=1.0, out=None, plus=None, gelu_mask=False, ln_bwd=None):
         if self.wd is None:
             raise RefidHipError(f"{self.name}: dgrad weights were not requested")
         base, cnt = rows if rows is not None else (0, self.d_rows)
@@ -492,6 +496,13 @@
                                     f"apply ops.gelu_bwd separately")
             fused = fused and plus is not None and len(parts) == 1
             extra = dict(add2=plus, out2=o2) if fused else (dict(mask_mode=1) if gelu_mask else {})
+            if ln_bwd is not None:
+                if not gelu_ok or cnt != 64 or rows is not None or res is not None or mask is not None or plus is not None or \
+                        len(parts) != 1:
+                    raise RefidHipError(f"{self.name}: ln_bwd needs the whole 64-channel input gradient from the fp32 pointwise "
+                                        f"tile, without res / mask / plus (see ln_bwd_ok)")
+                extra["pw"] = dict(ln_bwd_x=ln_bwd["x"], ln_bwd_gamma=ln_bwd["gamma"], ln_bwd_res=ln_bwd.get("res"),
+                                   ln_bwd_dw=ln_bwd["dw"], ln_bwd_db=ln_bwd["db"])
             if self.d_role == ops.ROLE_CONVT_DGRAD_PW and g_i.stride(2) != g_i.shape[3]:
                 g_i = g_i.contiguous()
             ops.conv2d(g_i, self._packed(attr), out_i, cout=cnt, co_base=base, res=res_i, mask=mask_i, slope_mask=slope_mask,
@@ -841,6 +852,7 @@
 
     def _egaca_bwd(self, A, g_u, img_grad, ip, st, gy_keep=None):
         e = st["eg"]
+        strict = os.environ.get("REFID_EGACA_BWD") == "2"
         A.conv5.wgrad(g_u, e["f4"])
         if LINEAR_SPLIT and A.conv5.gelu_mask_ok(g_u):
             g_c4 = A.conv5.dgrad(g_u, mask=e["c4"], gelu_mask=True)
@@ -848,29 +860,48 @@
             g_f4 = A.conv5.dgrad(g_u)
             g_c4 = ops.gelu_bwd(g_f4, e["c4"], out=g_f4)
         A.conv4.wgrad(g_c4, e["ln2"])
-        g_ln2 = A.conv4.dgrad(g_c4)
         A.side.wgrad(g_u, e["y"])
         g_y = A.side.dgrad(g_u)
-        ops.layernorm2d_bwd(g_ln2, e["y"], A.p("norm2.weight"), g_y, A.g("norm2.weight"), A.g("norm2.bias"),
-                            accumulate=True)
+        if A.conv4.ln_bwd_ok(g_c4):
+            A.conv4.dgrad(g_c4, out=g_y, ln_bwd=dict(x=e["y"], gamma=A.p("norm2.weight"), res=g_y, dw=A.g("norm2.weight"),
+                                                     db=A.g("norm2.bias")))
+        elif strict:
+            raise RuntimeError("REFID_EGACA_BWD=2, but conv4's input gradient cannot carry the LayerNorm backward")
+        else:
+            g_ln2 = A.conv4.dgrad(g_c4)
+            ops.layernorm2d_bwd(g_ln2, e["y"], A.p("norm2.weight"), g_y, A.g("norm2.weight"), A.g("norm2.bias"),
+                                accumulate=True)
         A.conv3.wgrad(g_y, e["xs"])
         g_xs = A.conv3.dgrad(g_y)
-        gs = ops.egaca_gs_reduce(g_xs, ip["xi"], e["xe"])
-        gm = ops.se_bwd(gs, e["s"], e["z1"], e["m"], A.p("se_1.1.weight"), A.p("se_1.3.weight"),
-                        A.g("se_1.1.weight"), A.g("se_1.1.bias"), A.g("se_1.3.weight"), A.g("se_1.3.bias"))
+        _, gm = ops.egaca_gs_se_bwd(g_xs, ip["xi"], e["xe"], e["s"], e["z1"], e["m"], A.p("se_1.1.weight"),
+                                    A.p("se_1.3.weight"), A.g("se_1.1.weight"), A.g("se_1.1.bias"), A.g("se_1.3.weight"),
+                                    A.g("se_1.3.bias"), strict=strict)
         first = ip["gxi"] is None
         if first:
             ip["gxi"] = torch.empty_like(ip["xi"])
-        g_dwe = ops.egaca_bwd_elem(g_xs, e["s"], gm, e["dwe"], ip["gxi"], accumulate_xi=not first)
-        g_c1e = ops.dwconv3x3_bwd(g_dwe, e["c1e"], A.p("conv2_e.weight"), A.g("conv2_e.weight"), A.g("conv2_e.bias"))
+        if ops.egaca_gate_dw_bwd_parts(*e["dwe"].shape[1:]) > 0:
+            g_c1e = ops.egaca_gate_dw_bwd(g_xs, e["s"], gm, e["dwe"], e["c1e"], A.p("conv2_e.weight"), ip["gxi"], not first,
+                                          A.g("conv2_e.weight"), A.g("conv2_e.bias"))
+        elif strict:
+            raise RuntimeError(f"REFID_EGACA_BWD=2, but {e['dwe'].shape[3]} channels take the unfused gate + depthwise backward")
+        else:
+            g_dwe = ops.egaca_bwd_elem(g_xs, e["s"], gm, e["dwe"], ip["gxi"], accumulate_xi=not first)
+            g_c1e = ops.dwconv3x3_bwd(g_dwe, e["c1e"], A.p("conv2_e.weight"), A.g("conv2_e.weight"), A.g("conv2_e.bias"))
         A.conv1_e.wgrad(g_c1e, e["ln_e"])
-        g_lne = A.conv1_e.dgrad(g_c1e)
+        fuse_ln = A.conv1_e.ln_bwd_ok(g_c1e)
+        if strict and not fuse_ln:
+            raise RuntimeError("REFID_EGACA_BWD=2, but conv1_e's input gradient cannot carry the LayerNorm backward")
+        g_lne = None if fuse_ln else A.conv1_e.dgrad(g_c1e)
         if gy_keep is not None:
             gy_keep.append(g_y)
         else:
             ops.add(img_grad, g_y, out=img_grad)
-        g_ev = ops.layernorm2d_bwd(g_lne, e["ev"], A.p("norm1_e.weight"), torch.empty_like(g_y),
-                                   A.g("norm1_e.weight"), A.g("norm1_e.bias"), res=g_y)
+        if fuse_ln:
+            g_ev = A.conv1_e.dgrad(g_c1e, ln_bwd=dict(x=e["ev"], gamma=A.p("norm1_e.weight"), res=g_y,
+                                                      dw=A.g("norm1_e.weight"), db=A.g("norm1_e.bias")))
+        else:
+            g_ev = ops.layernorm2d_bwd(g_lne, e["ev"], A.p("norm1_e.weight"), torch.empty_like(g_y),
+                                       A.g("norm1_e.weight"), A.g("norm1_e.bias"), res=g_y)
         return g_ev
 
     def _egaca_img_bwd(self, A, img, img_grad, ip):
diff --git a/refid_amd/ops.py b/refid_amd/ops.py
--- a/refid_amd/ops.py
+++ b/refid_amd/ops.py
@@ -168,6 +168,19 @@
         if pw["out2"].shape != out.shape:
             raise _lib.RefidHipError("conv2d: out2 shape differs from the output's")
         x.out2, x.ld_out2 = _nhwc(pw["out2"], "out2")
+    if pw.get("ln_bwd_x") is not None:
+        for k in ("ln_bwd_x", "ln_bwd_res"):
+            if pw.get(k) is not None and pw[k].shape != out.shape:
+                raise _lib.RefidHipError(f"conv2d: {k} shape differs from the output's")
+        x.ln_bwd_x, x.ld_ln_bwd_x = _nhwc(pw["ln_bwd_x"], "ln_bwd_x")
+        x.ln_bwd_gamma, x.ln_eps = _c(pw["ln_bwd_gamma"], "ln_bwd_gamma"), pw.get("ln_eps", 1e-6)
+        if pw.get("ln_bwd_res") is not None:
+            x.ln_bwd_res, x.ld_ln_bwd_res = _nhwc(pw["ln_bwd_res"], "ln_bwd_res")
+        x.ln_bwd_dw, x.ln_bwd_db = _c(pw["ln_bwd_dw"], "ln_bwd_dw"), _c(pw["ln_bwd_db"], "ln_bwd_db")
+        npix = out.shape[0] * out.shape[1] * out.shape[2]
+        parts = torch.empty((-(-npix // 128), 128), dtype=torch.float32, device=out.device)
+        x.ln_bwd_parts = parts.data_ptr()
+        _keep_rows(parts)
     return x
 
 
@@ -658,6 +671,42 @@
     return gdwe
 
 
+def egaca_gs_se_bwd(gxs, xi, xe, s, z1, m, w1, w2, dw1, db1, dw2, db2, strict=False):
+    n, h, w, c = xi.shape
+    gs = torch.empty((n, c), dtype=torch.float32, device=xi.device)
+    gm = torch.empty_like(gs)
+    nb = lib().refid_egaca_gs_reduce_parts(h * w, c)
+    if nb <= 0:
+        raise _lib.RefidHipError(f"egaca_gs_se_bwd: unsupported channel count {c}")
+    parts = torch.empty((n, nb, c), dtype=torch.float32, device=xi.device)
+    scratch = None if strict else torch.empty((n, c + c // 2), dtype=torch.float32, device=xi.device)
+    check(lib().refid_egaca_gs_se_bwd(_c(gxs, "gxs"), _c(xi, "xi"), _c(xe, "xe"), gs.data_ptr(), parts.data_ptr(), _c(s, "s"),
+                                      _c(z1, "z1"), _c(m, "m"), _c(w1, "w1"), _c(w2, "w2"), gm.data_ptr(), _c(dw1, "dw1"),
+                                      _c(db1, "db1"), _c(dw2, "dw2"), _c(db2, "db2"),
+                                      scratch.data_ptr() if scratch is not None else None, n, h * w, c, _stream()),
+          "refid_egaca_gs_se_bwd")
+    return gs, gm
+
+
+def egaca_gate_dw_bwd_parts(h, w, c):
+    return lib().refid_egaca_gate_dw_bwd_parts(h, w, c)
+
+
+def egaca_gate_dw_bwd(gxs, s, gm, dwe, x, w, gxi, accumulate_xi, dw, db):
+    px, ld = _nhwc(x, "x")
+    n, h, wd, c = dwe.shape
+    nparts = lib().refid_egaca_gate_dw_bwd_parts(h, wd, c)
+    if nparts <= 0:
+        raise _lib.RefidHipError(f"egaca_gate_dw_bwd: no tiled form for {c} channels")
+    gin = torch.empty((n, h, wd, c), dtype=torch.float32, device=dwe.device)
+    parts = torch.empty((n * nparts, 10 * c), dtype=torch.float32, device=dwe.device)
+    check(lib().refid_egaca_gate_dw_bwd(_c(gxs, "gxs"), _c(s, "s"), _c(gm, "gm"), 1.0 / (h * wd), _c(dwe, "dwe"), px, ld,
+                                        _c(w, "w"), gin.data_ptr(), _c(gxi, "gxi"), int(accumulate_xi), _c(dw, "dw"),
+                                        _c(db, "db"), parts.data_ptr(), n, h, wd, c, _stream()), "refid_egaca_gate_dw_bwd")
+    _keep_rows(parts)
+    return gin
+
+
 def gelu_fwd(x):
     out = torch.empty_like(x)
     check(lib().refid_gelu_fwd(_c(x, "x"), out.data_ptr(), x.numel(), _stream()), "refid_gelu_fwd")
```

Result: no change. 518.9, median of 6 (+0.2%).
